# cheshmi/parsy_bench

Hardware: AMD Instinct MI355X
Metric: Cholesky factorizations/sec (+ SpTRSV solves/sec), SuiteSparse SPD set (higher is better)
Workload: dtype f64; 1 GPU; flan-class stand-in (BASELINE.json configs[2] when flan: Flan_1565): grid (116, 116, 116) 27-point stencil, geometric nested dissection; n=1560896, nnz_A_lower=21491316, nsuper=81191, nnz_L=2044454227, xsize=2421483055, etree_levels=17, launches_per_factorization=357, parallelism=1 GPU

## Files before the change

### parsy_bench_amd/csrc/capi_exec.hip

```cpp
#include <hip/hip_runtime.h>

#include <chrono>
#include <cstdio>
#include <cstring>
#include <map>
#include <algorithm>
#include <atomic>
#include <mutex>
#include <thread>
#include <string>
#include <tuple>
#include <vector>

#include "../../include/parsy_amd.h"
#include "errors.hpp"
#include "hip_check.hpp"
#include "dist.hpp"
#include "executor.hpp"
#include "inspector.hpp"
#include "refine.hpp"

using parsy::set_last_error;

namespace {

double now_s() {
    return std::chrono::duration<double>(std::chrono::steady_clock::now().time_since_epoch()).count();
}

int pick_device() {
    const char* e = std::getenv("PARSY_DEVICE");
    return e ? std::atoi(e) : 0;
}

uint64_t fnv(uint64_t h, const void* p, size_t bytes) {
    const unsigned char* c = (const unsigned char*)p;
    uint64_t lane[4] = {h, h ^ 0x9E3779B97F4A7C15ULL, h ^ 0xC2B2AE3D27D4EB4FULL, h ^ 0x165667B19E3779F9ULL};
    size_t i = 0;
    for (; i + 32 <= bytes; i += 32)
        for (int k = 0; k < 4; ++k) {
            uint64_t w;
            std::memcpy(&w, c + i + 8 * k, 8);
            lane[k] = (lane[k] ^ w) * 1099511628211ULL;
            lane[k] ^= lane[k] >> 29;
        }
    for (int k = 0; k < 4; ++k) h = (h ^ lane[k]) * 1099511628211ULL;
    for (; i < bytes; ++i) {
        h ^= c[i];
        h *= 1099511628211ULL;
    }
    return h ^ (uint64_t)bytes;
}

struct CacheKey {
    const void* a;
    const void* b;
    const void* c;
    uint64_t hash;
    int n, supNo, kind;
    bool operator<(const CacheKey& o) const {
        return std::tie(a, b, c, hash, n, supNo, kind) < std::tie(o.a, o.b, o.c, o.hash, o.n, o.supNo, o.kind);
    }
};

std::mutex g_mu;
std::map<CacheKey, parsy_plan*> g_plans;

bool validate_partition(int supNo, int nLevels, const int* levelPtr, const int* parPtr,
                        const int* partition, const char* who) {
    if (!levelPtr || !parPtr || !partition || nLevels < 1) {
        set_last_error(std::string(who) + ": null H-level schedule");
        return false;
    }
    std::vector<char> seen(supNo, 0);
    const int nparts = levelPtr[nLevels];
    int cnt = 0;
    for (int q = 0; q < nparts; ++q)
        for (int k = parPtr[q]; k < parPtr[q + 1]; ++k) {
            const int s = partition[k];
            if (s < 0 || s >= supNo || seen[s]) {
                set_last_error(std::string(who) + ": H-level partition is not a permutation of the supernodes");
                return false;
            }
            seen[s] = 1;
            ++cnt;
        }
    if (cnt != supNo) {
        set_last_error(std::string(who) + ": H-level partition does not cover every supernode");
        return false;
    }
    return true;
}

bool validate_levelset(int supNo, int nLevels, const int* levelPtr, const int* levelSet, const char* who) {
    if (!levelPtr || !levelSet || nLevels < 1 || levelPtr[nLevels] != supNo) {
        set_last_error(std::string(who) + ": level set does not cover every supernode");
        return false;
    }
    std::vector<char> seen(supNo, 0);
    for (int k = 0; k < supNo; ++k) {
        const int s = levelSet[k];
        if (s < 0 || s >= supNo || seen[s]) {
            set_last_error(std::string(who) + ": level set is not a permutation of the supernodes");
            return false;
        }
        seen[s] = 1;
    }
    return true;
}

void loud(const char* who) {
    std::fprintf(stderr, "[parsy_amd] %s failed: %s\n", who, parsy_last_error());
}

parsy_plan* cached_chol_plan(int n, int supNo, const int* blockSet, const size_t* lC,
                             const size_t* Li_ptr, const int* lR, const int* aTree,
                             const int* col2Sup, const int* cT, const int* rT, const int* c,
                             const int* r) {
    uint64_t h = 1469598103934665603ULL;
    h = fnv(h, blockSet, sizeof(int) * (supNo + 1));
    h = fnv(h, lR, sizeof(int) * Li_ptr[n]);
    h = fnv(h, c, sizeof(int) * (n + 1));
    h = fnv(h, r, sizeof(int) * c[n]);
    h = fnv(h, Li_ptr, sizeof(size_t) * (n + 1));
    h = fnv(h, lC, sizeof(size_t) * (n + 1));
    h = fnv(h, aTree, sizeof(int) * supNo);
    CacheKey key{blockSet, lR, c, h, n, supNo, 0};
    std::lock_guard<std::mutex> lk(g_mu);
    auto it = g_plans.find(key);
    if (it != g_plans.end()) return it->second;
    parsy_plan* pl = parsy_plan_create(n, supNo, blockSet, lC, Li_ptr, lR, aTree, col2Sup, cT, rT, c, r,
                                       pick_device());
    if (pl) g_plans[key] = pl;
    return pl;
}

parsy_plan* cached_chol_plan_prune(int n, int supNo, const int* blockSet, const size_t* lC, const size_t* Li_ptr,
                                   const int* lR, const int* prunePtr, const int* pruneSet, const int* c,
                                   const int* r) {
    uint64_t h = 1469598103934665603ULL;
    h = fnv(h, blockSet, sizeof(int) * (supNo + 1));
    h = fnv(h, lR, sizeof(int) * Li_ptr[n]);
    h = fnv(h, c, sizeof(int) * (n + 1));
    h = fnv(h, r, sizeof(int) * c[n]);
    h = fnv(h, Li_ptr, sizeof(size_t) * (n + 1));
    h = fnv(h, lC, sizeof(size_t) * (n + 1));
    h = fnv(h, prunePtr, sizeof(int) * (supNo + 1));
    h = fnv(h, pruneSet, sizeof(int) * prunePtr[supNo]);
    CacheKey key{blockSet, lR, c, h, n, supNo, 2};
    std::lock_guard<std::mutex> lk(g_mu);
    auto it = g_plans.find(key);
    if (it != g_plans.end()) return it->second;
    const int dev = pick_device();
    if (dev >= parsy_device_count()) {
        set_last_error("cholesky_left_par_05_prune: no usable HIP device " + std::to_string(dev) +
                       " (this library has no CPU fallback)");
        return nullptr;
    }
    std::vector<int> col2sup(n), sparent(supNo, -1);
    for (int s = 0; s < supNo; ++s)
        for (int k = blockSet[s]; k < blockSet[s + 1]; ++k) col2sup[k] = s;
    for (int s = 0; s < supNo; ++s) {
        const int w = blockSet[s + 1] - blockSet[s];
        const size_t b = Li_ptr[blockSet[s]], e = Li_ptr[blockSet[s + 1]];
        if (e - b > (size_t)w) sparent[s] = col2sup[lR[b + w]];
    }
    parsy::PatternRef P;
    P.n = n;
    P.nsuper = supNo;
    P.super = blockSet;
    P.col2sup = col2sup.data();
    P.sparent = sparent.data();
    P.i_ptr = Li_ptr;
    P.s = lR;
    P.prunePtr = prunePtr;
    P.pruneSet = pruneSet;
    parsy_plan* pl = parsy::plan_build(P, lC, c, r, dev);
    if (pl) g_plans[key] = pl;
    return pl;
}

parsy_plan* cached_solve_plan(int n, int supNo, const size_t* Lp, const int* Li, const size_t* Li_ptr,
                              const int* sup2col) {
    uint64_t h = 1469598103934665603ULL;
    h = fnv(h, sup2col, sizeof(int) * (supNo + 1));
    h = fnv(h, Li, sizeof(int) * Li_ptr[n]);
    h = fnv(h, Li_ptr, sizeof(size_t) * (n + 1));
    h = fnv(h, Lp, sizeof(size_t) * (n + 1));
    CacheKey key{sup2col, Li, Lp, h, n, supNo, 1};
    std::lock_guard<std::mutex> lk(g_mu);
    auto it = g_plans.find(key);
    if (it != g_plans.end()) return it->second;
    std::vector<int> col2sup(n), sparent(supNo, -1);
    for (int s = 0; s < supNo; ++s)
        for (int k = sup2col[s]; k < sup2col[s + 1]; ++k) col2sup[k] = s;
    for (int s = 0; s < supNo; ++s) {
        const int w = sup2col[s + 1] - sup2col[s];
        const size_t b = Li_ptr[sup2col[s]], e = Li_ptr[sup2col[s + 1]];
        if (e - b > (size_t)w) sparent[s] = col2sup[Li[b + w]];
    }
    parsy::PatternRef P;
    P.n = n;
    P.nsuper = supNo;
    P.super = sup2col;
    P.col2sup = col2sup.data();
    P.sparent = sparent.data();
    P.i_ptr = Li_ptr;
    P.s = Li;
    if (parsy_device_count() < 1) {
        set_last_error("no usable HIP device: the BCSC solve has no CPU fallback in this library");
        return nullptr;
    }
    parsy_plan* pl = parsy::plan_build(P, Lp, nullptr, nullptr, pick_device());
    if (pl) g_plans[key] = pl;
    return pl;
}

int dropin_solve(const char* who, int n, size_t* Lp, int* Li, double* Lx, size_t* Li_ptr,
                 int* sup2col, int supNo, double* x) {
    if (!Lp || !Li || !x) return 0;
    parsy_plan* pl = cached_solve_plan(n, supNo, Lp, Li, Li_ptr, sup2col);
    std::unique_lock<std::mutex> use;
    if (pl) use = std::unique_lock<std::mutex>(pl->use_mu);
    if (!pl || parsy_solve_host(pl, Lx, x, 1, n, nullptr) != 0) {
        loud(who);
        return 0;
    }
    return 1;
}

}

extern "C" {

int parsy_device_count(void) {
    int n = 0;
    if (hipGetDeviceCount(&n) != hipSuccess) return 0;
    return n;
}

parsy_plan* parsy_plan_create(int n, int supNo, const int* blockSet, const size_t* lC,
                              const size_t* Li_ptr, const int* lR, const int* aTree,
                              const int* col2Sup, const int* cT, const int* rT, const int* c,
                              const int* r, int device) {
    if (!blockSet || !lC || !Li_ptr || !lR || !aTree || !col2Sup || !cT || !rT || !c || !r || n < 0 ||
        supNo < 0) {
        set_last_error("parsy_plan_create: null or negative argument");
        return nullptr;
    }
    if (device >= 0 && device >= parsy_device_count()) {
        set_last_error("parsy_plan_create: no usable HIP device " + std::to_string(device) +
                       " (this library has no CPU fallback; pass device < 0 for a host-only schedule)");
        return nullptr;
    }
    parsy::PatternRef P;
    P.n = n;
    P.nsuper = supNo;
    P.super = blockSet;
    P.col2sup = col2Sup;
    P.sparent = aTree;
    P.i_ptr = Li_ptr;
    P.s = lR;
    P.A1p = cT;
    P.A1i = rT;
    return parsy::plan_build(P, lC, c, r, device);
}

parsy_plan* parsy_plan_from_symbolic(const parsy_symbolic* sym, int device) {
    const parsy::Symbolic* S = parsy_symbolic_cxx(sym);
    if (!S) {
        set_last_error("parsy_plan_from_symbolic: null symbolic");
        return nullptr;
    }
    return parsy_plan_create(S->n, S->nsuper, S->super.data(), S->p.data(), S->i_ptr.data(), S->s.data(),
                             S->sparent.data(), S->col2sup.data(), S->A1.p.data(), S->A1.i.data(),
                             S->A2.p.data(), S->A2.i.data(), device);
}

void parsy_plan_destroy(parsy_plan* plan) { parsy::plan_free(plan); }

int parsy_plan_get_info(const parsy_plan* pl, parsy_plan_info* o) {
    if (!pl || !o) return -1;
    const parsy::Schedule& S = pl->S;
    std::memset(o, 0, sizeof(*o));
    o->n = S.n;
    o->nsuper = S.nsuper;
    o->nlevels = S.nlevels;
    o->max_width = S.max_width;
    o->max_rows = S.max_rows;
    o->n_small = S.n_small;
    o->n_big = S.n_big;
    o->chol_launches = (int32_t)S.chol.size() + 1;
    o->solve_launches = (int32_t)S.solve.size();
    o->nnzA = S.nnzA;
    o->ssize = S.ssize;
    o->xsize = S.xsize;
    o->nnzL = S.nnzL;
    o->n_updates = (int64_t)S.upd.size();
    o->relpos_len = (int64_t)S.relpos.size();
    o->device_bytes = pl->device_bytes;
    o->flops_stored = S.flops_stored;
    o->update_flops = S.update_flops;
    o->reread_bytes = S.reread_bytes;
    o->inner_flops = S.inner_flops;
    o->tile_update_flops = S.tile_update_flops;
    o->big_flops = S.big_flops;
    o->big_entries = (int64_t)S.big_entries.size();
    o->big_tasks = (int32_t)S.big_tasks.size();
    o->n_pieces = (int32_t)S.csn.size();
    o->chol_levels = S.cnlevels;
    o->piece_width = S.piece_width;
    o->big_min_k = S.big_min_k;
    o->chol_subtrees = (int32_t)S.small_ranges.size() / 2;
    for (size_t b = 0; b + 1 < S.small_ranges.size(); b += 2) o->chol_subtree_supernodes += S.small_ranges[b + 1] - S.small_ranges[b];
    o->solve_subtrees = (int32_t)S.solve_small_ranges.size() / 2;
    for (size_t b = 0; b + 1 < S.solve_small_ranges.size(); b += 2)
        o->solve_subtree_supernodes += S.solve_small_ranges[b + 1] - S.solve_small_ranges[b];
    o->backsolve_launches = (int32_t)S.bsolve.size();
    for (const parsy::Launch& l : S.chol)
        if (l.kind == parsy::kLaunchDense) o->dense_tasks += l.count;
    o->dense_flops = S.dense_flops;
    o->dense_entries = S.n_dense_entries;
    o->solve_one = (S.solve_one ? 1 : 0) | (S.solve_one_back ? 2 : 0) | ((S.solve_one || S.solve_one_back) && S.one_subtrees ? 4 : 0);
    o->solve_one_blocks = S.solve_one ? (int32_t)S.one_f.sn.size() : S.solve_one_back ? (int32_t)S.one_back().sn.size() : 0;
    o->sub_mrhs_trees = (int32_t)S.sub_trees.size();
    o->sub_mrhs_slots = S.sub_max_slots;
    o->sub_mrhs_tiers = (int32_t)S.sub_tiers.size();
    o->sub_mrhs_cover_level = S.sub_cover_level;
    o->dense_strip_entries = S.n_strip_entries;
    return 0;
}

long long parsy_plan_chain_check(const parsy_plan* pl, int slots) {
    if (!pl || slots < 1) {
        set_last_error("parsy_plan_chain_check: null plan or slots < 1");
        return -1;
    }
    return (long long)simulate_chain(pl->S, slots);
}

long long parsy_plan_check(const parsy_plan* pl) {
    if (!pl) {
        set_last_error("parsy_plan_check: null plan");
        return -1;
    }
    std::string what;
    const long long bad = (long long)parsy::check_schedule(pl->S, what);
    if (bad) set_last_error("parsy_plan_check: " + what);
    return bad;
}

int parsy_plan_set_active(parsy_plan* pl, const uint8_t* mask) {
    if (!pl) return -1;
    std::vector<uint8_t> pieces;
    if (pl->piece_mask_set) pieces = pl->S.active_piece;
    parsy::build_launches(pl->S, mask, pl->piece_mask_set ? pieces.data() : nullptr);
    pl->sn_mask_set = mask != nullptr;
    return parsy::plan_upload_launches(pl);
}

int parsy_plan_set_active_pieces(parsy_plan* pl, const uint8_t* piece_mask) {
    if (!pl) return -1;
    std::vector<uint8_t> sn_mask;
    if (pl->sn_mask_set) sn_mask = pl->S.active;
    parsy::build_launches(pl->S, pl->sn_mask_set ? sn_mask.data() : nullptr, piece_mask);
    pl->piece_mask_set = piece_mask != nullptr;
    return parsy::plan_upload_launches(pl);
}

int parsy_plan_pieces(const parsy_plan* pl, int32_t* supernode, int32_t* level, int32_t* col0, int32_t* width,
                      int32_t* rows, int64_t* value_begin, int64_t* value_end) {
    if (!pl) return -1;
    const parsy::Schedule& S = pl->S;
    const int nc = (int)S.csn.size();
    for (int p = 0; p < nc; ++p) {
        const parsy::SnDesc& C = S.csn[(size_t)p];
        const parsy::SnDesc& R = S.sn[(size_t)S.csn_real[(size_t)p]];
        if (supernode) supernode[p] = S.csn_real[(size_t)p];
        if (level) level[p] = S.level_of.empty() ? 0 : S.level_of[(size_t)p];
        if (col0) col0[p] = C.c0;
        if (width) width[p] = C.w;
        if (rows) rows[p] = C.r;
        if (value_begin) value_begin[p] = R.px + (int64_t)C.rbias * R.r;
        if (value_end) value_end[p] = R.px + (int64_t)(C.rbias + C.w) * R.r;
    }
    return nc;
}

int parsy_plan_solve_levels(const parsy_plan* pl, int32_t* level) {
    if (!pl) return -1;
    const parsy::Schedule& S = pl->S;
    if (level)
        for (int l = 0; l < S.nlevels; ++l)
            for (int q = S.levelPtr[(size_t)l]; q < S.levelPtr[(size_t)l + 1]; ++q) level[S.levelSet[(size_t)q]] = l;
    return S.nlevels;
}

int64_t parsy_debug_big_entries(const parsy_plan* pl, int32_t* out, int64_t cap) {
    if (!pl) return -1;
    const parsy::Schedule& S = pl->S;
    int64_t n = 0, t = 0;
    for (const parsy::Schedule::BigTask& b : S.big_all) {
        for (int64_t e = b.e0; e < b.e1; ++e, ++n) {
            if (!out || n >= cap) continue;
            const parsy::WaveEntry& E = S.big_entries[(size_t)e];
            int32_t* o = out + 7 * n;
            o[0] = (int32_t)t;
            o[1] = b.src_level * 2 + (b.next ? 0 : 1);
            o[2] = E.K;
            o[3] = E.mn & 255;
            o[4] = (E.mn >> 8) & 255;
            o[5] = ((E.mn >> 16) & 1) != 0;
            o[6] = E.ia - E.ja;
        }
        ++t;
    }
    return n;
}

int64_t parsy_debug_big_windows(const parsy_plan* pl, int64_t* out, int64_t cap) {
    if (!pl) return -1;
    const parsy::Schedule& S = pl->S;
    int64_t n = 0, t = 0;
    for (const parsy::Schedule::BigTask& b : S.big_all) {
        for (int64_t e = b.e0; e < b.e1; ++e, ++n) {
            if (!out || n >= cap) continue;
            const parsy::WaveEntry& E = S.big_entries[(size_t)e];
            int64_t* o = out + 9 * n;
            o[0] = t;
            o[1] = b.src_level * 2 + (b.next ? 0 : 1);
            o[2] = E.K;
            o[3] = E.mn & 255;
            o[4] = (E.mn >> 8) & 255;
            o[5] = E.ia;
            o[6] = E.ja;
            o[7] = E.src;
            o[8] = e < b.em;
        }
        ++t;
    }
    return n;
}

int64_t parsy_debug_dense_tasks(const parsy_plan* pl, int32_t* out, int64_t cap) {
    if (!pl) return -1;
    const parsy::Schedule& S = pl->S;
    int64_t n = 0;
    int li = 0;
    for (const parsy::Launch& l : S.chol) {
        if (l.kind != parsy::kLaunchDense) continue;
        for (int q = l.first; q < l.first + l.count; ++q, ++n)
            if (out && n < cap) {
                out[2 * n] = li;
                out[2 * n + 1] = S.big_tasks[(size_t)q].part;
            }
        ++li;
    }
    return n;
}

int64_t parsy_debug_launch_times(const parsy_plan* pl, double* out, int64_t cap) {
    if (!pl) return -1;
    const int64_t n = (int64_t)std::min(pl->pev_ms.size(), pl->pev_kind.size());
    for (int64_t i = 0; out && i < n && i < cap; ++i) {
        out[4 * i] = pl->pev_kind[(size_t)i];
        out[4 * i + 1] = (size_t)i < pl->pev_level.size() ? pl->pev_level[(size_t)i] : -1;
        out[4 * i + 2] = (size_t)i < pl->pev_count.size() ? pl->pev_count[(size_t)i] : 0;
        out[4 * i + 3] = pl->pev_ms[(size_t)i];
    }
    return n;
}

int parsy_factor_begin(parsy_plan* pl, const double* d_values, double* d_lValues, void* stream, int flags) {
    if (!pl || !d_values || !d_lValues) {
        set_last_error("parsy_factor_begin: null argument");
        return -1;
    }
    return parsy::plan_factor_begin(pl, d_values, d_lValues, (hipStream_t)stream, (flags & PARSY_FACTOR_NO_INIT) == 0);
}

int parsy_factor_level(parsy_plan* pl, int level, double* d_lValues, void* stream) {
    if (!pl || !d_lValues) {
        set_last_error("parsy_factor_level: null argument");
        return -1;
    }
    return parsy::plan_factor_levels(pl, level, level + 1, d_lValues, (hipStream_t)stream);
}

int parsy_factor_end(parsy_plan* pl, void* stream) {
    if (!pl) {
        set_last_error("parsy_factor_end: null plan");
        return -1;
    }
    return parsy::plan_factor_end(pl, (hipStream_t)stream);
}

int parsy_factor_device(parsy_plan* pl, const double* d_values, double* d_lValues, void* stream) {
    if (!pl || !d_values || !d_lValues) {
        set_last_error("parsy_factor_device: null argument");
        return -1;
    }
    return parsy::plan_factor(pl, d_values, d_lValues, (hipStream_t)stream);
}

int parsy_factor_device_ex(parsy_plan* pl, const double* d_values, double* d_lValues, void* stream,
                           int flags) {
    if (!pl || !d_values || !d_lValues) {
        set_last_error("parsy_factor_device_ex: null argument");
        return -1;
    }
    return parsy::plan_factor(pl, d_values, d_lValues, (hipStream_t)stream,
                              (flags & PARSY_FACTOR_NO_INIT) == 0);
}

int parsy_factor_status(parsy_plan* pl) {
    if (!pl || pl->device < 0) return -1;
    int v = 0;
    if (hipMemcpy(&v, pl->dp.info, sizeof(int), hipMemcpyDeviceToHost) != hipSuccess) return -1;
    return v >= 0x7f7f7f7f ? 0 : v;
}

int parsy_solve_status(parsy_plan* pl) {
    if (!pl || pl->device < 0) return -1;
    int v = 0;
    const int* word = pl->solve_status_word ? pl->solve_status_word : pl->dp.sinfo;
    if (hipMemcpy(&v, word, sizeof(int), hipMemcpyDeviceToHost) != hipSuccess) return -1;
    if (v < 0) set_last_error("solve: a hand-off wait inside a chain launch timed out; x is not the solution");
    return v < 0 ? -1 : 0;
}

int parsy_solve_device(parsy_plan* pl, const double* d_lValues, double* d_x, int nrhs, int ldx,
                       void* stream) {
    if (!pl || !d_lValues || !d_x) {
        set_last_error("parsy_solve_device: null argument");
        return -1;
    }
    return parsy::plan_solve(pl, d_lValues, d_x, nrhs, ldx, (hipStream_t)stream);
}

double parsy_last_factor_ms(parsy_plan* pl) {
    float ms = -1;
    if (!pl || !pl->have_f) return -1;
    if (hipEventSynchronize(pl->ev_f1) != hipSuccess) return -1;
    if (hipEventElapsedTime(&ms, pl->ev_f0, pl->ev_f1) != hipSuccess) return -1;
    return ms;
}

double parsy_last_solve_ms(parsy_plan* pl) {
    float ms = -1;
    if (!pl || !pl->have_s) return -1;
    if (hipEventSynchronize(pl->ev_s1) != hipSuccess) return -1;
    if (hipEventElapsedTime(&ms, pl->ev_s0, pl->ev_s1) != hipSuccess) return -1;
    return ms;
}

int parsy_plan_profile(parsy_plan* pl, int enable) {
    if (!pl) return -1;
    pl->profile = enable != 0;
    if (enable == 2) {
        for (int k = 0; k < 10; ++k) pl->kind_ms[k] = 0, pl->kind_launches[k] = 0;
        pl->profiled_runs = 0;
        pl->level_ms.clear();
    }
    return 0;
}

int parsy_plan_profile_collect(parsy_plan* pl) { return pl ? parsy::plan_collect_profile(pl) : -1; }

int parsy_plan_profile_get(parsy_plan* pl, double* kind_ms, int* kind_launches, int* runs) {
    if (!pl) return -1;
    for (int k = 0; k < 10; ++k) {
        if (kind_ms) kind_ms[k] = pl->kind_ms[k];
        if (kind_launches) kind_launches[k] = pl->kind_launches[k];
    }
    if (runs) *runs = pl->profiled_runs;
    return 0;
}

int parsy_plan_profile_levels(parsy_plan* pl, double* main_ms, double* side_ms) {
    if (!pl) return -1;
    const int nl = pl->S.cnlevels;
    for (int l = 0; l < nl; ++l) {
        const size_t a = (size_t)l << 1, b = a | 1;
        if (main_ms) main_ms[l] = a < pl->level_ms.size() ? pl->level_ms[a] : 0.0;
        if (side_ms) side_ms[l] = b < pl->level_ms.size() ? pl->level_ms[b] : 0.0;
    }
    return nl;
}

static void build_download_bands(parsy_plan* pl) {
    const parsy::Schedule& S = pl->S;
    const int nl = S.cnlevels, np = (int)S.csn.size();
    {
        std::vector<double> bytes((size_t)nl, 0.0);
        for (int p = 0; p < np; ++p) bytes[(size_t)S.level_of[(size_t)p]] += 8.0 * S.csn[(size_t)p].w * S.csn[(size_t)p].ld;
        const double total = 8.0 * (double)S.xsize;
        pl->h_band_level.clear();
        double run = 0, next = total / 8;
        for (int l = 0; l < nl; ++l) {
            run += bytes[(size_t)l];
            if (l == nl - 1 || run >= next) {
                pl->h_band_level.push_back(l);
                while (next <= run) next += total / 8;
            }
        }
    }
    const size_t nb = pl->h_band_level.size();
    pl->h_band_runs.assign(nb, {});
    std::vector<int> band_of((size_t)nl, 0);
    for (size_t b = 0, l = 0; b < nb; ++b)
        for (; (int)l <= pl->h_band_level[b]; ++l) band_of[l] = (int)b;
    const int64_t gap = 131072;
    for (int p = 0; p < np; ++p) {
        const parsy::SnDesc& C = S.csn[(size_t)p];
        const parsy::SnDesc& R = S.sn[(size_t)S.csn_real[(size_t)p]];
        const int64_t a = R.px + (int64_t)C.rbias * R.r, e = R.px + (int64_t)(C.rbias + C.w) * R.r;
        auto& runs = pl->h_band_runs[(size_t)band_of[(size_t)S.level_of[(size_t)p]]];
        if (!runs.empty() && a - (runs.back().first + runs.back().second) <= gap && a >= runs.back().first)
            runs.back().second = std::max(runs.back().second, e - runs.back().first);
        else
            runs.push_back({a, e - a});
    }
}

int parsy_factor_host(parsy_plan* pl, const double* values, double* lValues, double* seconds) {
    if (!pl || !values || !lValues) {
        set_last_error("parsy_factor_host: null argument");
        return -1;
    }
    if (pl->device < 0) {
        set_last_error("parsy_factor_host: plan has no device");
        return -1;
    }
    const parsy::Schedule& S = pl->S;
    PARSY_HIP(hipSetDevice(pl->device));
    if (!pl->h_values_dev) PARSY_HIP(hipMalloc((void**)&pl->h_values_dev, std::max<int64_t>(S.nnzA, 1) * 8));
    if (!pl->h_L_dev) PARSY_HIP(hipMalloc((void**)&pl->h_L_dev, std::max<int64_t>(S.xsize, 1) * 8));
    PARSY_HIP(hipMemcpy(pl->h_values_dev, values, (size_t)S.nnzA * 8, hipMemcpyHostToDevice));
    const char* pe = std::getenv("PARSY_HOST_PIPELINE");
    const bool pipeline_on = !(pe && pe[0] == '0'), pipeline_forced = pe && pe[0] == '2';
    if (!pipeline_on || (!pipeline_forced && S.xsize * 8 < (int64_t)256 << 20) || pl->profile || S.cnlevels < 1) {
        if (parsy::plan_factor(pl, pl->h_values_dev, pl->h_L_dev, nullptr) != 0) return -1;
        PARSY_HIP(hipDeviceSynchronize());
        if (seconds) *seconds = parsy_last_factor_ms(pl) * 1e-3;
        PARSY_HIP(hipMemcpy(lValues, pl->h_L_dev, (size_t)S.xsize * 8, hipMemcpyDeviceToHost));
        return 0;
    }
    if (!pl->h_ready) {
        hipStream_t hs = nullptr, hc = nullptr;
        std::vector<hipEvent_t> evs;
        auto undo = [&] {
            for (hipEvent_t e : evs) (void)hipEventDestroy(e);
            if (hs) (void)hipStreamDestroy(hs);
            if (hc) (void)hipStreamDestroy(hc);
            pl->h_band_level.clear();
            pl->h_band_runs.clear();
            (void)hipGetLastError();
        };
        bool ok = hipStreamCreateWithFlags(&hs, hipStreamNonBlocking) == hipSuccess &&
                  hipStreamCreateWithFlags(&hc, hipStreamNonBlocking) == hipSuccess;
        if (ok) {
            build_download_bands(pl);
            evs.resize(pl->h_band_level.size(), nullptr);
            for (hipEvent_t& e : evs)
                if (ok && hipEventCreateWithFlags(&e, hipEventDisableTiming) != hipSuccess) {
                    e = nullptr;
                    ok = false;
                }
            ok = ok && !evs.empty();
        }
        if (!ok) {
            evs.erase(std::remove(evs.begin(), evs.end(), (hipEvent_t) nullptr), evs.end());
            undo();
            if (parsy::plan_factor(pl, pl->h_values_dev, pl->h_L_dev, nullptr) != 0) return -1;
            PARSY_HIP(hipDeviceSynchronize());
            if (seconds) *seconds = parsy_last_factor_ms(pl) * 1e-3;
            PARSY_HIP(hipMemcpy(lValues, pl->h_L_dev, (size_t)S.xsize * 8, hipMemcpyDeviceToHost));
            return 0;
        }
        pl->h_stream = hs;
        pl->h_copy = hc;
        pl->h_band_ev = evs;
        pl->h_ready = true;
    }
    const size_t nb = pl->h_band_level.size();
    std::atomic<int> recorded{0};
    std::atomic<int> failed{0};
    double* const dL = pl->h_L_dev;
    const int device = pl->device;
    std::thread worker([&, dL, device] {
        if (hipSetDevice(device) != hipSuccess) {
            failed = 1;
            return;
        }
        for (size_t b = 0; b < nb; ++b) {
            while (recorded.load(std::memory_order_acquire) <= (int)b && !failed.load()) std::this_thread::yield();
            if (failed.load()) return;
            if (hipEventSynchronize(pl->h_band_ev[b]) != hipSuccess) {
                failed = 1;
                return;
            }
            for (const auto& r : pl->h_band_runs[b])
                if (hipMemcpyAsync(lValues + r.first, dL + r.first, (size_t)r.second * 8, hipMemcpyDeviceToHost, pl->h_copy) !=
                    hipSuccess) {
                    failed = 1;
                    return;
                }
            if (hipStreamSynchronize(pl->h_copy) != hipSuccess) {
                failed = 1;
                return;
            }
        }
    });
    int rc = parsy::plan_factor_begin(pl, pl->h_values_dev, dL, pl->h_stream, true);
    size_t b = 0;
    for (int lev = 0; rc == 0 && lev < S.cnlevels; ++lev) {
        rc = parsy::plan_factor_levels(pl, lev, lev + 1, dL, pl->h_stream);
        if (rc == 0 && b < nb && pl->h_band_level[b] == lev) {
            if (hipEventRecord(pl->h_band_ev[b], pl->h_stream) != hipSuccess) rc = -1;
            ++b;
            recorded.store((int)b, std::memory_order_release);
        }
    }
    if (rc == 0) rc = parsy::plan_factor_end(pl, pl->h_stream);
    if (rc != 0) {
        failed = 1;
        worker.join();
        parsy::plan_factor_abort(pl, pl->h_stream);
        return -1;
    }
    const hipError_t es = hipStreamSynchronize(pl->h_stream);
    worker.join();
    if (es != hipSuccess || failed.load()) {
        set_last_error("parsy_factor_host: the pipelined download failed");
        return -1;
    }
    if (seconds) *seconds = parsy_last_factor_ms(pl) * 1e-3;
    return 0;
}

int parsy_solve_host(parsy_plan* pl, const double* lValues, double* x, int nrhs, int ldx,
                     double* seconds) {
    if (!pl || !lValues || !x) {
        set_last_error("parsy_solve_host: null argument");
        return -1;
    }
    if (pl->device < 0) {
        set_last_error("parsy_solve_host: plan has no device");
        return -1;
    }
    const parsy::Schedule& S = pl->S;
    PARSY_HIP(hipSetDevice(pl->device));
    if (!pl->h_L_dev) PARSY_HIP(hipMalloc((void**)&pl->h_L_dev, std::max<int64_t>(S.xsize, 1) * 8));
    const int64_t need = (int64_t)ldx * nrhs;
    PARSY_HIP(parsy::grow_device(pl->h_x_dev, pl->h_x_len, need));
    PARSY_HIP(hipMemcpy(pl->h_L_dev, lValues, (size_t)S.xsize * 8, hipMemcpyHostToDevice));
    PARSY_HIP(hipMemcpy(pl->h_x_dev, x, (size_t)need * 8, hipMemcpyHostToDevice));
    if (parsy::plan_solve(pl, pl->h_L_dev, pl->h_x_dev, nrhs, ldx, nullptr) != 0) return -1;
    PARSY_HIP(hipDeviceSynchronize());
    if (parsy_solve_status(pl) != 0) return -1;
    if (seconds) *seconds = parsy_last_solve_ms(pl) * 1e-3;
    PARSY_HIP(hipMemcpy(x, pl->h_x_dev, (size_t)need * 8, hipMemcpyDeviceToHost));
    return 0;
}

int parsy_backsolve_device(parsy_plan* pl, const double* d_lValues, double* d_x, int nrhs, int ldx,
                           void* stream) {
    if (!pl || !d_lValues || !d_x) {
        set_last_error("parsy_backsolve_device: null argument");
        return -1;
    }
    return parsy::plan_backsolve(pl, d_lValues, d_x, nrhs, ldx, (hipStream_t)stream);
}

int parsy_solve_levels_device(parsy_plan* pl, const double* d_lValues, double* d_x, int nrhs, int ldx, void* stream,
                              int level_begin, int level_end, int flags) {
    if (!pl || !d_lValues || !d_x) {
        set_last_error("parsy_solve_levels_device: null argument");
        return -1;
    }
    return parsy::plan_solve_levels(pl, d_lValues, d_x, nrhs, ldx, (hipStream_t)stream, level_begin, level_end, flags);
}

int parsy_copy_segments_device(double* d_dst, const double* d_src, const int64_t* d_dst_off,
                               const int64_t* d_src_off, const int32_t* d_len, int64_t nseg, void* stream) {
    if (nseg < 0 || (nseg > 0 && (!d_dst || !d_src || !d_dst_off || !d_src_off || !d_len))) {
        set_last_error("parsy_copy_segments_device: null argument");
        return -1;
    }
    parsy::launch_copy_segments(d_dst, d_src, d_dst_off, d_src_off, d_len, nseg, (hipStream_t)stream);
    PARSY_HIP(hipGetLastError());
    return 0;
}

int parsy_rhs_ones_device(parsy_plan* pl, const double* d_lValues, double* d_b, void* stream) {
    if (!pl || !d_lValues || !d_b || pl->device < 0) {
        set_last_error("parsy_rhs_ones_device: null argument or plan without a device");
        return -1;
    }
    PARSY_HIP(hipSetDevice(pl->device));
    PARSY_HIP(hipMemsetAsync(d_b, 0, (size_t)pl->S.n * sizeof(double), (hipStream_t)stream));
    parsy::launch_rhs_ones(pl->dp, pl->S.nsuper, pl->S.max_rows, d_lValues, d_b, (hipStream_t)stream);
    PARSY_HIP(hipGetLastError());
    return 0;
}

int parsy_solve2_host(parsy_plan* pl, const double* lValues, double* x, int nrhs, int ldx, int forward,
                      double* seconds) {
    if (!pl || !lValues || !x) {
        set_last_error("parsy_solve2_host: null argument");
        return -1;
    }
    if (pl->device < 0) {
        set_last_error("parsy_solve2_host: plan has no device");
        return -1;
    }
    const parsy::Schedule& S = pl->S;
    PARSY_HIP(hipSetDevice(pl->device));
    if (!pl->h_L_dev) PARSY_HIP(hipMalloc((void**)&pl->h_L_dev, std::max<int64_t>(S.xsize, 1) * 8));
    const int64_t need = (int64_t)ldx * nrhs;
    PARSY_HIP(parsy::grow_device(pl->h_x_dev, pl->h_x_len, need));
    PARSY_HIP(hipMemcpy(pl->h_L_dev, lValues, (size_t)S.xsize * 8, hipMemcpyHostToDevice));
    PARSY_HIP(hipMemcpy(pl->h_x_dev, x, (size_t)need * 8, hipMemcpyHostToDevice));
    double sec = 0;
    if (forward) {
        if (parsy::plan_solve(pl, pl->h_L_dev, pl->h_x_dev, nrhs, ldx, nullptr) != 0) return -1;
        PARSY_HIP(hipDeviceSynchronize());
        if (parsy_solve_status(pl) != 0) return -1;
        sec += parsy_last_solve_ms(pl) * 1e-3;
    }
    if (parsy::plan_backsolve(pl, pl->h_L_dev, pl->h_x_dev, nrhs, ldx, nullptr) != 0) return -1;
    PARSY_HIP(hipDeviceSynchronize());
    if (parsy_solve_status(pl) != 0) return -1;
    sec += parsy_last_solve_ms(pl) * 1e-3;
    if (seconds) *seconds = sec;
    PARSY_HIP(hipMemcpy(x, pl->h_x_dev, (size_t)need * 8, hipMemcpyDeviceToHost));
    return 0;
}

int parsy_plan_set_perm(parsy_plan* pl, const int* perm) {
    if (!pl) {
        set_last_error("parsy_plan_set_perm: null plan");
        return -1;
    }
    return parsy::plan_set_perm(pl, perm);
}

int parsy_residual_device(parsy_plan* pl, const double* d_values, const double* d_x, int ldx, const double* d_b, int ldb,
                          double* d_r, int ldr, int nrhs, double* berr, void* stream) {
    if (!pl || !d_values || !d_x || !d_b) {
        set_last_error("parsy_residual_device: null argument");
        return -1;
    }
    return parsy::plan_residual(pl, d_values, d_x, ldx, d_b, ldb, d_r, ldr, nrhs, berr, (hipStream_t)stream);
}

int parsy_solve_spd_device(parsy_plan* pl, const double* d_values, const double* d_lValues, const double* d_b, int ldb,
                           double* d_x, int ldx, int nrhs, int max_steps, int32_t* steps, double* berr, void* stream) {
    if (!pl || !d_values || !d_lValues || !d_b || !d_x) {
        set_last_error("parsy_solve_spd_device: null argument");
        return -1;
    }
    return parsy::plan_solve_refined(pl, d_values, d_lValues, d_b, ldb, d_x, ldx, nrhs, max_steps, steps, berr,
                                     (hipStream_t)stream);
}

int parsy_solve_spd_host(parsy_plan* pl, const double* values, const double* lValues, const double* b, int ldb,
                         double* x, int ldx, int nrhs, int max_steps, int32_t* steps, double* berr, double* seconds) {
    if (!pl || !values || !lValues || !b || !x) {
        set_last_error("parsy_solve_spd_host: null argument");
        return -1;
    }
    if (pl->device < 0) {
        set_last_error("parsy_solve_spd_host: plan was built without a device (device < 0)");
        return -1;
    }
    const parsy::Schedule& S = pl->S;
    if (nrhs < 1 || ldb < S.n || ldx < S.n) {
        set_last_error("parsy_solve_spd_host: need nrhs >= 1 and leading dimensions >= n");
        return -1;
    }
    PARSY_HIP(hipSetDevice(pl->device));
    if (!pl->h_values_dev) PARSY_HIP(hipMalloc((void**)&pl->h_values_dev, std::max<int64_t>(S.nnzA, 1) * 8));
    if (!pl->h_L_dev) PARSY_HIP(hipMalloc((void**)&pl->h_L_dev, std::max<int64_t>(S.xsize, 1) * 8));
    const int64_t need = std::max<int64_t>((int64_t)S.n * nrhs, 1);
    PARSY_HIP(parsy::grow_device(pl->h_x_dev, pl->h_x_len, need));
    const size_t row = (size_t)S.n * 8;
    PARSY_HIP(hipMemcpy(pl->h_values_dev, values, (size_t)S.nnzA * 8, hipMemcpyHostToDevice));
    PARSY_HIP(hipMemcpy(pl->h_L_dev, lValues, (size_t)S.xsize * 8, hipMemcpyHostToDevice));
    if (S.n > 0) PARSY_HIP(hipMemcpy2D(pl->h_x_dev, row, b, (size_t)ldb * 8, row, nrhs, hipMemcpyHostToDevice));
    hipEvent_t e0 = nullptr, e1 = nullptr;
    PARSY_HIP(hipEventCreate(&e0));
    if (hipEventCreate(&e1) != hipSuccess) {
        (void)hipEventDestroy(e0);
        set_last_error("parsy_solve_spd_host: hipEventCreate failed");
        return -1;
    }
    (void)hipEventRecord(e0, nullptr);
    int rc = parsy::plan_solve_refined(pl, pl->h_values_dev, pl->h_L_dev, pl->h_x_dev, S.n, pl->h_x_dev, S.n, nrhs,
                                       max_steps, steps, berr, nullptr);
    float ms = 0;
    if (rc == 0 && (hipEventRecord(e1, nullptr) != hipSuccess || hipEventSynchronize(e1) != hipSuccess ||
                    hipEventElapsedTime(&ms, e0, e1) != hipSuccess)) {
        set_last_error("parsy_solve_spd_host: timing the call failed");
        rc = -1;
    }
    (void)hipEventDestroy(e0);
    (void)hipEventDestroy(e1);
    if (rc != 0) return -1;
    if (parsy_solve_status(pl) != 0) return -1;
    if (seconds) *seconds = ms * 1e-3;
    if (S.n > 0) PARSY_HIP(hipMemcpy2D(x, (size_t)ldx * 8, pl->h_x_dev, row, row, nrhs, hipMemcpyDeviceToHost));
    return 0;
}

void parsy_dropin_reset(void) {
    std::lock_guard<std::mutex> lk(g_mu);
    for (auto& kv : g_plans) parsy::plan_free(kv.second);
    g_plans.clear();
}


bool cholesky_left_par_05(int n, int* c, int* r, double* values, size_t* lC, int* lR, size_t* Li_ptr,
                          double* lValues, int* blockSet, int supNo, double* timing, int* aTree,
                          int* cT, int* rT, int* col2Sup, int nLevels, int* levelPtr, int* levelSet,
                          int nPar, int* parPtr, int* partition, int chunk, int threads,
                          int super_max, int col_max, double* nodCost) {
    (void)levelSet; (void)nPar; (void)chunk; (void)threads; (void)super_max; (void)col_max; (void)nodCost;
    const char* who = "cholesky_left_par_05";
    const double t0 = now_s();
    if (!validate_partition(supNo, nLevels, levelPtr, parPtr, partition, who)) {
        loud(who);
        return false;
    }
    parsy_plan* pl = cached_chol_plan(n, supNo, blockSet, lC, Li_ptr, lR, aTree, col2Sup, cT, rT, c, r);
    double dev_s = 0;
    std::unique_lock<std::mutex> use;
    if (pl) use = std::unique_lock<std::mutex>(pl->use_mu);
    if (!pl || parsy_factor_host(pl, values, lValues, &dev_s) != 0) {
        loud(who);
        return false;
    }
    if (timing) {
        timing[0] = now_s() - t0;
        timing[1] = 0.0;
        timing[2] = dev_s;
    }
    return parsy_factor_status(pl) == 0;
}

bool cholesky_left_par_05_prune(int n, int* c, int* r, double* values, size_t* lC, int* lR, size_t* Li_ptr,
                                double* lValues, int* blockSet, int supNo, double* timing, int* prunePtr,
                                int* pruneSet, int nLevels, int* levelPtr, int* levelSet, int nPar, int* parPtr,
                                int* partition, int chunk, int threads, int super_max, int col_max,
                                double* nodCost) {
    (void)levelSet; (void)nPar; (void)chunk; (void)threads; (void)super_max; (void)col_max; (void)nodCost;
    const char* who = "cholesky_left_par_05_prune";
    const double t0 = now_s();
    if (!c || !r || !values || !lC || !lR || !Li_ptr || !lValues || !blockSet || !prunePtr || !pruneSet || n < 0 ||
        supNo < 0) {
        set_last_error(std::string(who) + ": null or negative argument");
        loud(who);
        return false;
    }
    if (!validate_partition(supNo, nLevels, levelPtr, parPtr, partition, who)) {
        loud(who);
        return false;
    }
    parsy_plan* pl = cached_chol_plan_prune(n, supNo, blockSet, lC, Li_ptr, lR, prunePtr, pruneSet, c, r);
    double dev_s = 0;
    std::unique_lock<std::mutex> use;
    if (pl) use = std::unique_lock<std::mutex>(pl->use_mu);
    if (!pl || parsy_factor_host(pl, values, lValues, &dev_s) != 0) {
        loud(who);
        return false;
    }
    if (timing) {
        timing[0] = now_s() - t0;
        timing[1] = 0.0;
        timing[2] = dev_s;
    }
    return parsy_factor_status(pl) == 0;
}

bool cholesky_left_par_waveFront(int n, int* c, int* r, double* values, size_t* lC, int* lR,
                                 size_t* Li_ptr, double* lValues, int* blockSet, int supNo,
                                 double* timing, int* aTree, int* cT, int* rT, int* col2Sup,
                                 int nLevels, int* levelPtr, int* levelSet, int chunk, int threads,
                                 int super_max, int col_max) {
    (void)chunk; (void)threads; (void)super_max; (void)col_max;
    const char* who = "cholesky_left_par_waveFront";
    const double t0 = now_s();
    if (!validate_levelset(supNo, nLevels, levelPtr, levelSet, who)) {
        loud(who);
        return false;
    }
    parsy_plan* pl = cached_chol_plan(n, supNo, blockSet, lC, Li_ptr, lR, aTree, col2Sup, cT, rT, c, r);
    double dev_s = 0;
    std::unique_lock<std::mutex> use;
    if (pl) use = std::unique_lock<std::mutex>(pl->use_mu);
    if (!pl || parsy_factor_host(pl, values, lValues, &dev_s) != 0) {
        loud(who);
        return false;
    }
    if (timing) {
        timing[0] = now_s() - t0;
        timing[1] = 0.0;
        timing[2] = dev_s;
    }
    const int st = parsy_factor_status(pl);
    if (st != 0)
        std::fprintf(stderr, "[parsy_amd] %s: non-positive pivot at column %d (the reference ignores LAPACK's info here)\n",
                     who, st);
    return true;
}

int blockedLsolve(int n, size_t* Lp, int* Li, double* Lx, int NNZ, size_t* Li_ptr, int* col2sup,
                  int* sup2col, int supNo, double* x) {
    (void)NNZ; (void)col2sup;
    return dropin_solve("blockedLsolve", n, Lp, Li, Lx, Li_ptr, sup2col, supNo, x);
}

int leveledBlockedLsolve(int n, size_t* Lp, int* Li, double* Lx, int NNZ, size_t* Li_ptr,
                         int* col2sup, int* sup2col, int supNo, double* x, int levels,
                         int* levelPtr, int* levelSet, int chunk) {
    (void)NNZ; (void)col2sup; (void)chunk;
    if (!Lp || !Li || !x) return 0;
    if (!validate_levelset(supNo, levels, levelPtr, levelSet, "leveledBlockedLsolve")) {
        loud("leveledBlockedLsolve");
        return 0;
    }
    return dropin_solve("leveledBlockedLsolve", n, Lp, Li, Lx, Li_ptr, sup2col, supNo, x);
}

int H2LeveledBlockedLsolve(int n, size_t* Lp, int* Li, double* Lx, int NNZ, size_t* Li_ptr,
                           int* col2sup, int* sup2col, int supNo, double* x, int levels,
                           int* levelPtr, int* levelSet, int parts, int* parPtr, int* partition,
                           int chunk) {
    (void)NNZ; (void)col2sup; (void)chunk; (void)levelSet; (void)parts;
    if (!Lp || !Li || !x) return 0;
    if (!validate_partition(supNo, levels, levelPtr, parPtr, partition, "H2LeveledBlockedLsolve")) {
        loud("H2LeveledBlockedLsolve");
        return 0;
    }
    return dropin_solve("H2LeveledBlockedLsolve", n, Lp, Li, Lx, Li_ptr, sup2col, supNo, x);
}

int H2LeveledBlockedLsolve_Peeled(int n, size_t* Lp, int* Li, double* Lx, int NNZ, size_t* Li_ptr,
                                  int* col2sup, int* sup2col, int supNo, double* x, int levels,
                                  int* levelPtr, int* levelSet, int parts, int* parPtr,
                                  int* partition, int chunk, int threads) {
    (void)NNZ; (void)col2sup; (void)chunk; (void)levelSet; (void)parts; (void)threads;
    if (!Lp || !Li || !x) return 0;
    if (!validate_partition(supNo, levels, levelPtr, parPtr, partition, "H2LeveledBlockedLsolve_Peeled")) {
        loud("H2LeveledBlockedLsolve_Peeled");
        return 0;
    }
    return dropin_solve("H2LeveledBlockedLsolve_Peeled", n, Lp, Li, Lx, Li_ptr, sup2col, supNo, x);
}

}
```

### parsy_bench_amd/csrc/schedule.cpp

```cpp
#include "schedule.hpp"

#include <cstdio>
#include <map>
#include <algorithm>
#include <queue>
#include <climits>
#include <cmath>
#include <cstdlib>
#include <cstdint>
#include <functional>
#include <stdexcept>
#include <string>

namespace parsy {

static inline int ceil_div(int a, int b) { return (a + b - 1) / b; }

static int env_int(const char* name, int dflt) {
    const char* v = std::getenv(name);
    if (!v || !*v) return dflt;
    return std::atoi(v);
}

static int find_subtrees(const std::vector<int>& parent, const std::vector<uint8_t>& eligible,
                         const std::vector<double>& cost, double cap, std::vector<int32_t>& subtree,
                         const std::vector<std::pair<int32_t, int32_t>>* slots = nullptr, int64_t slot_cap = 0) {
    const int ns = (int)parent.size();
    subtree.assign(ns, -1);
    std::vector<uint8_t> whole(eligible);
    std::vector<double> sub(cost);
    std::vector<int64_t> cols(slots ? ns : 0);
    for (int s = 0; s < ns && slots; ++s) cols[s] = (*slots)[s].first;
    for (int s = 0; s < ns; ++s) {
        const int p = parent[s];
        if (p < 0) continue;
        if (p <= s) return 0;
        if (!whole[s]) whole[p] = 0;
        sub[p] += sub[s];
        if (slots) cols[p] += cols[s];
    }
    int count = 0;
    for (int s = ns - 1; s >= 0; --s) {
        const int p = parent[s];
        if (p >= 0 && subtree[p] >= 0) subtree[s] = subtree[p];
        else if (whole[s] && sub[s] <= cap && (!slots || cols[s] + (*slots)[s].second <= slot_cap)) subtree[s] = count++;
    }
    return count;
}

void build_schedule(const PatternRef& P, const size_t* lC, const int* A2p, const int* A2i,
                    const uint8_t* active, Schedule& S, int compute_units) {
    S = Schedule();
    if (compute_units > 0) S.walker_batch = std::max(4, std::min(kWalkerBatch, compute_units / 2));
    const int n = P.n, ns = P.nsuper;
    S.n = n;
    S.nsuper = ns;
    S.solve_only = (A2p == nullptr);
    S.nnzA = A2p ? A2p[n] : 0;
    S.rows.assign(P.s, P.s + P.i_ptr[n]);
    S.ssize = (int64_t)P.i_ptr[n];
    S.xsize = (int64_t)lC[n];
    S.sn.resize(ns);
    for (int t = 0; t < ns; ++t) {
        SnDesc& d = S.sn[t];
        d.c0 = P.super[t];
        d.w = P.super[t + 1] - P.super[t];
        d.r = (int)(P.i_ptr[P.super[t + 1]] - P.i_ptr[P.super[t]]);
        d.ld = d.r;
        d.rbias = 0;
        d.px = (int64_t)lC[d.c0];
        d.pi = (int64_t)P.i_ptr[d.c0];
        d.a0 = A2p ? A2p[d.c0] : 0;
        d.a1 = A2p ? A2p[P.super[t + 1]] : 0;
        d.upd0 = 0;
        d.nupd = 0;
        d.dslot = -1;
        d.tflag0 = -1;
        if (d.w <= 0 || d.r < d.w) throw std::runtime_error("schedule: malformed supernode");
        if ((int64_t)d.w * d.r > 0x7fffffffLL)
            throw std::runtime_error("schedule: a single panel exceeds 2^31 entries");
        for (int col = d.c0; col < d.c0 + d.w; ++col)
            if (lC[col + 1] - lC[col] != (size_t)d.r || P.i_ptr[col] != P.i_ptr[d.c0])
                throw std::runtime_error("schedule: lC / Li_ptr are not a column-major panel layout");
        S.max_width = std::max(S.max_width, d.w);
        S.max_rows = std::max(S.max_rows, d.r);
        S.nnzL += (int64_t)d.w * d.r - (int64_t)d.w * (d.w - 1) / 2;
        for (int k = 0; k < d.w; ++k) S.flops_stored += (double)(d.r - k) * (double)(d.r - k);
        for (int k = 0; k < d.w; ++k)
            if (S.rows[d.pi + k] != d.c0 + k)
                throw std::runtime_error("schedule: supernode rows do not start with its own columns");
        if (d.w > kTile) {
            d.dslot = (int32_t)S.n_dslots;
            S.n_dslots += ceil_div(d.w, kTile);
        }
    }

    std::vector<int64_t> uptr(ns + 1, 0);
    std::vector<int> usn, ulb, uub;
    if (!S.solve_only) build_update_lists(P, uptr, usn, ulb, uub);
    std::vector<int64_t> urel(usn.size(), 0);
    S.a_dst.assign((size_t)S.nnzA, 0);
    std::vector<int> map(n, -1), stamp(n, -1);
    for (int t = 0; t < ns; ++t) {
        const SnDesc& T = S.sn[t];
        for (int k = 0; k < T.r; ++k) {
            const int row = S.rows[T.pi + k];
            map[row] = k;
            stamp[row] = t;
        }
        for (int col = T.c0; !S.solve_only && col < T.c0 + T.w; ++col)
            for (int q = A2p[col]; q < A2p[col + 1]; ++q) {
                const int row = A2i[q];
                if (stamp[row] != t) throw std::runtime_error("schedule: A entry outside the pattern of L");
                S.a_dst[q] = (int64_t)lC[col] + map[row];
            }
        for (int64_t u = uptr[t]; u < uptr[t + 1]; ++u) {
            const SnDesc& D = S.sn[usn[u]];
            urel[u] = (int64_t)S.relpos.size();
            for (int k = ulb[u]; k < D.r; ++k) {
                const int row = S.rows[D.pi + k];
                if (stamp[row] != t)
                    throw std::runtime_error("schedule: descendant row missing from the target's pattern");
                S.relpos.push_back(map[row]);
            }
            const double K = D.w, m = D.r - ulb[u], n1 = uub[u] - ulb[u] + 1;
            S.update_flops += K * n1 * (n1 + 1) + 2.0 * K * (m - n1) * n1;
            S.reread_bytes += 8.0 * K * m;
        }
    }
    if (S.relpos.size() > 0x7fffffffULL) throw std::runtime_error("schedule: relative index array exceeds int32");

    S.big_min_k = S.update_flops >= kBigAutoFlops ? kBigMinK : INT_MAX;
    S.piece_width = S.update_flops >= kPieceAutoFlops ? kPieceWidth : 0;
    if (std::getenv("PARSY_BIG_MINK")) S.big_min_k = std::max(1, env_int("PARSY_BIG_MINK", kBigMinK));
    if (std::getenv("PARSY_PIECE_WIDTH")) S.piece_width = env_int("PARSY_PIECE_WIDTH", kPieceWidth);
    if (S.piece_width > 0) S.piece_width = ceil_div(std::max(S.piece_width, kBigTile), kBigTile) * kBigTile;
    if (S.piece_width < S.big_min_k) S.piece_width = 0;
    S.push_group = std::max(1, env_int("PARSY_PUSH_GROUP", kPushGroup));
    const int split_chunks = env_int("PARSY_SPLIT_CHUNKS", kSplitChunks), split_target = std::max(1, env_int("PARSY_SPLIT_TARGET", kSplitTarget)),
              split_max = std::max(1, env_int("PARSY_SPLIT_MAX", kSplitMaxParts));
    const bool split_env = std::getenv("PARSY_SPLIT_CHUNKS") != nullptr;

    std::vector<int> tree(P.sparent, P.sparent + ns);
    S.sparent = tree;
    level_sets(tree, S.levelPtr, S.levelSet);
    S.nlevels = (int)S.levelPtr.size() - 1;

    S.piece0.assign(ns + 1, 0);
    for (int t = 0; t < ns; ++t) {
        const SnDesc& T = S.sn[t];
        S.piece0[t] = (int32_t)S.csn.size();
        int np = 1;
        const int pw = S.piece_width;
        if (!S.solve_only && pw > 0 && T.w > pw + pw / 2) {
            np = ceil_div(T.w, pw);
            if (T.w - (np - 1) * pw < pw / 2) --np;
        }
        for (int j = 0; j < np; ++j) {
            const int off = j * pw;
            SnDesc c = T;
            c.c0 = T.c0 + off;
            c.w = (j == np - 1) ? T.w - off : pw;
            c.r = T.r - off;
            c.ld = T.r;
            c.rbias = off;
            c.px = T.px + (int64_t)off * T.r + off;
            c.pi = T.pi + off;
            c.dslot = -1;
            S.csn.push_back(c);
            S.csn_real.push_back(t);
        }
    }
    const int nc = (int)S.csn.size();
    S.piece0[ns] = nc;
    {
        std::vector<int> ctree(nc, -1);
        for (int t = 0; t < ns; ++t)
            for (int p = S.piece0[t]; p < S.piece0[t + 1]; ++p)
                ctree[p] = (p + 1 < S.piece0[t + 1]) ? p + 1 : (tree[t] >= 0 ? S.piece0[tree[t]] : -1);
        level_sets(ctree, S.clevelPtr, S.clevelSet);
    }
    S.cnlevels = (int)S.clevelPtr.size() - 1;
    S.level_of.assign(nc, 0);
    for (int l = 0; l < S.cnlevels; ++l)
        for (int q = S.clevelPtr[l]; q < S.clevelPtr[l + 1]; ++q) S.level_of[S.clevelSet[q]] = l;

    for (int t = 0; t < ns && !S.solve_only; ++t) {
        const SnDesc& T = S.sn[t];
        for (int p = S.piece0[t]; p < S.piece0[t + 1]; ++p) {
            SnDesc& C = S.csn[p];
            C.upd0 = (int64_t)S.upd.size();
            const int col_lo = C.c0, col_hi = C.c0 + C.w;
            for (int64_t u = uptr[t]; u < uptr[t + 1]; ++u) {
                const SnDesc& D = S.sn[usn[u]];
                int lb = ulb[u], ub = uub[u];
                if (S.piece0[t + 1] - S.piece0[t] > 1) {
                    while (lb <= ub && S.rows[D.pi + lb] < col_lo) ++lb;
                    while (ub >= lb && S.rows[D.pi + ub] >= col_hi) --ub;
                    if (lb > ub) continue;
                }
                UpdDesc U;
                U.src = D.px + lb;
                U.ld = D.r;
                U.K = D.w;
                U.m = D.r - lb;
                U.n1 = ub - lb + 1;
                U.rel = urel[u] + (lb - ulb[u]);
                S.upd.push_back(U);
                S.upd_src.push_back(S.piece0[usn[u] + 1] - 1);
            }
            const int j = p - S.piece0[t];
            for (int g0 = 0; g0 < j; ) {
                int g1 = (g0 == j - 1) ? j : std::min(j - 1, (g0 / S.push_group + 1) * S.push_group);
                const SnDesc& Q0 = S.csn[S.piece0[t] + g0];
                int K = 0;
                for (int q = g0; q < g1; ++q) K += S.csn[S.piece0[t] + q].w;
                UpdDesc U;
                U.src = T.px + (int64_t)Q0.rbias * T.r + C.rbias;
                U.ld = T.r;
                U.K = K;
                U.m = C.r;
                U.n1 = C.w;
                U.rel = -1;
                S.upd.push_back(U);
                S.upd_src.push_back(S.piece0[t] + g1 - 1);
                g0 = g1;
            }
            C.nupd = (int)((int64_t)S.upd.size() - C.upd0);
        }
    }
    const bool forced = std::getenv("PARSY_SUBTREES") != nullptr;
    const int per_cu = env_int("PARSY_SUBTREES", kSubtreesPerCu);
    if (per_cu > 0) {
        const int cus = compute_units > 0 ? compute_units : 256;
        std::vector<uint8_t> elig(ns, 0);
        auto cut = [&](std::vector<double>& cost, double min_cost, std::vector<int32_t>& subtree,
                       const std::vector<std::pair<int32_t, int32_t>>* slots = nullptr, int64_t min_members = -1, int aim_per_cu = 0) {
            double total = 0;
            int64_t members = 0;
            {
                std::vector<int32_t> all;
                find_subtrees(tree, elig, cost, 1e300, all, slots, kSubMaxSlots);
                for (int t = 0; t < ns; ++t)
                    if (all[t] >= 0) {
                        total += cost[t];
                        ++members;
                    }
            }
            if (!forced && members < (min_members >= 0 ? min_members : (int64_t)kSubtreeMinPerSlot * per_cu * cus)) return 0;
            return find_subtrees(tree, elig, cost, std::max(min_cost, total / ((double)(aim_per_cu > 0 ? aim_per_cu : per_cu) * cus)), subtree, slots,
                                 kSubMaxSlots);
        };
        if (!S.solve_only) {
            S.chol_cost.assign(ns, 0.0);
            for (int t = 0; t < ns; ++t) {
                const SnDesc& C = S.csn[S.piece0[t]];
                elig[t] = S.piece0[t + 1] - S.piece0[t] == 1 && is_small(C);
                double c = 5e4 + (double)C.w * C.r * C.r;
                for (int64_t u = C.upd0; u < C.upd0 + C.nupd && elig[t]; ++u)
                    c += 1e4 + 2.0 * S.upd[u].K * (double)S.upd[u].m * S.upd[u].n1;
                S.chol_cost[t] = c;
            }
            S.n_chol_subtrees = cut(S.chol_cost, kSubtreeMinCost, S.chol_subtree, nullptr, -1,
                                    forced ? 0 : std::max(1, env_int("PARSY_CHOL_SUBTREES", kCholSubtreesPerCu)));
        }
        S.solve_cost.assign(ns, 0.0);
        std::vector<std::pair<int32_t, int32_t>> slots((size_t)ns);
        for (int t = 0; t < ns; ++t) {
            elig[t] = S.sn[t].w <= kTinyWidth;
            S.solve_cost[t] = 2e3 + (double)S.sn[t].w * S.sn[t].r;
            slots[(size_t)t] = {S.sn[t].w, S.sn[t].r - S.sn[t].w};
        }
        S.n_solve_subtrees = cut(S.solve_cost, kSubtreeMinCost / 16, S.solve_subtree, &slots, kSolveSubtreeMinMembers);
        S.bsolve_subtree = S.solve_subtree;
        S.n_bsolve_subtrees = S.n_solve_subtrees;
    }
    if (S.chol_subtree.empty()) S.chol_subtree.assign(ns, -1);
    if (S.solve_subtree.empty()) S.solve_subtree.assign(ns, -1);
    if (S.bsolve_subtree.empty()) S.bsolve_subtree.assign(ns, -1);

    auto is_big = [&](const UpdDesc& U, int target_piece) {
        const int real = S.csn_real[target_piece];
        return U.rel < 0 || U.K >= S.big_min_k || S.piece0[real + 1] - S.piece0[real] > 1;
    };

    S.sn_wp0.assign(nc, -1);
    S.sn_tw0.assign(nc, -1);
    struct Group { int32_t win, first, len; };
    std::vector<Group> groups, cgroups;
    std::vector<int64_t> cursor;
    struct BigKeyed { int64_t launch_tile; WaveEntry e; int16_t sr, sc; };
    std::vector<BigKeyed> bigk;
    std::vector<int64_t> big_tile0(nc + 1, 0);
    int env_sr = 0, env_sc = 0;
    if (const char* e = std::getenv("PARSY_BIG_SUPER")) {
        int a = 0, b = 0;
        const int got = std::sscanf(e, "%dx%d", &a, &b);
        if (got >= 1 && a >= 1 && a <= 64) {
            env_sr = a;
            env_sc = (got == 2 && b >= 1 && b <= 64) ? b : a;
        }
    }
    std::vector<int8_t> launch_super((size_t)2 * std::max(S.cnlevels, 1), 1);
    if (env_sr == 0 && !S.solve_only) {
        const int64_t super_min_tasks = env_int("PARSY_BIG_SUPER_MIN", kBigSuperMinTasks);
        const double super_max_fill = env_int("PARSY_BIG_SUPER_FILL", (int)(kBigSuperMaxFill * 100 + 0.5)) / 100.0;
        const int super_hi = std::max(1, std::min(8, env_int("PARSY_BIG_SUPER_HI", 2)));
        std::vector<int64_t> ltasks(launch_super.size(), 0);
        std::vector<double> lfrag(launch_super.size(), 0.0), lchunks(launch_super.size(), 0.0);
        std::vector<int64_t> keys;
        for (int t = 0; t < nc; ++t) {
            const SnDesc& T = S.csn[t];
            if (is_small(T)) continue;
            const int lev_t = S.level_of[t], nbr128 = ceil_div(T.r, kBigTile);
            keys.clear();
            for (int64_t u = T.upd0; u < T.upd0 + T.nupd; ++u) {
                const UpdDesc& U = S.upd[u];
                if (!is_big(U, t)) continue;
                const int lev_s = S.level_of[S.upd_src[u]];
                const int64_t launch = (int64_t)lev_s * 2 + (lev_s == lev_t - 1 ? 0 : 1);
                groups.clear();
                for (int k = 0; k < U.m;) {
                    const int win = (U.rel < 0 ? k : S.relpos[(size_t)U.rel + k] - T.rbias) / kBigTile;
                    int k1 = k + 1;
                    if (U.rel < 0) k1 = std::min(U.m, (win + 1) * kBigTile);
                    else while (k1 < U.m && (S.relpos[(size_t)U.rel + k1] - T.rbias) / kBigTile == win) ++k1;
                    groups.push_back(Group{win, k, k1 - k});
                    k = k1;
                }
                const double chunks = ceil_div(U.K, 16);
                for (const Group& gc : groups) {
                    if (gc.first >= U.n1) break;
                    const int nj = std::min(gc.len, U.n1 - gc.first);
                    for (const Group& gr : groups) {
                        if (gr.win < gc.win) continue;
                        keys.push_back((launch << 40) | ((int64_t)gc.win * nbr128 + gr.win));
                        lfrag[(size_t)launch] += chunks * ceil_div(gr.len, 16) * ceil_div(nj, 16);
                        lchunks[(size_t)launch] += chunks;
                    }
                }
            }
            std::sort(keys.begin(), keys.end());
            keys.erase(std::unique(keys.begin(), keys.end()), keys.end());
            for (int64_t k : keys) ltasks[(size_t)(k >> 40)]++;
        }
        for (size_t l = 0; l < launch_super.size(); ++l)
            if (ltasks[l] >= super_min_tasks && lfrag[l] < super_max_fill * 64.0 * lchunks[l]) launch_super[l] = (int8_t)super_hi;
    }
    S.big_super_r = env_sr;
    S.big_super_c = env_sc;
    std::vector<int64_t> level_tiles((size_t)std::max(S.cnlevels, 1), 0);
    if (!S.solve_only)
        for (int t = 0; t < nc; ++t)
            if (!is_small(S.csn[t])) {
                const int nbc = ceil_div(S.csn[t].w, kTile), nbr = ceil_div(S.csn[t].r, kTile);
                level_tiles[(size_t)S.level_of[t]] += (int64_t)nbc * nbr - (int64_t)nbc * (nbc - 1) / 2;
            }
    for (int t = 0; t < nc; ++t) {
        SnDesc& T = S.csn[t];
        big_tile0[t + 1] = big_tile0[t];
        if (S.solve_only) continue;
        if (is_small(T)) {
            S.n_small++;
            continue;
        }
        S.n_big++;
        const int nbc = ceil_div(T.w, kTile), nbr = ceil_div(T.r, kTile);
        if (S.n_tflags + (int64_t)nbc * nbr > 0x7fffffffLL) throw std::runtime_error("schedule: too many tiles");
        T.tflag0 = (int32_t)S.n_tflags;
        S.n_tflags += (int64_t)nbc * nbr;
        for (int jb = 1; jb < nbc; ++jb) {
            const double K = (double)jb * kTile, wb = std::min(kTile, T.w - jb * kTile);
            S.inner_flops += K * wb * (wb + 1) + 2.0 * K * (double)(T.r - jb * kTile - wb) * wb;
        }
        const int lev_t = S.level_of[t];
        auto rel_at = [&](const UpdDesc& U, int k) { return U.rel < 0 ? k : S.relpos[(size_t)U.rel + k] - T.rbias; };
        const size_t nkeys = (size_t)nbc * nbr * 8;
        auto for_each_entry = [&](auto&& fn) {
            for (int64_t u = T.upd0; u < T.upd0 + T.nupd; ++u) {
                const UpdDesc& U = S.upd[u];
                if (is_big(U, t)) continue;
                const int phase = (S.level_of[S.upd_src[u]] <= lev_t - 2) ? 0 : 1;
                groups.clear();
                for (int k = 0; k < U.m;) {
                    const int win = rel_at(U, k) / kSub;
                    int k1 = k + 1;
                    while (k1 < U.m && rel_at(U, k1) / kSub == win) ++k1;
                    groups.push_back(Group{win, k, k1 - k});
                    k = k1;
                }
                for (const Group& gc : groups) {
                    if (gc.first >= U.n1) break;
                    const int nj = std::min(gc.len, U.n1 - gc.first);
                    for (const Group& gr : groups) {
                        if (gr.win < gc.win) continue;
                        const int I = gr.win / 2, J = gc.win / 2;
                        const size_t key = (((size_t)J * nbr + I) * 2 + phase) * 4 + (gr.win & 1) * 2 + (gc.win & 1);
                        fn(key, U, gr.first, gr.len, gc.first, nj);
                    }
                }
            }
        };
        cursor.assign(nkeys + 1, 0);
        for_each_entry([&](size_t key, const UpdDesc&, int, int, int, int) { cursor[key + 1]++; });
        const int64_t base = (int64_t)S.wave_entries.size();
        for (size_t k = 0; k < nkeys; ++k) cursor[k + 1] += cursor[k];
        S.sn_wp0[t] = (int64_t)S.wave_ptr.size();
        for (size_t k = 0; k <= nkeys; ++k) S.wave_ptr.push_back(base + cursor[k]);
        S.wave_entries.resize((size_t)(base + cursor[nkeys]));
        for_each_entry([&](size_t key, const UpdDesc& U, int ia, int mi, int ja, int nj) {
            S.wave_entries[(size_t)(base + cursor[key]++)] =
                WaveEntry{U.src, (int32_t)U.rel, U.ld, U.K, ia, ja, mi | (nj << 8)};
        });
        const int nbr128 = ceil_div(T.r, kBigTile), nbc128 = ceil_div(T.w, kBigTile);
        big_tile0[t + 1] = big_tile0[t] + (int64_t)nbr128 * nbc128;
        for (int64_t u = T.upd0; u < T.upd0 + T.nupd; ++u) {
            const UpdDesc& U = S.upd[u];
            const double f = (double)U.K * U.n1 * (U.n1 + 1) + 2.0 * U.K * (double)(U.m - U.n1) * U.n1;
            if (!is_big(U, t)) {
                S.tile_update_flops += f;
                continue;
            }
            S.big_flops += f;
            const int lev_s = S.level_of[S.upd_src[u]];
            if (lev_s >= lev_t) throw std::runtime_error("schedule: an update source is not below its target");
            const int64_t launch = (int64_t)lev_s * 2 + (lev_s == lev_t - 1 ? 0 : 1);
            const int sr = env_sr ? env_sr : launch_super[(size_t)launch], sc = env_sr ? env_sc : launch_super[(size_t)launch];
            auto make_groups = [&](int win_rows, std::vector<Group>& out) {
                out.clear();
                for (int k = 0; k < U.m;) {
                    const int win = rel_at(U, k) / win_rows;
                    int k1 = k + 1;
                    if (U.rel < 0) k1 = std::min(U.m, (win + 1) * win_rows);
                    else while (k1 < U.m && rel_at(U, k1) / win_rows == win) ++k1;
                    out.push_back(Group{win, k, k1 - k});
                    k = k1;
                }
            };
            make_groups(kBigTile * sr, groups);
            if (sc == sr) cgroups = groups;
            else make_groups(kBigTile * sc, cgroups);
            for (const Group& gc : cgroups) {
                if (gc.first >= U.n1) break;
                const int njt = std::min(gc.len, U.n1 - gc.first);
                for (const Group& gr : groups) {
                    if ((int64_t)(gr.win + 1) * sr * kBigTile - 1 < (int64_t)gc.win * sc * kBigTile) continue;
                    const int64_t tile = big_tile0[t] + (int64_t)gc.win * sc * nbr128 + (int64_t)gr.win * sr;
                    for (int cb = 0; cb < njt; cb += kBigTile)
                        for (int rb = 0; rb < gr.len; rb += kBigTile) {
                            const int mi = std::min(kBigTile, gr.len - rb), nj = std::min(kBigTile, njt - cb);
                            const int ia = gr.first + rb, ja = gc.first + cb;
                            if (ia + mi - 1 < ja) continue;
                            bigk.push_back(BigKeyed{(launch << 40) | tile,
                                                    WaveEntry{U.src, (int32_t)std::max<int64_t>(U.rel, 0), U.ld, U.K, ia, ja,
                                                              mi | (nj << 8) | ((U.rel < 0) << 16)},
                                                    (int16_t)sr, (int16_t)sc});
                        }
                }
            }
        }
        S.sn_tw0[t] = (int64_t)S.tile_w.size();
        S.tile_w.resize(S.tile_w.size() + (size_t)nbc * nbr * 2, 0);
        S.tile_split.resize(S.tile_w.size() / 2, -1);
        int32_t* tw = &S.tile_w[S.sn_tw0[t]];
        int64_t* tsplit = &S.tile_split[S.sn_tw0[t] / 2];
        const int64_t* wp = &S.wave_ptr[S.sn_wp0[t]];
        for (size_t tp = 0; tp < (size_t)nbc * nbr * 2; ++tp) {
            int64_t wchunks[4];
            for (int q = 0; q < 4; ++q) {
                int64_t chunks = 0;
                for (int64_t e = wp[tp * 4 + q]; e < wp[tp * 4 + q + 1]; ++e)
                    chunks += ceil_div(S.wave_entries[(size_t)e].K, 16);
                wchunks[q] = chunks;
                tw[tp] = std::max<int32_t>(tw[tp], (int32_t)std::min<int64_t>(chunks, INT32_MAX));
            }
            const bool few = level_tiles[(size_t)lev_t] <= kSplitFewTiles && !split_env;
            if ((tp & 1) == 0 && tw[tp] > (few ? kSplitFewChunks : split_chunks)) {
                const int nparts = few ? std::min<int>(kSplitFewMaxParts, ceil_div(tw[tp], kSplitFewTarget))
                                       : std::min<int>(split_max, ceil_div(tw[tp], split_target));
                Schedule::SplitDesc sd{(int64_t)S.split_ranges.size(), S.n_split_doubles, nparts, 0};
                S.n_split_doubles += (int64_t)(nparts - 1) * kTile * kTile;
                S.split_ranges.resize(S.split_ranges.size() + (size_t)nparts * 8, 0);
                int64_t* rg = &S.split_ranges[(size_t)sd.ranges];
                for (int q = 0; q < 4; ++q) {
                    int64_t e = wp[tp * 4 + q], done = 0;
                    for (int part = 0; part < nparts; ++part) {
                        rg[part * 8 + 2 * q] = e;
                        const int64_t goal = wchunks[q] * (part + 1) / nparts;
                        while (e < wp[tp * 4 + q + 1] && (part == nparts - 1 || done < goal))
                            done += ceil_div(S.wave_entries[(size_t)e++].K, 16);
                        rg[part * 8 + 2 * q + 1] = e;
                    }
                }
                tsplit[tp / 2] = (int64_t)S.split_desc.size();
                S.split_desc.push_back(sd);
            }
        }
    }
    if (!bigk.empty()) {
        std::stable_sort(bigk.begin(), bigk.end(),
                         [](const BigKeyed& a, const BigKeyed& b) { return a.launch_tile < b.launch_tile; });
        auto is_full = [](const WaveEntry& E) {
            const int mi = E.mn & 255, nj = (E.mn >> 8) & 255;
            return mi == kBigTile && nj == kBigTile && E.K >= kDenseChunk;
        };
        const int dense_mode = env_int("PARSY_BIG_DENSE", 1);
        std::vector<double> lprod(launch_super.size(), 0.0), ldense(launch_super.size(), 0.0);
        auto products_of = [](const WaveEntry& E) {
            const int mi = E.mn & 255, nj = (E.mn >> 8) & 255;
            return (double)ceil_div(E.K, 4) * ceil_div(mi, 16) * ceil_div(nj, 16);
        };
        for (const BigKeyed& b : bigk) {
            const size_t l = (size_t)(b.launch_tile >> 40);
            lprod[l] += products_of(b.e);
            if (is_full(b.e)) ldense[l] += products_of(b.e);
        }
        std::vector<uint8_t> launch_dense(launch_super.size(), 0);
        for (size_t l = 0; l < launch_dense.size(); ++l) {
            if (dense_mode == 4) {
                launch_dense[l] = lprod[l] > 0 ? 2 : 0;
                continue;
            }
            if (dense_mode == 0 || ldense[l] <= 0) continue;
            if (dense_mode >= 2 || ldense[l] >= kDenseMinShare * lprod[l]) launch_dense[l] = 1;
            if (launch_dense[l] && lprod[l] - ldense[l] <= kDenseAllShare * lprod[l] && dense_mode != 3) launch_dense[l] = 2;
        }
        const double min_share = env_int("PARSY_DENSE_MIN_SHARE", (int)(kDenseMinShare * 100 + 0.5)) / 100.0;
        const double all_share = env_int("PARSY_DENSE_ALL_SHARE", (int)(kDenseAllShare * 100 + 0.5)) / 100.0;
        const int fill_min = env_int("PARSY_DENSE_FILL", (int)(kDenseMinFill * 100 + 0.5)) * kBigTile * kBigTile / 100;
        for (size_t l = 0; l < launch_dense.size(); ++l) {
            if (dense_mode == 4 || dense_mode == 0 || ldense[l] <= 0) continue;
            launch_dense[l] = (dense_mode >= 2 || ldense[l] >= min_share * lprod[l]) ? 1 : 0;
            if (launch_dense[l] && lprod[l] - ldense[l] <= all_share * lprod[l] && dense_mode != 3) launch_dense[l] = 2;
        }
        auto is_dense = [&](const WaveEntry& E, int mode) {
            if (mode == 2) return E.K >= kDenseChunk;
            const int mi = E.mn & 255, nj = (E.mn >> 8) & 255;
            return mode == 1 && E.K >= kDenseChunk && mi * nj >= fill_min;
        };
        S.big_entries.resize(bigk.size());
        const bool dense_strips = env_int("PARSY_DENSE_STRIPS", 1) != 0;
        std::map<std::pair<int64_t, int64_t>, size_t> strip_of;
        std::vector<uint8_t> absorbed;
        int t = 0;
        for (size_t i = 0; i < bigk.size();) {
            size_t j = i;
            while (j < bigk.size() && bigk[j].launch_tile == bigk[i].launch_tile) ++j;
            const int64_t launch = bigk[i].launch_tile >> 40, tile = bigk[i].launch_tile & ((1LL << 40) - 1);
            size_t at = i;
            int64_t weight = 0, dweight = 0, dchunks = 0;
            const int lmode = launch_dense[(size_t)launch];
            if (lmode)
                for (size_t q = i; q < j; ++q)
                    if (is_dense(bigk[q].e, lmode)) {
                        S.big_entries[at++] = bigk[q].e;
                        dchunks += ceil_div(bigk[q].e.K, kDenseChunk);
                        dweight += ceil_div(bigk[q].e.K, 16) + 2;
                        {
                            const WaveEntry& E = bigk[q].e;
                            const int mi = E.mn & 255, nj = (E.mn >> 8) & 255;
                            double pairs = 0;
                            for (int jj = E.ja; jj < E.ja + nj; ++jj) pairs += std::max(0, E.ia + mi - std::max(E.ia, jj));
                            S.dense_flops += 2.0 * E.K * pairs;
                        }
                    }
            const size_t mid = at;
            int32_t nstrips = 0;
            absorbed.assign(j - i, 0);
            if (lmode && dense_strips && mid > i) {
                strip_of.clear();
                for (size_t d = i; d < mid; ++d) {
                    const WaveEntry& E = S.big_entries[d];
                    if ((E.mn & 0xffff) == (kBigTile | (kBigTile << 8))) strip_of[{E.src, ((int64_t)E.ia << 32) | (uint32_t)E.ja}] = d;
                }
                for (size_t q = i; q < j && !strip_of.empty(); ++q) {
                    const WaveEntry& R = bigk[q].e;
                    if (is_dense(R, lmode)) continue;
                    const int mi = R.mn & 255, nj = (R.mn >> 8) & 255;
                    const bool row_strip = mi <= kStripMax && nj == kBigTile, col_strip = nj <= kStripMax && mi == kBigTile;
                    if (!row_strip && !col_strip) continue;
                    const auto it = strip_of.find({R.src, ((int64_t)(R.ia - (row_strip ? kBigTile : 0)) << 32) |
                                                          (uint32_t)(R.ja - (col_strip ? kBigTile : 0))});
                    if (it == strip_of.end()) continue;
                    WaveEntry& E = S.big_entries[it->second];
                    if (E.K != R.K || ((E.mn >> 16) & 1) != ((R.mn >> 16) & 1) || E.rel != R.rel || E.ld != R.ld) continue;
                    if ((row_strip ? big_strip_rows(E) : big_strip_cols(E)) != 0) continue;
                    if (big_strip_rows(E) == 0 && big_strip_cols(E) == 0) ++nstrips;
                    E.mn |= row_strip ? mi << 17 : nj << 22;
                    absorbed[q - i] = 1;
                    {
                        double pairs = 0;
                        for (int jj = R.ja; jj < R.ja + nj; ++jj) pairs += std::max(0, R.ia + mi - std::max(R.ia, jj));
                        S.dense_flops += 2.0 * R.K * pairs;
                    }
                    dweight += ceil_div(R.K, 64);
                }
            }
            for (size_t q = i; q < j; ++q)
                if (!is_dense(bigk[q].e, lmode) && !absorbed[q - i]) {
                    S.big_entries[at++] = bigk[q].e;
                    weight += ceil_div(bigk[q].e.K, 16) + 4;
                }
            const size_t jend = at;
            S.n_dense_entries += (int64_t)(mid - i);
            S.n_strip_entries += nstrips;
            while (t + 1 < nc && big_tile0[t + 1] <= tile) ++t;
            if (tile < big_tile0[t]) {
                t = 0;
                while (big_tile0[t + 1] <= tile) ++t;
            }
            const int nbr128 = ceil_div(S.csn[t].r, kBigTile);
            const int64_t local = tile - big_tile0[t];
            S.big_all.push_back(Schedule::BigTask{t, (int32_t)(local % nbr128) * kBigTile,
                                                  (int32_t)(local / nbr128) * kBigTile,
                                                  (int32_t)std::min<int64_t>(weight, INT32_MAX), (int64_t)i, (int64_t)jend,
                                                  (int32_t)(launch >> 1), (int32_t)((launch & 1) == 0), bigk[i].sr, bigk[i].sc,
                                                  (int64_t)mid, (int32_t)std::min<int64_t>(dweight, INT32_MAX),
                                                  (int32_t)std::min<int64_t>(dchunks, INT32_MAX), nstrips});
            i = j;
        }
    }

    build_launches(S, active);
}

static void build_solve_one(Schedule& S, bool sharded);

static bool append_sub_tier(Schedule& S, const std::vector<std::vector<int32_t>>& trees, int top_level, int max_slots) {
    const size_t members0 = S.sub_members.size(), trees0 = S.sub_trees.size(), slots0 = S.sub_slots.size(),
                 outs0 = S.sub_out_rows.size();
    auto drop = [&] {
        S.sub_members.resize(members0);
        S.sub_trees.resize(trees0);
        S.sub_slots.resize(slots0);
        S.sub_out_rows.resize(outs0);
        return false;
    };
    if (trees.empty()) return false;
    std::vector<int32_t> col_slot((size_t)S.n, -1);
    std::vector<int32_t> out_slot((size_t)S.n, -1);
    std::vector<int32_t> root_slot((size_t)S.nsuper, -1);
    std::vector<int32_t> owner;
    SubTier tier{(int32_t)trees0, 0, 0, top_level};
    for (const std::vector<int32_t>& tree : trees) {
        SubTree T{};
        T.m0 = (int32_t)S.sub_members.size();
        T.out0 = (int32_t)S.sub_out_rows.size();
        for (size_t q = tree.size(); q-- > 0;) {
            const int32_t t = tree[q];
            const SnDesc& D = S.sn[t];
            const int p = S.sparent[(size_t)t];
            const int32_t off = (p >= 0 && root_slot[(size_t)p] >= 0) ? root_slot[(size_t)p] + S.sn[p].w : 0;
            root_slot[(size_t)t] = off;
            for (int c = 0; c < D.w; ++c) col_slot[(size_t)D.c0 + c] = off + c;
            T.ncols = std::max(T.ncols, off + D.w);
        }
        std::vector<int32_t> outs;
        for (int32_t t : tree) {
            const SnDesc& D = S.sn[t];
            for (int k = D.w; k < D.r; ++k) {
                const int32_t row = S.rows[(size_t)D.pi + k];
                if (col_slot[(size_t)row] < 0 && out_slot[(size_t)row] < 0) {
                    out_slot[(size_t)row] = 0;
                    outs.push_back(row);
                }
            }
        }
        std::sort(outs.begin(), outs.end());
        T.nout = (int32_t)outs.size();
        for (int32_t j = 0; j < T.nout; ++j) out_slot[(size_t)outs[(size_t)j]] = T.ncols + j;
        S.sub_out_rows.insert(S.sub_out_rows.end(), outs.begin(), outs.end());
        const int32_t trash = T.ncols + T.nout;
        bool ok = trash + 1 <= max_slots && trash + 1 <= 65535;
        auto row_id = [&](const SnDesc& D, int k) { return k < D.w ? D.c0 + k : S.rows[(size_t)D.pi + k]; };
        auto slot_of = [&](int32_t row) { return col_slot[(size_t)row] >= 0 ? col_slot[(size_t)row] : out_slot[(size_t)row]; };
        for (size_t q = 0; q < tree.size() && ok; ++q) {
            const SnDesc& D = S.sn[tree[q]];
            for (int j0 = 0; j0 < D.w; j0 += kTinyWidth) {
                const int wb = std::min(kTinyWidth, D.w - j0);
                SubMember M{D.px + (int64_t)j0 * D.r + j0, D.c0 + j0, wb, D.r - j0, root_slot[(size_t)tree[q]] + j0,
                            (int32_t)(S.sub_slots.size() / 16), D.r};
                for (int k0 = wb; k0 < M.r; k0 += 16)
                    for (int kq = 0; kq < 4; ++kq)
                        for (int v = 0; v < 4; ++v) {
                            const int k = k0 + 4 * v + kq;
                            S.sub_slots.push_back((uint16_t)(k < M.r ? slot_of(row_id(D, j0 + k)) : trash));
                        }
                S.sub_members.push_back(M);
            }
        }
        T.m1 = (int32_t)S.sub_members.size();
        owner.assign((size_t)T.ncols, -1);
        for (size_t q = 0; q < tree.size() && ok; ++q) {
            const SnDesc& D = S.sn[tree[q]];
            for (int c = 0; c < D.w && ok; ++c) {
                int32_t& o = owner[(size_t)col_slot[(size_t)D.c0 + c]];
                ok = o < 0 || o == D.c0 + c;
                o = -1;
            }
            for (int k = D.w; k < D.r && ok; ++k) {
                const int32_t row = S.rows[(size_t)D.pi + k];
                if (col_slot[(size_t)row] < 0) continue;
                int32_t& o = owner[(size_t)col_slot[(size_t)row]];
                ok = o < 0 || o == row;
                o = row;
            }
        }
        for (int32_t o : owner) ok = ok && o < 0;
        owner.assign((size_t)T.ncols, -1);
        for (size_t q = tree.size(); q-- > 0 && ok;) {
            const SnDesc& D = S.sn[tree[q]];
            for (int k = D.w; k < D.r && ok; ++k) {
                const int32_t row = S.rows[(size_t)D.pi + k];
                if (col_slot[(size_t)row] >= 0) ok = owner[(size_t)col_slot[(size_t)row]] == row;
            }
            for (int c = 0; c < D.w; ++c) owner[(size_t)col_slot[(size_t)D.c0 + c]] = D.c0 + c;
        }
        for (int32_t t : tree) {
            const SnDesc& D = S.sn[t];
            for (int c = 0; c < D.w; ++c) col_slot[(size_t)D.c0 + c] = -1;
            root_slot[(size_t)t] = -1;
        }
        for (int32_t row : outs) out_slot[(size_t)row] = -1;
        if (!ok) return drop();
        tier.max_slots = std::max(tier.max_slots, trash + 1);
        S.sub_trees.push_back(T);
    }
    tier.ntrees = (int32_t)(S.sub_trees.size() - trees0);
    S.sub_tiers.push_back(tier);
    S.sub_max_slots = std::max(S.sub_max_slots, tier.max_slots);
    return true;
}

static void build_sub_tiers(Schedule& S) {
    S.sub_members.clear();
    S.sub_trees.clear();
    S.sub_slots.clear();
    S.sub_out_rows.clear();
    S.sub_tiers.clear();
    S.sub_max_slots = 0;
    S.sub_cover_level = -1;
    const int ns = S.nsuper;
    std::vector<uint8_t> covered((size_t)ns, 0);
    {
        std::vector<std::vector<int32_t>> trees(S.solve_small_ranges.size() / 2);
        for (size_t b = 0; b < trees.size(); ++b)
            trees[b].assign(S.solve_small_list.begin() + S.solve_small_ranges[2 * b],
                            S.solve_small_list.begin() + S.solve_small_ranges[2 * b + 1]);
        if (trees.empty() || !append_sub_tier(S, trees, -1, kSubMaxSlots + 1)) return;
        for (const auto& tr : trees)
            for (int32_t t : tr) covered[(size_t)t] = 1;
    }
    const int min_trees = env_int("PARSY_SUB_TIER_MIN_TREES", kSubTierMinTrees);
    if (min_trees <= 0) return;
    if (std::getenv("PARSY_SUB_TIER_MIN_TREES") == nullptr && S.xsize >= (int64_t)kSubTierMaxDensity * S.n) return;
    std::vector<int> level((size_t)ns, 0);
    for (int l = 0; l < S.nlevels; ++l)
        for (int q = S.levelPtr[l]; q < S.levelPtr[l + 1]; ++q) level[(size_t)S.levelSet[q]] = l;
    int lmax = S.nlevels - 1;
    for (int t = 0; t < ns; ++t)
        if (!covered[(size_t)t] && (S.sn[t].w > kSubTierMaxWidth || !S.active[t])) lmax = std::min(lmax, level[(size_t)t] - 1);
    auto trees_of_band = [&](int top, std::vector<std::vector<int32_t>>& trees) {
        std::vector<int32_t> root_of((size_t)ns, -1), tree_of((size_t)ns, -1);
        trees.clear();
        for (int t = ns - 1; t >= 0; --t) {
            if (covered[(size_t)t] || level[(size_t)t] > top) continue;
            const int p = S.sparent[(size_t)t];
            if (p >= 0 && tree_of[(size_t)p] >= 0) tree_of[(size_t)t] = tree_of[(size_t)p];
            else {
                tree_of[(size_t)t] = (int32_t)trees.size();
                trees.emplace_back();
            }
        }
        for (int t = 0; t < ns; ++t)
            if (tree_of[(size_t)t] >= 0) trees[(size_t)tree_of[(size_t)t]].push_back(t);
    };
    int next = 0;
    while (true) {
        next = S.nlevels;
        for (int t = 0; t < ns; ++t)
            if (!covered[(size_t)t]) next = std::min(next, level[(size_t)t]);
        if (next > lmax) break;
        std::vector<std::vector<int32_t>> trees, best;
        int best_top = -1;
        for (int need : {min_trees, std::max(min_trees / 4, 1)}) {
            for (int top = next; top <= lmax; ++top) {
                trees_of_band(top, trees);
                if ((int)trees.size() < need) continue;
                best.swap(trees);
                best_top = top;
            }
            if (best_top >= 0) break;
        }
        if (best_top < 0) break;
        std::vector<double> cost(best.size(), 0.0);
        for (size_t b = 0; b < best.size(); ++b)
            for (int32_t t : best[b]) cost[b] += 2e3 + (double)S.sn[t].w * S.sn[t].r;
        std::vector<size_t> order(best.size());
        for (size_t b = 0; b < order.size(); ++b) order[b] = b;
        std::stable_sort(order.begin(), order.end(), [&](size_t a, size_t b) { return cost[a] > cost[b]; });
        std::vector<std::vector<int32_t>> sorted(best.size());
        for (size_t b = 0; b < order.size(); ++b) sorted[b].swap(best[order[b]]);
        bool ok = append_sub_tier(S, sorted, best_top, kSubTierMaxSlots + 1);
        while (!ok && best_top > next) {
            --best_top;
            trees_of_band(best_top, sorted);
            ok = append_sub_tier(S, sorted, best_top, kSubTierMaxSlots + 1);
        }
        if (!ok) break;
        for (const auto& tr : sorted)
            for (int32_t t : tr) covered[(size_t)t] = 1;
        S.sub_cover_level = best_top;
    }
}

void build_launches(Schedule& S, const uint8_t* active, const uint8_t* active_pieces) {
    const int ns = S.nsuper;
    const char* fu = std::getenv("PARSY_FORCE_UNFUSED");
    const bool force_unfused = fu && fu[0] == '1';
    const int max_chain = force_unfused ? -1 : INT_MAX;
    S.n_solve_chain_launches = 0;
    S.active.assign(ns, 1);
    if (active) S.active.assign(active, active + ns);
    const int npieces = (int)S.csn.size();
    S.active_piece.assign((size_t)npieces, 1);
    for (int t = 0; t < npieces; ++t)
        S.active_piece[t] = active_pieces ? (active_pieces[t] != 0) : S.active[S.csn_real[t]];
    if (S.solve_subtree_all.empty()) {
        S.solve_subtree_all = S.solve_subtree;
        S.bsolve_subtree_all = S.bsolve_subtree;
    }
    S.solve_subtree = S.solve_subtree_all;
    S.bsolve_subtree = S.bsolve_subtree_all;
    if (active)
        for (auto* sub : {&S.solve_subtree, &S.bsolve_subtree}) {
            const int count = sub == &S.solve_subtree ? S.n_solve_subtrees : S.n_bsolve_subtrees;
            std::vector<uint8_t> whole((size_t)std::max(count, 0), 1);
            for (int t = 0; t < ns; ++t)
                if ((*sub)[t] >= 0 && !S.active[t]) whole[(size_t)(*sub)[t]] = 0;
            for (int t = 0; t < ns; ++t)
                if ((*sub)[t] >= 0 && !whole[(size_t)(*sub)[t]]) (*sub)[t] = -1;
        }
    S.small_list.clear();
    S.tiles.clear();
    S.n_chain_launches = 0;
    S.chol.clear();
    S.solve_small_list.clear();
    S.solve_panels.clear();
    S.solve_mtasks.clear();
    S.solve_fix_list.clear();
    S.solve_wide_list.clear();
    S.solve.clear();
    S.n_solve_wide = 0;

    S.big_tasks.clear();
    std::vector<Launch> early_launches;
    std::vector<size_t> level_begin;
    std::vector<int> bigs, sbigs;
    std::vector<std::vector<const Schedule::BigTask*>> big_next(S.cnlevels), big_push(S.cnlevels);
    for (const Schedule::BigTask& b : S.big_all)
        if (S.active_piece[b.sn]) (b.next ? big_next : big_push)[b.src_level].push_back(&b);
    const int big_group = env_int("PARSY_BIG_GROUP", kBigGroup);
    auto emit_big = [&](const std::vector<const Schedule::BigTask*>& all, Launch L, bool dense) {
        std::vector<const Schedule::BigTask*> v;
        for (const Schedule::BigTask* b : all)
            if (dense ? b->em > b->e0 : b->e1 > b->em) v.push_back(b);
        if (v.empty()) return L;
        L.first = (int32_t)S.big_tasks.size();
        auto wt = [dense](const Schedule::BigTask* b) { return dense ? b->dweight : b->weight; };
        auto desc = [dense](const Schedule::BigTask* b) {
            return dense ? TileDesc{b->sn, b->row0, b->col0, b->dchunks | (b->strips > 0 ? kDenseStripTask : 0), b->e0, b->em}
                         : TileDesc{b->sn, b->row0, b->col0, 0, b->em, b->e1};
        };
        auto by_weight = [&](const Schedule::BigTask* a, const Schedule::BigTask* b) { return wt(a) > wt(b); };
        int g = big_group;
        const int per_task = v[0]->sr * v[0]->sc;
        while (g > 1 && (int64_t)v.size() * per_task < (int64_t)8 * kBigGroupsPerXcd * g * g) g /= 2;
        if (g < std::max(v[0]->sr, v[0]->sc)) g = 1;
        if (g <= 1) {
            std::stable_sort(v.begin(), v.end(), by_weight);
            for (const Schedule::BigTask* b : v) S.big_tasks.push_back(desc(b));
            L.count = (int32_t)v.size();
            return L;
        }
        struct Group { int64_t key, weight; int32_t maxw; std::vector<const Schedule::BigTask*> tasks; };
        std::vector<const Schedule::BigTask*> seq[8];
        int64_t load[8] = {0, 0, 0, 0, 0, 0, 0, 0};
        auto least = [&] {
            int x = 0;
            for (int q = 1; q < 8; ++q)
                if (load[q] < load[x]) x = q;
            return x;
        };
        std::vector<const Schedule::BigTask*> rest(v);
        for (; !rest.empty(); g /= 2) {
            if (g <= 1) {
                std::stable_sort(rest.begin(), rest.end(), by_weight);
                for (const Schedule::BigTask* b : rest) {
                    const int x = least();
                    seq[x].push_back(b);
                    load[x] += wt(b);
                }
                break;
            }
            std::vector<std::pair<int64_t, const Schedule::BigTask*>> keyed;
            keyed.reserve(rest.size());
            for (const Schedule::BigTask* b : rest) {
                const int64_t gi = b->row0 / (kBigTile * g), gj = b->col0 / (kBigTile * g);
                keyed.push_back({((int64_t)b->sn << 32) | (gj << 16) | gi, b});
            }
            std::stable_sort(keyed.begin(), keyed.end(), [](const auto& a, const auto& b) { return a.first < b.first; });
            std::vector<Group> groups;
            for (const auto& kb : keyed) {
                if (groups.empty() || groups.back().key != kb.first) groups.push_back(Group{kb.first, 0, 0, {}});
                Group& G = groups.back();
                G.tasks.push_back(kb.second);
                G.weight += wt(kb.second);
                G.maxw = std::max(G.maxw, wt(kb.second));
            }
            std::stable_sort(groups.begin(), groups.end(), [](const Group& a, const Group& b) {
                return a.maxw != b.maxw ? a.maxw > b.maxw : a.weight > b.weight;
            });
            const size_t bulk = groups.size() > (size_t)kBigTailGroups ? groups.size() - kBigTailGroups : 0;
            rest.clear();
            for (size_t q = 0; q < groups.size(); ++q) {
                Group& G = groups[q];
                if (q >= bulk) {
                    rest.insert(rest.end(), G.tasks.begin(), G.tasks.end());
                    continue;
                }
                const int x = least();
                std::stable_sort(G.tasks.begin(), G.tasks.end(), by_weight);
                seq[x].insert(seq[x].end(), G.tasks.begin(), G.tasks.end());
                load[x] += G.weight;
            }
        }
        size_t len = 0;
        for (int x = 0; x < 8; ++x) len = std::max(len, seq[x].size());
        for (size_t s = 0; s < len; ++s)
            for (int x = 0; x < 8; ++x) {
                if (s < seq[x].size()) {
                    S.big_tasks.push_back(desc(seq[x][s]));
                } else {
                    S.big_tasks.push_back(TileDesc{0, 0, 0, 0, 0, 0});
                }
            }
        L.count = (int32_t)(8 * len);
        return L;
    };
    auto subtree_ranges = [&](const std::vector<int32_t>& subtree, int count, const std::vector<double>& cost,
                              auto&& position, auto&& append, std::vector<int32_t>& ranges, bool chol = false) {
        std::vector<std::vector<int32_t>> members((size_t)count);
        std::vector<double> total((size_t)count, 0.0);
        for (int t = 0; t < ns; ++t)
            if (subtree[t] >= 0 && (chol ? S.active_piece[S.piece0[t]] : S.active[t])) {
                members[(size_t)subtree[t]].push_back(t);
                total[(size_t)subtree[t]] += cost[t];
            }
        std::vector<int32_t> order;
        for (int k = 0; k < count; ++k)
            if (!members[(size_t)k].empty()) order.push_back(k);
        std::stable_sort(order.begin(), order.end(), [&](int a, int b) { return total[(size_t)a] > total[(size_t)b]; });
        for (int k : order) {
            ranges.push_back(position());
            for (int32_t t : members[(size_t)k]) append(t);
            ranges.push_back(position());
        }
        return (int32_t)order.size();
    };
    S.small_ranges.clear();
    S.solve_small_ranges.clear();
    S.bsolve_ranges.clear();
    S.sub_members.clear();
    S.sub_trees.clear();
    S.sub_slots.clear();
    S.sub_out_rows.clear();
    S.sub_max_slots = 0;
    S.bsolve_blocks.clear();
    S.bsolve_pairs.clear();
    for (int lev = 0; lev < S.cnlevels && !S.solve_only; ++lev) {
        level_begin.push_back(S.chol.size());
        bigs.clear();
        if (lev == 0 && S.n_chol_subtrees > 0) {
            Launch L{kLaunchSmall, 0, 0, 0, 0, 0, 2, 0, -1, 0};
            L.count = subtree_ranges(
                S.chol_subtree, S.n_chol_subtrees, S.chol_cost, [&] { return (int32_t)S.small_list.size(); },
                [&](int32_t t) {
                    const SnDesc& T = S.csn[S.piece0[t]];
                    S.small_list.push_back(S.piece0[t]);
                    L.lds_bytes = std::max<int32_t>(L.lds_bytes, T.w * T.r * (int)sizeof(double));
                    for (int64_t u = T.upd0; u < T.upd0 + T.nupd; ++u)
                        L.jb = std::max<int32_t>(L.jb, std::min<int64_t>((int64_t)S.upd[u].m * S.upd[u].K, 2048));
                },
                S.small_ranges, true);
            if (L.count > 0) S.chol.push_back(L);
        }
        {
            Launch L{kLaunchSmall, (int32_t)S.small_list.size(), 0, lev, 0, 0, 0, 0, -1, 0};
            for (int q = S.clevelPtr[lev]; q < S.clevelPtr[lev + 1]; ++q) {
                const int t = S.clevelSet[q];
                if (!S.active_piece[t] || S.chol_subtree[S.csn_real[t]] >= 0) continue;
                const SnDesc& T = S.csn[t];
                if (is_small(T)) {
                    S.small_list.push_back(t);
                    L.lds_bytes = std::max<int32_t>(L.lds_bytes, T.w * T.r * (int)sizeof(double));
                    for (int64_t u = T.upd0; u < T.upd0 + T.nupd; ++u)
                        L.jb = std::max<int32_t>(L.jb, std::min<int64_t>((int64_t)S.upd[u].m * S.upd[u].K, 2048));
                } else {
                    bigs.push_back(t);
                }
            }
            L.count = (int32_t)S.small_list.size() - L.first;
            if (L.count > 0) S.chol.push_back(L);
        }
        if (lev + 2 < S.cnlevels) {
            Launch Ld = emit_big(big_push[lev], Launch{kLaunchDense, 0, 0, lev + 2, 0, 0, 0, 1, lev, 1}, true);
            if (Ld.count > 0) early_launches.push_back(Ld);
            Launch Lp = emit_big(big_push[lev], Launch{kLaunchBig, 0, 0, lev + 2, 0, 0, 0, 1, lev, 1}, false);
            if (Lp.count > 0) early_launches.push_back(Lp);
        }
        if (lev > 0) {
            Launch Ld = emit_big(big_next[lev - 1], Launch{kLaunchDense, 0, 0, lev, 0, 0, 0, 0, -1, 0}, true);
            if (Ld.count > 0) S.chol.push_back(Ld);
            Launch Ln = emit_big(big_next[lev - 1], Launch{kLaunchBig, 0, 0, lev, 0, 0, 0, 0, -1, 0}, false);
            if (Ln.count > 0) S.chol.push_back(Ln);
        }
        if (!bigs.empty()) {
            {
                Launch Lt{kLaunchTiles, (int32_t)S.tiles.size(), 0, lev, 0, 0, 0, 1, lev - 2, 1};
                std::vector<std::pair<int32_t, TileDesc>> wt;
                for (int t : bigs) {
                    const SnDesc& T = S.csn[t];
                    const int nbc = ceil_div(T.w, kTile), nbr = ceil_div(T.r, kTile);
                    const int32_t* tw = &S.tile_w[S.sn_tw0[t]];
                    for (int J = 0; J < nbc; ++J)
                        for (int I = J; I < nbr; ++I) {
                            const int32_t wgt = tw[((size_t)J * nbr + I) * 2];
                            if (wgt <= 0) continue;
                            const int64_t si = S.tile_split[S.sn_tw0[t] / 2 + (size_t)J * nbr + I];
                            if (si < 0) {
                                wt.push_back({wgt, TileDesc{t, I * kTile, J * kTile, 0,
                                                            S.sn_wp0[t] + (((int64_t)J * nbr + I) * 2) * 4, -1}});
                            } else {
                                const Schedule::SplitDesc& sd = S.split_desc[(size_t)si];
                                for (int part = 0; part < sd.nparts; ++part)
                                    wt.push_back({ceil_div(wgt, sd.nparts),
                                                  TileDesc{t, I * kTile, J * kTile, part | (sd.nparts << 8),
                                                           sd.ranges + part * 8, sd.sp}});
                            }
                        }
                }
                std::stable_sort(wt.begin(), wt.end(),
                                 [](const auto& a, const auto& b) { return a.first > b.first; });
                for (auto& x : wt) S.tiles.push_back(x.second);
                Lt.count = (int32_t)S.tiles.size() - Lt.first;
                if (Lt.count > 0) early_launches.push_back(Lt);
            }
            const int chain_split_mode = env_int("PARSY_CHAIN_SPLIT", S.update_flops >= kChainSplitAutoFlops ? 2 : 0);
            auto splits = [&](int t) {
                const int real = S.csn_real[t];
                return chain_split_mode == 2 || (chain_split_mode == 1 && S.piece0[real + 1] - S.piece0[real] > 1);
            };
            bool chain_split = false;
            for (int t : bigs) chain_split = chain_split || splits(t);
            for (int part = 0; part < (chain_split ? 2 : 1); ++part) {
            Launch Lc{kLaunchChain, (int32_t)S.tiles.size(), 0, lev, S.n_chain_launches++, 0, 0, 0, -1, 0};
            Lc.fused = part;
            for (size_t b0 = 0; b0 < bigs.size(); b0 += (size_t)S.walker_batch) {
              const size_t b1 = std::min(bigs.size(), b0 + (size_t)S.walker_batch);
              int maxnb = 0;
              for (size_t q = b0; q < b1; ++q) maxnb = std::max(maxnb, ceil_div(S.csn[bigs[q]].w, kTile));
              for (int J = 0; J < maxnb; ++J)
                for (size_t q = b0; q < b1; ++q) {
                    const int t = bigs[q];
                    const SnDesc& T = S.csn[t];
                    const int nbc = ceil_div(T.w, kTile), nbr = ceil_div(T.r, kTile);
                    if (J >= nbc) continue;
                    auto push = [&](int I, int Jc) {
                        if (chain_split && ((I < nbc || !splits(t)) != (part == 0))) return;
                        const int64_t si = S.tile_split[S.sn_tw0[t] / 2 + (size_t)Jc * nbr + I];
                        S.tiles.push_back(TileDesc{t, I * kTile, Jc * kTile,
                                                   si < 0 ? 0 : S.split_desc[(size_t)si].nparts,
                                                   S.sn_wp0[t] + (((int64_t)Jc * nbr + I) * 2 + 1) * 4,
                                                   si < 0 ? -1 : S.split_desc[(size_t)si].sp});
                    };
                    if (J == 0) push(0, 0);
                    const bool next_diag = J + 1 < nbc;
                    if (next_diag) {
                        push(J + 1, J);
                        push(J + 1, J + 1);
                    }
                    for (int I = next_diag ? J + 2 : J + 1; I < nbr; ++I) push(I, J);
                }
            }
            Lc.count = (int32_t)S.tiles.size() - Lc.first;
            if (Lc.count > 0) S.chol.push_back(Lc);
            else --S.n_chain_launches;
            }
        }
    }
    S.chol_level_begin.assign(level_begin.begin(), level_begin.end());
    if (!early_launches.empty()) {
        std::vector<Launch> merged;
        size_t e = 0;
        std::stable_sort(early_launches.begin(), early_launches.end(),
                         [](const Launch& a, const Launch& b) { return a.level < b.level; });
        for (int lev = 0; lev < S.cnlevels; ++lev) {
            S.chol_level_begin[(size_t)lev] = merged.size();
            while (e < early_launches.size() && early_launches[e].level - 1 <= lev) merged.push_back(early_launches[e++]);
            const size_t b0 = level_begin[lev], b1 = lev + 1 < S.cnlevels ? level_begin[lev + 1] : S.chol.size();
            merged.insert(merged.end(), S.chol.begin() + b0, S.chol.begin() + b1);
        }
        S.chol.swap(merged);
    }
    S.chol_level_begin.push_back(S.chol.size());
    for (int lev = 0; lev < S.nlevels; ++lev) {
        sbigs.clear();
        if (lev == 0 && S.n_solve_subtrees > 0) {
            Launch L{kLaunchSolveSmall, 0, 0, 0, 0, 0, 2, 0, -1, 0};
            L.count = subtree_ranges(
                S.solve_subtree, S.n_solve_subtrees, S.solve_cost, [&] { return (int32_t)S.solve_small_list.size(); },
                [&](int32_t t) {
                    S.solve_small_list.push_back(t);
                    L.jb = std::max<int32_t>(L.jb, S.sn[t].w);
                },
                S.solve_small_ranges);
            if (L.count > 0) S.solve.push_back(L);
        }
        {
            std::vector<int32_t> tiny, narrow;
            for (int q = S.levelPtr[lev]; q < S.levelPtr[lev + 1]; ++q) {
                const int t = S.levelSet[q];
                if (!S.active[t] || S.solve_subtree[t] >= 0) continue;
                if (S.sn[t].w <= kTinyWidth) tiny.push_back(t);
                else if (S.sn[t].w <= kTile) narrow.push_back(t);
                else sbigs.push_back(t);
            }
            if (!narrow.empty() && tiny.size() < 64) {
                narrow.insert(narrow.end(), tiny.begin(), tiny.end());
                tiny.clear();
            }
            for (const std::vector<int32_t>* group : {&tiny, &narrow}) {
                if (group->empty()) continue;
                Launch L{kLaunchSolveSmall, (int32_t)S.solve_small_list.size(), (int32_t)group->size(), lev, 0, 0, 0, 0, -1, 0};
                for (int32_t t : *group) {
                    S.solve_small_list.push_back(t);
                    L.jb = std::max<int32_t>(L.jb, S.sn[t].w);
                }
                S.solve.push_back(L);
            }
        }
        if (!sbigs.empty()) {
            S.n_solve_wide += (int)sbigs.size();
            int chain_wgs = 0;
            for (int t : sbigs) chain_wgs += ceil_div(S.sn[t].r, kSolveRows);
            if (chain_wgs <= max_chain) {
                Launch Lc{kLaunchSolvePanel, (int32_t)S.solve_panels.size(), 0, lev, S.n_solve_chain_launches++, 0, 1, 0, -1, 0};
                for (int t : sbigs)
                    for (int c = 0; c * kSolveRows < S.sn[t].r; ++c)
                        S.solve_panels.push_back(PanelDesc{t, c, c * kSolveRows, 0});
                Lc.count = (int32_t)S.solve_panels.size() - Lc.first;
                Lc.lds_bytes = (int32_t)S.solve_mtasks.size();
                for (int t : sbigs)
                    for (int jb = 0; jb * kTile < S.sn[t].w; ++jb) S.solve_mtasks.push_back(PanelDesc{t, jb, -1, 0});
                for (int t : sbigs)
                    for (int c = 0, row0 = S.sn[t].w; row0 < S.sn[t].r; ++c, row0 += kSolveRowsMrhs)
                        S.solve_mtasks.push_back(PanelDesc{t, c, row0, 0});
                Lc.wait_level = (int32_t)S.solve_mtasks.size() - Lc.lds_bytes;
                S.solve.push_back(Lc);
                for (int t : sbigs) {
                    for (int jb = 0; jb * kTile < S.sn[t].w; ++jb) {
                        S.solve_wide_list.push_back(t);
                        S.solve_wide_list.push_back(jb);
                    }
                }
            } else {
                int maxnb = 0;
                for (int t : sbigs) maxnb = std::max(maxnb, ceil_div(S.sn[t].w, kTile));
                for (int jb = 0; jb < maxnb; ++jb) {
                    Launch Lp{kLaunchSolvePanel, (int32_t)S.solve_panels.size(), 0, lev, jb, 0, 0, 0, -1, 0};
                    for (int t : sbigs) {
                        const SnDesc& T = S.sn[t];
                        if (ceil_div(T.w, kTile) <= jb) continue;
                        const int wb = std::min(kTile, T.w - jb * kTile);
                        S.solve_panels.push_back(PanelDesc{t, jb, -1, 0});
                        for (int row0 = jb * kTile + wb; row0 < T.r; row0 += kSolveRows)
                            S.solve_panels.push_back(PanelDesc{t, jb, row0, 0});
                    }
                    Lp.count = (int32_t)S.solve_panels.size() - Lp.first;
                    S.solve.push_back(Lp);
                }
                S.solve_fix_list.insert(S.solve_fix_list.end(), sbigs.begin(), sbigs.end());
            }
        }
    }
    build_sub_tiers(S);
    S.bsolve.clear();
    S.bsolve_below.clear();
    S.n_bpart_slots = 0;
    const int below_mode = env_int("PARSY_BSOLVE_BELOW", 1);
    auto in_level_launches = [&](int t) { return S.active[t] && S.bsolve_subtree[t] < 0; };
    auto narrow_launches = [&](int lev) {
        std::vector<int32_t> tiny, tiny2, narrow;
        for (int q = S.levelPtr[lev]; q < S.levelPtr[lev + 1]; ++q) {
            const int t = S.levelSet[q];
            if (!in_level_launches(t) || S.sn[t].w > kTile) continue;
            (S.sn[t].w <= kTinyWidth ? tiny : S.sn[t].w <= kTinyWidth2 ? tiny2 : narrow).push_back(t);
        }
        if (tiny2.size() < 512 && !narrow.empty()) {
            narrow.insert(narrow.end(), tiny2.begin(), tiny2.end());
            tiny2.clear();
        }
        if (tiny.size() < 64 && !(tiny2.empty() && narrow.empty())) {
            (tiny2.empty() ? narrow : tiny2).insert((tiny2.empty() ? narrow : tiny2).end(), tiny.begin(), tiny.end());
            tiny.clear();
        }
        for (const std::vector<int32_t>* group : {&tiny, &tiny2, &narrow}) {
            if (group->empty()) continue;
            Launch Ln{kLaunchBackBlock, (int32_t)S.bsolve_blocks.size(), (int32_t)group->size(), lev, 0, 0, 0, 0, -1,
                      group == &tiny ? 1 : group == &tiny2 ? 2 : 0};
            for (int32_t t : *group) S.bsolve_blocks.push_back(PanelDesc{t, 0, 0, 0});
            S.bsolve.push_back(Ln);
        }
    };
    for (int lev = S.nlevels - 1; lev >= 0; --lev) {
        int maxnb = 0, wide_blocks = 0;
        for (int q = S.levelPtr[lev]; q < S.levelPtr[lev + 1]; ++q) {
            const int t = S.levelSet[q];
            if (!in_level_launches(t)) continue;
            const int nbc = ceil_div(S.sn[t].w, kTile);
            maxnb = std::max(maxnb, nbc);
            if (nbc > 1) wide_blocks += nbc;
        }
        if (wide_blocks > 0 && wide_blocks <= max_chain) {
            Launch Lc{kLaunchBackBlock, (int32_t)S.bsolve_blocks.size(), 0, lev, S.n_solve_chain_launches++,
                      (int32_t)S.bsolve_pairs.size(), 1, 0, -1, 0};
            int64_t groups_here = 0;
            for (int q = S.levelPtr[lev]; q < S.levelPtr[lev + 1]; ++q) {
                const int t = S.levelSet[q];
                if (S.active[t] && S.sn[t].w > kTile) groups_here += ceil_div(ceil_div(S.sn[t].w, kTile), kBackGroup);
            }
            const bool below_level = below_mode >= 2 || (below_mode == 1 && groups_here <= kBelowMaxGroups);
            Launch Lw{kLaunchBackBelow, (int32_t)S.bsolve_below.size(), 0, lev, 0, 0, 0, 0, -1, 0};
            for (int q = S.levelPtr[lev]; q < S.levelPtr[lev + 1]; ++q) {
                const int t = S.levelSet[q];
                const int nbc = ceil_div(S.sn[t].w, kTile);
                if (!S.active[t] || nbc < 2) continue;
                const int below = S.sn[t].r - S.sn[t].w;
                int32_t slot1 = 0;
                if (below_level && below >= (below_mode >= 2 ? 1 : kBelowRows) &&
                    S.n_bpart_slots + (int64_t)nbc * ceil_div(below, kBelowRows) < 0x7fffffffLL) {
                    const int nch = ceil_div(below, kBelowRows);
                    slot1 = (int32_t)S.n_bpart_slots + 1;
                    for (int jb = 0; jb < nbc; ++jb)
                        for (int c = 0; c < nch; ++c)
                            S.bsolve_below.push_back(PanelDesc{t, jb, S.sn[t].w + c * kBelowRows, (int32_t)(S.n_bpart_slots + (int64_t)jb * nch + c)});
                    S.n_bpart_slots += (int64_t)nbc * nch;
                }
                for (int jb = nbc - 1; jb >= 0; --jb) S.bsolve_blocks.push_back(PanelDesc{t, jb, 0, 0});
                for (int jb = nbc - 1; jb >= 0; jb -= kBackGroup)
                    S.bsolve_pairs.push_back(PanelDesc{t, jb, std::min(kBackGroup, jb + 1), slot1});
            }
            Lw.count = (int32_t)S.bsolve_below.size() - Lw.first;
            if (Lw.count > 0) S.bsolve.push_back(Lw);
            Lc.count = (int32_t)S.bsolve_blocks.size() - Lc.first;
            Lc.wait_level = (int32_t)S.bsolve_pairs.size() - Lc.lds_bytes;
            S.bsolve.push_back(Lc);
            narrow_launches(lev);
            continue;
        }
        for (int jb = maxnb - 1; jb >= 1; --jb) {
            Launch Lb{kLaunchBackBlock, (int32_t)S.bsolve_blocks.size(), 0, lev, jb, 0, 0, 0, -1, 0};
            for (int q = S.levelPtr[lev]; q < S.levelPtr[lev + 1]; ++q) {
                const int t = S.levelSet[q];
                if (in_level_launches(t) && ceil_div(S.sn[t].w, kTile) > jb) S.bsolve_blocks.push_back(PanelDesc{t, jb, 0, 0});
            }
            Lb.count = (int32_t)S.bsolve_blocks.size() - Lb.first;
            if (Lb.count > 0) S.bsolve.push_back(Lb);
        }
        if (maxnb > 1) {
            Launch Lb{kLaunchBackBlock, (int32_t)S.bsolve_blocks.size(), 0, lev, 0, 0, 0, 0, -1, 0};
            for (int q = S.levelPtr[lev]; q < S.levelPtr[lev + 1]; ++q) {
                const int t = S.levelSet[q];
                if (in_level_launches(t) && ceil_div(S.sn[t].w, kTile) > 1) S.bsolve_blocks.push_back(PanelDesc{t, 0, 0, 0});
            }
            Lb.count = (int32_t)S.bsolve_blocks.size() - Lb.first;
            if (Lb.count > 0) S.bsolve.push_back(Lb);
        }
        narrow_launches(lev);
    }
    if (S.n_bsolve_subtrees > 0) {
        Launch L{kLaunchBackBlock, 0, 0, 0, 0, 0, 2, 0, -1, 1};
        std::vector<int32_t> members;
        L.count = subtree_ranges(
            S.bsolve_subtree, S.n_bsolve_subtrees, S.solve_cost,
            [&] {
                for (size_t q = members.size(); q-- > 0;) S.bsolve_blocks.push_back(PanelDesc{members[q], 0, 0, 0});
                members.clear();
                return (int32_t)S.bsolve_blocks.size();
            },
            [&](int32_t t) { members.push_back(t); }, S.bsolve_ranges);
        if (L.count > 0) S.bsolve.push_back(L);
    }
    if (!S.solve_fix_list.empty())
        S.solve.push_back(Launch{kLaunchSolveFixup, 0, (int32_t)S.solve_fix_list.size(), S.nlevels, 0, 0, 0, 0, -1, 0});
    build_solve_one(S, active != nullptr || active_pieces != nullptr);
}

static void build_one_lists(const Schedule& S, const std::vector<uint8_t>& member, Schedule::OneLists& O) {
    const int ns = S.nsuper;
    O.clear();
    O.member = member;
    std::vector<int32_t> blk_of_col((size_t)S.n, -1), blk_sn;
    for (int q = 0; q < ns; ++q) {
        const int t = S.levelSet[(size_t)q];
        if (!member[(size_t)t]) continue;
        const SnDesc& T = S.sn[t];
        for (int cb = 0; cb < T.w; cb += kTile) {
            SnDesc B = T;
            B.c0 = T.c0 + cb;
            B.w = std::min(kTile, T.w - cb);
            B.r = T.r - cb;
            B.px = T.px + (int64_t)cb * T.r + cb;
            B.pi = T.pi + cb;
            B.ld = T.r;
            for (int c = B.c0; c < B.c0 + B.w; ++c) blk_of_col[(size_t)c] = (int32_t)O.sn.size();
            O.slot0.push_back(O.nslots);
            O.wleft.push_back(T.w - cb);
            O.nslots += B.r - B.w;
            O.sn.push_back(B);
            blk_sn.push_back(t);
        }
    }
    const int nb = (int)O.sn.size();
    if (O.nslots > INT32_MAX / 2) throw std::runtime_error("schedule: too many hand-off slots for a ONE-launch solve");
    auto col_of = [&](int p, int k) {
        const SnDesc& T = S.sn[blk_sn[(size_t)p]];
        const int kk = (O.sn[(size_t)p].c0 - T.c0) + k;
        return kk < T.w ? T.c0 + kk : S.rows[(size_t)T.pi + kk];
    };
    O.pull_ptr.assign((size_t)nb + 1, 0);
    for (int p = 0; p < nb; ++p)
        for (int k = O.sn[(size_t)p].w; k < O.sn[(size_t)p].r; ++k) {
            const int owner = blk_of_col[(size_t)col_of(p, k)];
            if (owner <= p) throw std::runtime_error("schedule: a row below a block's columns is not owned by a later block of the launch");
            O.pull_ptr[(size_t)owner + 1]++;
        }
    for (int p = 0; p < nb; ++p) O.pull_ptr[(size_t)p + 1] += O.pull_ptr[(size_t)p];
    O.pull_slot.resize((size_t)O.pull_ptr[(size_t)nb]);
    O.pull_pos.resize(O.pull_slot.size());
    std::vector<int32_t> at(O.pull_ptr.begin(), O.pull_ptr.end() - 1);
    for (int p = 0; p < nb; ++p)
        for (int k = O.sn[(size_t)p].w; k < O.sn[(size_t)p].r; ++k) {
            const int col = col_of(p, k), owner = blk_of_col[(size_t)col];
            const int32_t e = at[(size_t)owner]++;
            O.pull_slot[(size_t)e] = (int32_t)(O.slot0[(size_t)p] + (k - O.sn[(size_t)p].w));
            O.pull_pos[(size_t)e] = col - O.sn[(size_t)owner].c0;
        }
}

static void build_solve_one(Schedule& S, bool sharded) {
    const int ns = S.nsuper;
    S.solve_one = S.solve_one_back = S.one_subtrees = S.one_forced = S.one_big = false;
    S.one_f.clear();
    S.one_b.clear();
    const int mode = env_int("PARSY_SOLVE_ONE", 1);
    if (mode == 0 || sharded || ns == 0 || (int)S.levelSet.size() != ns) return;
    const bool sub = S.n_solve_subtrees > 0 || S.n_bsolve_subtrees > 0;
    std::vector<uint8_t> mf((size_t)ns, 1), mb((size_t)ns, 1);
    int64_t nf = ns, nbk = ns;
    if (sub) {
        nf = nbk = 0;
        for (int t = 0; t < ns; ++t) {
            mf[(size_t)t] = S.solve_subtree[t] < 0;
            mb[(size_t)t] = S.bsolve_subtree[t] < 0;
            nf += mf[(size_t)t];
            nbk += mb[(size_t)t];
        }
        int nfused_f = 0, nfused_b = 0;
        for (const Launch& l : S.solve) nfused_f += l.fused == 2 && l.kind == kLaunchSolveSmall;
        for (const Launch& l : S.bsolve) nfused_b += l.fused == 2 && l.kind == kLaunchBackBlock;
        const bool first_ok = nfused_f == (S.n_solve_subtrees > 0) && (nfused_f == 0 || S.solve.front().fused == 2);
        const bool last_ok = nfused_b == (S.n_bsolve_subtrees > 0) && (nfused_b == 0 || S.bsolve.back().fused == 2);
        if (!first_ok || !last_ok || nf == 0 || nbk == 0) return;
    }
    auto fits = [&](int64_t members) {
        return S.xsize <= kOneMaxEntries && members <= 2 * kOneMaxSupernodes &&
               (members <= kOneMaxSupernodes || S.xsize >= kOneLargeEntries * (int64_t)ns);
    };
    const bool ok_f = mode == 2 || fits(nf);
    const bool ok_b = mode == 2 || fits(nbk) || (sub && nbk <= kOneMaxSupernodesBig);
    S.one_big = mode != 2 && !fits(nbk);
    if (!ok_f && !ok_b) return;
    try {
        if (ok_f) build_one_lists(S, mf, S.one_f);
        if (ok_b && (!ok_f || mb != mf)) build_one_lists(S, mb, S.one_b);
    } catch (const std::runtime_error&) {
        S.one_f.clear();
        S.one_b.clear();
        S.one_big = false;
        return;
    }
    S.one_subtrees = sub;
    S.one_forced = mode == 2;
    S.solve_one = ok_f;
    S.solve_one_back = ok_b;
}

int64_t simulate_chain(const Schedule& S, int slots) {
    if (slots < 1) slots = 1;
    std::vector<uint8_t> fin((size_t)std::max<int64_t>(S.n_tflags, 1), 0), prep(fin.size(), 0);
    struct Task {
        int32_t sn, I, J, role;
        int32_t k;
    };
    int64_t stuck = 0;
    for (const Launch& L : S.chol) {
        if (L.kind != kLaunchChain) continue;
        std::vector<Task> resident;
        int64_t next = 0;
        const int64_t count = L.count;
        bool progress = true;
        while (progress && (next < count || !resident.empty())) {
            progress = false;
            while ((int)resident.size() < slots && next < count) {
                const TileDesc& td = S.tiles[(size_t)L.first + (size_t)next++];
                const SnDesc& D = S.csn[td.sn];
                const int nbc = ceil_div(D.w, kTile);
                Task t{td.sn, td.row0 / kTile, td.col0 / kTile, 3, 0};
                if (t.I == 0 && t.J == 0) t.role = 0;
                else if (t.I == t.J) t.role = 2;
                else if (t.I == t.J + 1 && t.I < nbc) t.role = 1;
                if (L.fused != 0 && t.I < nbc) ++stuck;
                resident.push_back(t);
                progress = true;
            }
            for (size_t q = 0; q < resident.size();) {
                Task& t = resident[q];
                const SnDesc& D = S.csn[t.sn];
                const int nbc = ceil_div(D.w, kTile);
                auto flag = [&](int I, int J) { return (size_t)D.tflag0 + (size_t)I * nbc + J; };
                bool done = false;
                if (t.role == 0) {
                    for (;;) {
                        fin[flag(t.k, t.k)] = 1;
                        if (t.k + 1 >= nbc) {
                            done = true;
                            break;
                        }
                        if (!prep[flag(t.k + 1, t.k)] || !prep[flag(t.k + 1, t.k + 1)]) break;
                        fin[flag(t.k + 1, t.k)] = 1;
                        ++t.k;
                        progress = true;
                    }
                } else {
                    const int need = t.role == 2 ? t.J - 1 : t.J;
                    while (t.k < need && fin[flag(t.I, t.k)] && fin[flag(t.J, t.k)]) ++t.k;
                    if (t.k >= need) {
                        if (t.role == 3) {
                            if (fin[flag(t.J, t.J)]) {
                                fin[flag(t.I, t.J)] = 1;
                                done = true;
                            }
                        } else {
                            prep[flag(t.I, t.J)] = 1;
                            done = true;
                        }
                    }
                }
                if (done) {
                    resident[q] = resident.back();
                    resident.pop_back();
                    progress = true;
                } else {
                    ++q;
                }
            }
        }
        stuck += (count - next) + (int64_t)resident.size();
    }
    return stuck;
}

static void check_solve_launches(const Schedule& S, const std::function<void(const std::string&)>& fail) {
    const int ns = S.nsuper;
    std::vector<int> level_of(ns, 0);
    for (int l = 0; l < S.nlevels; ++l)
        for (int q = S.levelPtr[l]; q < S.levelPtr[l + 1]; ++q) level_of[S.levelSet[q]] = l;
    {
        std::vector<int> seen(ns, 0);
        std::vector<int64_t> chunks(ns, 0);
        int last_level = -1;
        for (const Launch& l : S.solve) {
            if (l.kind == kLaunchSolveSmall) {
                if (l.fused == 2) {
                    for (int b = l.first; b < l.first + l.count; ++b) {
                        const int32_t q0 = S.solve_small_ranges[2 * (size_t)b], q1 = S.solve_small_ranges[2 * (size_t)b + 1];
                        if (q0 < 0 || q1 <= q0 || q1 > (int32_t)S.solve_small_list.size()) {
                            fail("forward subtree launch: bad range " + std::to_string(b));
                            continue;
                        }
                        for (int32_t q = q0; q < q1; ++q) {
                            const int t = S.solve_small_list[q];
                            seen[t]++;
                            if (q > q0 && t <= S.solve_small_list[q - 1]) fail("forward subtree run is not in index order");
                            if (S.sn[t].w > l.jb) fail("forward subtree launch: supernode wider than the launch's width class");
                        }
                    }
                } else {
                    if (l.level < last_level) fail("forward solve launches go down a level");
                    last_level = l.level;
                    for (int q = l.first; q < l.first + l.count; ++q) {
                        const int t = S.solve_small_list[q];
                        seen[t]++;
                        if (level_of[t] != l.level) fail("forward launch holds a supernode of another level");
                        if (S.sn[t].w > l.jb || S.sn[t].w > kTile) fail("forward launch: supernode wider than its width class");
                    }
                }
            } else if (l.kind == kLaunchSolvePanel) {
                if (l.level < last_level) fail("forward solve launches go down a level");
                last_level = l.level;
                for (int q = l.first; q < l.first + l.count; ++q) {
                    const PanelDesc& pd = S.solve_panels[q];
                    if (pd.sn < 0 || pd.sn >= ns || S.sn[pd.sn].w <= kTile || level_of[pd.sn] != l.level)
                        fail("forward chain launch: bad chunk descriptor " + std::to_string(q));
                    else if (l.fused) {
                        if (pd.row0 != pd.jb * kSolveRows || pd.row0 >= S.sn[pd.sn].r) fail("forward chain launch: bad chunk rows");
                        chunks[pd.sn]++;
                    }
                }
                if (l.fused) {
                    if (l.lds_bytes < 0 || l.wait_level < 0 || (size_t)l.lds_bytes + (size_t)l.wait_level > S.solve_mtasks.size())
                        fail("forward chain launch: bad task range (many right-hand sides)");
                    else {
                        std::vector<int> next_block(ns, 0);
                        std::vector<int64_t> next_row(ns, -1);
                        for (int q = l.lds_bytes; q < l.lds_bytes + l.wait_level; ++q) {
                            const PanelDesc& pd = S.solve_mtasks[(size_t)q];
                            if (pd.sn < 0 || pd.sn >= ns || S.sn[pd.sn].w <= kTile || level_of[pd.sn] != l.level) {
                                fail("forward chain launch: bad task " + std::to_string(q));
                                continue;
                            }
                            const SnDesc& T = S.sn[pd.sn];
                            if (pd.row0 < 0) {
                                if (pd.jb != next_block[pd.sn]++ || pd.jb * kTile >= T.w) fail("forward chain launch: block columns out of order");
                                if (next_row[pd.sn] >= 0) fail("forward chain launch: a block column after the row chunks that wait for it");
                            } else {
                                if (next_block[pd.sn] != ceil_div(T.w, kTile)) fail("forward chain launch: row chunk before the supernode's block columns");
                                if (next_row[pd.sn] < 0) next_row[pd.sn] = T.w;
                                if (pd.row0 != next_row[pd.sn] || pd.row0 >= T.r) fail("forward chain launch: row chunks do not tile the rows below");
                                next_row[pd.sn] = pd.row0 + kSolveRowsMrhs;
                            }
                        }
                        for (int q = l.first; q < l.first + l.count; ++q) {
                            const int t = S.solve_panels[q].sn;
                            if (t < 0 || t >= ns) continue;
                            const SnDesc& T = S.sn[t];
                            if (next_block[t] != ceil_div(T.w, kTile) || (T.r > T.w && next_row[t] < T.r) || (T.r == T.w && next_row[t] >= 0))
                                fail("forward chain launch: supernode " + std::to_string(t) + " is not covered by the many-right-hand-side tasks");
                        }
                    }
                }
            }
        }
        for (int t = 0; t < ns; ++t) {
            const bool narrow = S.sn[t].w <= kTile;
            if (narrow && seen[t] != (S.active[t] ? 1 : 0))
                fail("supernode " + std::to_string(t) + " is in " + std::to_string(seen[t]) + " forward launches");
            if (!narrow && S.solve_fix_list.empty() && chunks[t] != (S.active[t] ? ceil_div(S.sn[t].r, kSolveRows) : 0))
                fail("wide supernode " + std::to_string(t) + ": " + std::to_string(chunks[t]) + " forward chunks");
        }
    }
    {
        std::vector<int> seen(ns, 0);
        std::vector<int64_t> blocks(ns, 0), grouped(ns, 0);
        {
            std::vector<uint8_t> slot_seen((size_t)S.n_bpart_slots, 0);
            for (const PanelDesc& pd : S.bsolve_below) {
                const SnDesc& T = S.sn[(size_t)pd.sn];
                if (pd.pad < 0 || pd.pad >= S.n_bpart_slots || slot_seen[(size_t)pd.pad]++) fail("backward solve: a partial-sum slot is written twice or out of range");
                if (pd.row0 < T.w || pd.row0 >= T.r || (pd.row0 - T.w) % kBelowRows || pd.jb < 0 || pd.jb * kTile >= T.w)
                    fail("backward solve: a k_bsolve_below task has a bad chunk");
            }
            for (uint8_t v : slot_seen)
                if (v != 1) fail("backward solve: a partial-sum slot is never written");
            int64_t below_done = 0;
            for (const Launch& l : S.bsolve) {
                if (l.kind == kLaunchBackBelow) below_done += l.count;
                if (l.kind != kLaunchBackBlock || l.fused != 1) continue;
                for (int g = l.lds_bytes; g < l.lds_bytes + l.wait_level; ++g) {
                    const PanelDesc& pd = S.bsolve_pairs[(size_t)g];
                    if (pd.pad <= 0) continue;
                    const SnDesc& T = S.sn[(size_t)pd.sn];
                    const int nch = ceil_div(T.r - T.w, kBelowRows), nbc = ceil_div(T.w, kTile);
                    const int64_t last = (int64_t)(pd.pad - 1) + (int64_t)nbc * nch;
                    if (T.r <= T.w || last > S.n_bpart_slots) fail("backward solve: a chain group names partial sums that do not exist");
                    if (last > 0 && below_done < (int64_t)S.bsolve_below.size()) {
                        bool found = false;
                        for (int64_t q = 0; q < below_done && !found; ++q) found = S.bsolve_below[(size_t)q].pad == last - 1;
                        if (!found) fail("backward solve: a chain launch runs before the launch that forms its partial sums");
                    }
                }
            }
        }
        for (const Launch& l : S.bsolve) {
            if (l.kind != kLaunchBackBlock) continue;
            if (l.fused == 2) {
                for (int b = l.first; b < l.first + l.count; ++b) {
                    const int32_t q0 = S.bsolve_ranges[2 * (size_t)b], q1 = S.bsolve_ranges[2 * (size_t)b + 1];
                    if (q0 < 0 || q1 <= q0 || q1 > (int32_t)S.bsolve_blocks.size()) {
                        fail("backward subtree launch: bad range " + std::to_string(b));
                        continue;
                    }
                    for (int32_t q = q0; q < q1; ++q) {
                        const int t = S.bsolve_blocks[q].sn;
                        seen[t]++;
                        if (q > q0 && t >= S.bsolve_blocks[q - 1].sn) fail("backward subtree run is not in reverse index order");
                        if (S.sn[t].w > kTinyWidth) fail("backward subtree launch: supernode wider than the one-wave kernel");
                    }
                }
                continue;
            }
            for (int q = l.first; q < l.first + l.count; ++q) {
                const PanelDesc& pd = S.bsolve_blocks[q];
                if (pd.sn < 0 || pd.sn >= ns || pd.jb < 0 || pd.jb * kTile >= S.sn[pd.sn].w || level_of[pd.sn] != l.level) {
                    fail("backward launch: bad block descriptor " + std::to_string(q));
                    continue;
                }
                if (S.sn[pd.sn].w <= kTile) {
                    seen[pd.sn]++;
                    if (l.early == 1 && S.sn[pd.sn].w > kTinyWidth) fail("backward launch: supernode wider than its width class");
                    if (l.early == 2 && S.sn[pd.sn].w > kTinyWidth2) fail("backward launch: supernode wider than its width class");
                } else {
                    blocks[pd.sn]++;
                }
            }
            if (l.fused == 1) {
                int prev_sn = -1, next_jb = -1;
                for (int g = l.lds_bytes; g < l.lds_bytes + l.wait_level; ++g) {
                    const PanelDesc& pd = S.bsolve_pairs[(size_t)g];
                    if (pd.sn != prev_sn) {
                        if (prev_sn >= 0 && next_jb != -1) fail("backward groups of supernode " + std::to_string(prev_sn) + " stop early");
                        prev_sn = pd.sn;
                        next_jb = ceil_div(S.sn[pd.sn].w, kTile) - 1;
                    }
                    if (pd.jb != next_jb || pd.row0 < 1 || pd.row0 > kBackGroup || pd.row0 > pd.jb + 1)
                        fail("backward group " + std::to_string(g) + " does not continue its supernode's block columns");
                    grouped[pd.sn] += pd.row0;
                    next_jb = pd.jb - pd.row0;
                }
                if (prev_sn >= 0 && next_jb != -1) fail("backward groups of supernode " + std::to_string(prev_sn) + " stop early");
            }
        }
        for (int t = 0; t < ns; ++t) {
            const int nbc = ceil_div(S.sn[t].w, kTile);
            if (nbc == 1 && seen[t] != (S.active[t] ? 1 : 0))
                fail("supernode " + std::to_string(t) + " is in " + std::to_string(seen[t]) + " backward launches");
            if (nbc > 1 && blocks[t] != (S.active[t] ? nbc : 0))
                fail("wide supernode " + std::to_string(t) + ": " + std::to_string(blocks[t]) + " backward blocks");
            if (nbc > 1 && S.active[t] && !S.bsolve_pairs.empty() && grouped[t] != nbc)
                fail("wide supernode " + std::to_string(t) + ": groups cover " + std::to_string(grouped[t]) + " block columns");
        }
    }
}

template <class Fail>
static void check_one_lists(const Schedule& S, const Schedule::OneLists& O, const std::vector<int32_t>* subtree, const char* dir,
                            Fail&& fail) {
    const int ns = S.nsuper, nb = (int)O.sn.size();
    const std::string who = std::string("one-launch ") + dir + " solve: ";
    if ((int)O.member.size() != ns || (int)O.pull_ptr.size() != nb + 1 || (int)O.slot0.size() != nb || (int)O.wleft.size() != nb ||
        O.pull_slot.size() != O.pull_pos.size() || (int64_t)O.pull_slot.size() != O.nslots ||
        O.pull_ptr[(size_t)nb] != (int32_t)O.pull_slot.size()) {
        fail(who + "lists of the wrong length");
        return;
    }
    for (int t = 0; t < ns; ++t)
        if ((O.member[(size_t)t] != 0) != (subtree ? (*subtree)[(size_t)t] < 0 : true))
            fail(who + "supernode " + std::to_string(t) + " is on the wrong side of the subtree launch");
    std::vector<int32_t> blk_of_col((size_t)S.n, -1), slot_blk((size_t)O.nslots, -1), slot_col((size_t)O.nslots, -1);
    {
        int p = 0;
        int64_t slots = 0;
        for (int q = 0; q < ns; ++q) {
            const int t = S.levelSet[(size_t)q];
            if (!O.member[(size_t)t]) continue;
            const SnDesc& T = S.sn[t];
            for (int cb = 0; cb < T.w && p < nb; cb += kTile, ++p) {
                const SnDesc& B = O.sn[(size_t)p];
                const int wbk = std::min(kTile, T.w - cb);
                if (B.c0 != T.c0 + cb || B.w != wbk || B.r != T.r - cb || B.ld != T.r || B.px != T.px + (int64_t)cb * T.r + cb ||
                    B.pi != T.pi + cb || O.slot0[(size_t)p] != slots || O.wleft[(size_t)p] != T.w - cb)
                    fail(who + "block " + std::to_string(p) + " is not a block column of its supernode");
                for (int kk = cb + wbk; kk < T.r; ++kk) {
                    slot_blk[(size_t)(slots + (kk - cb - wbk))] = p;
                    slot_col[(size_t)(slots + (kk - cb - wbk))] = kk < T.w ? T.c0 + kk : S.rows[(size_t)T.pi + kk];
                }
                slots += B.r - B.w;
                for (int c = B.c0; c < B.c0 + B.w; ++c) blk_of_col[(size_t)c] = p;
            }
        }
        if (p != nb || slots != O.nslots) {
            fail(who + "the blocks do not tile the supernodes");
            return;
        }
    }
    std::vector<uint8_t> seen((size_t)O.nslots, 0);
    for (int p = 0; p < nb; ++p)
        for (int32_t e = O.pull_ptr[(size_t)p]; e < O.pull_ptr[(size_t)p + 1]; ++e) {
            const int32_t slot = O.pull_slot[(size_t)e], pos = O.pull_pos[(size_t)e];
            const bool in = slot >= 0 && slot < O.nslots;
            if (!in || seen[(size_t)slot] || pos < 0 || pos >= O.sn[(size_t)p].w || slot_col[(size_t)slot] != O.sn[(size_t)p].c0 + pos ||
                slot_blk[(size_t)slot] >= p) {
                fail(who + "bad entry " + std::to_string(e) + " in the gather list of block " + std::to_string(p));
                continue;
            }
            seen[(size_t)slot] = 1;
        }
    for (int64_t sl = 0; sl < O.nslots; ++sl)
        if (!seen[(size_t)sl]) fail(who + "slot " + std::to_string(sl) + " is never gathered");
}

template <class Fail>
static void check_solve_one(const Schedule& S, Fail&& fail) {
    if (!S.solve_one && !S.solve_one_back) return;
    if ((int)S.levelSet.size() != S.nsuper) {
        fail("one-launch solve: no level sets");
        return;
    }
    if (S.solve_one) check_one_lists(S, S.one_f, S.one_subtrees ? &S.solve_subtree : nullptr, "forward", fail);
    if (!S.solve_one_back) return;
    if (!S.one_b.sn.empty()) check_one_lists(S, S.one_b, S.one_subtrees ? &S.bsolve_subtree : nullptr, "backward", fail);
    else if (!S.solve_one) fail("one-launch backward solve: no lists");
    else if (S.one_subtrees)
        for (int t = 0; t < S.nsuper; ++t)
            if ((S.solve_subtree[t] < 0) != (S.bsolve_subtree[t] < 0)) {
                fail("one-launch backward solve: shares the forward lists although the subtree launches differ");
                break;
            }
    if (S.one_subtrees) {
        if (S.n_solve_subtrees > 0 && (S.solve.empty() || S.solve.front().fused != 2))
            fail("one-launch forward solve: the subtree launch is not the first launch");
        if (S.n_bsolve_subtrees > 0 && (S.bsolve.empty() || S.bsolve.back().fused != 2))
            fail("one-launch backward solve: the subtree launch is not the last launch");
    }
}

template <class Fail>
static void check_sub_tiers(const Schedule& S, Fail&& fail) {
    if (S.sub_tiers.empty()) return;
    const int ns = S.nsuper;
    std::vector<int32_t> sn_of_col((size_t)S.n, -1);
    for (int t = 0; t < ns; ++t)
        for (int c = 0; c < S.sn[t].w; ++c) sn_of_col[(size_t)S.sn[t].c0 + c] = t;
    std::vector<int> level((size_t)ns, 0);
    for (int l = 0; l < S.nlevels; ++l)
        for (int q = S.levelPtr[l]; q < S.levelPtr[l + 1]; ++q) level[(size_t)S.levelSet[q]] = l;
    std::vector<int32_t> tree_of((size_t)ns, -1);
    int32_t next_tree = 0;
    for (size_t k = 0; k < S.sub_tiers.size(); ++k) {
        const SubTier& R = S.sub_tiers[k];
        if (R.tree0 != next_tree || R.ntrees <= 0 || (size_t)(R.tree0 + R.ntrees) > S.sub_trees.size())
            return fail("sub tiers: tiers do not tile the trees");
        next_tree = R.tree0 + R.ntrees;
        if (k == 0 && (size_t)R.ntrees != S.solve_small_ranges.size() / 2) return fail("sub tiers: tier 0 is not the subtree launch");
        for (int32_t b = R.tree0; b < R.tree0 + R.ntrees; ++b) {
            const SubTree& T = S.sub_trees[(size_t)b];
            if (T.m0 >= T.m1 || (size_t)T.m1 > S.sub_members.size() || T.ncols + T.nout + 1 > R.max_slots ||
                (size_t)(T.out0 + T.nout) > S.sub_out_rows.size())
                return fail("sub tiers: a tree's ranges");
            int32_t prev_sn = -1, expect_c = -1;
            for (int32_t q = T.m0; q < T.m1; ++q) {
                const SubMember& M = S.sub_members[(size_t)q];
                if (M.c0 < 0 || M.c0 >= S.n || M.w < 1 || M.w > kTinyWidth) return fail("sub tiers: a member's columns");
                const int t = sn_of_col[(size_t)M.c0];
                const SnDesc& D = S.sn[t];
                const int j0 = M.c0 - D.c0;
                if (!S.active[t] || j0 % kTinyWidth != 0 || M.w != std::min(kTinyWidth, D.w - j0) || M.r != D.r - j0 || M.ld != D.r ||
                    M.px != D.px + (int64_t)j0 * D.r + j0)
                    return fail("sub tiers: a member is not a 16-column block of an active supernode");
                if (j0 == 0) {
                    if (tree_of[(size_t)t] >= 0) return fail("sub tiers: a supernode in two trees");
                    if (t <= prev_sn) return fail("sub tiers: members out of index order");
                    if (k == 0 ? S.solve_subtree[t] < 0 : (level[(size_t)t] > R.top_level || S.sn[t].w > kSubTierMaxWidth))
                        return fail("sub tiers: a supernode that does not belong to its tier");
                    tree_of[(size_t)t] = b;
                    prev_sn = t;
                } else if (t != prev_sn || M.c0 != expect_c) {
                    return fail("sub tiers: the blocks of a supernode are not in a row");
                }
                expect_c = M.c0 + M.w;
                if (M.slot0 < 0 || M.slot0 + M.w > T.ncols) return fail("sub tiers: a member's column slots");
                const int nch = (M.r - M.w + 15) / 16;
                if ((size_t)(M.so + nch) * 16 > S.sub_slots.size()) return fail("sub tiers: a member's slot words");
                for (int ch = 0; ch < nch; ++ch)
                    for (int e = 0; e < 16; ++e) {
                        const int k2 = M.w + 16 * ch + 4 * (e & 3) + (e >> 2), slot = S.sub_slots[(size_t)(M.so + ch) * 16 + e];
                        if (k2 >= M.r) {
                            if (slot != T.ncols + T.nout) return fail("sub tiers: a padding row not in the padding slot");
                            continue;
                        }
                        const int32_t row = j0 + k2 < D.w ? D.c0 + j0 + k2 : S.rows[(size_t)D.pi + j0 + k2];
                        if (slot < T.ncols) {
                            const int tt = sn_of_col[(size_t)row];
                            bool found = false;
                            for (int32_t q2 = q + 1; q2 < T.m1 && !found; ++q2) {
                                const SubMember& M2 = S.sub_members[(size_t)q2];
                                found = row >= M2.c0 && row < M2.c0 + M2.w && slot == M2.slot0 + row - M2.c0;
                            }
                            if (!found || tt < 0) return fail("sub tiers: a row's column slot does not belong to a later member");
                        } else if (slot >= T.ncols + T.nout || S.sub_out_rows[(size_t)T.out0 + slot - T.ncols] != row) {
                            return fail("sub tiers: a row's outside slot");
                        }
                    }
            }
            for (int32_t j = 0; j < T.nout; ++j) {
                const int32_t row = S.sub_out_rows[(size_t)T.out0 + j];
                if (j > 0 && row <= S.sub_out_rows[(size_t)T.out0 + j - 1]) return fail("sub tiers: outside rows not sorted");
                if (tree_of[(size_t)sn_of_col[(size_t)row]] == b) return fail("sub tiers: an outside row is a column of the tree");
            }
        }
    }
    for (int t = 0; t < ns; ++t) {
        if (S.solve_subtree[t] >= 0 && S.active[t] && tree_of[(size_t)t] < 0) return fail("sub tiers: a supernode of the subtree launch is missing");
        if (S.active[t] && level[(size_t)t] <= S.sub_cover_level && tree_of[(size_t)t] < 0) return fail("sub tiers: a covered level has a supernode outside the tiers");
    }
}

int64_t check_schedule(const Schedule& S, std::string& what) {
    int64_t bad = 0;
    auto fail = [&](const std::string& msg) {
        if (bad++ == 0) what = msg;
    };
    check_solve_launches(S, fail);
    check_solve_one(S, fail);
    check_sub_tiers(S, fail);
    if (S.solve_only) return bad;
    const int nc = (int)S.csn.size();
    for (int t = 0; t < S.nsuper; ++t) {
        int cols = 0;
        for (int p = S.piece0[t]; p < S.piece0[t + 1]; ++p) {
            const SnDesc& C = S.csn[p];
            if (C.c0 != S.sn[t].c0 + cols || C.rbias != cols || C.r != S.sn[t].r - cols || C.ld != S.sn[t].r)
                fail("piece " + std::to_string(p) + " is not a window of its supernode's panel");
            if (p > S.piece0[t] && S.level_of[p] != S.level_of[p - 1] + 1) fail("pieces of a supernode are not on consecutive levels");
            cols += C.w;
        }
        if (cols != S.sn[t].w) fail("pieces of supernode " + std::to_string(t) + " do not add up to its width");
    }
    std::vector<double> covered(S.upd.size(), 0.0);
    auto entry_flops = [](const WaveEntry& E, bool same_window) {
        const double K = E.K, mi = E.mn & 255, nj = (E.mn >> 8) & 255;
        return same_window ? K * nj * (nj + 1) + 2.0 * K * (mi - nj) * nj : 2.0 * K * mi * nj;
    };
    auto block_flops = [](const WaveEntry& E) {
        const int mi = E.mn & 255, nj = (E.mn >> 8) & 255;
        auto pairs_of = [](int ia, int m, int ja, int n) {
            double pairs = 0;
            for (int j = ja; j < ja + n; ++j) pairs += std::max(0, ia + m - std::max(ia, j));
            return pairs;
        };
        return 2.0 * E.K * (pairs_of(E.ia, mi, E.ja, nj) + pairs_of(E.ia + mi, big_strip_rows(E), E.ja, nj) +
                            pairs_of(E.ia, mi, E.ja + nj, big_strip_cols(E)));
    };
    for (int t = 0; t < nc; ++t) {
        const SnDesc& T = S.csn[t];
        for (int64_t u = T.upd0; u < T.upd0 + T.nupd; ++u)
            if (S.level_of[S.upd_src[u]] >= S.level_of[t]) fail("update " + std::to_string(u) + " comes from a level that is not below its target");
        if (is_small(T) || T.nupd == 0) continue;
        auto find_upd = [&](const WaveEntry& E) -> int64_t {
            for (int64_t u = T.upd0; u < T.upd0 + T.nupd; ++u)
                if (S.upd[u].src == E.src && S.upd[u].K == E.K) return u;
            return -1;
        };
        if (S.sn_wp0[t] >= 0) {
            const int nbc = ceil_div(T.w, kTile), nbr = ceil_div(T.r, kTile);
            const int64_t* wp = &S.wave_ptr[S.sn_wp0[t]];
            for (size_t key = 0; key < (size_t)nbc * nbr * 8; ++key)
                for (int64_t e = wp[key]; e < wp[key + 1]; ++e) {
                    const WaveEntry& E = S.wave_entries[(size_t)e];
                    const int64_t u = find_upd(E);
                    const int mi = E.mn & 255, nj = (E.mn >> 8) & 255;
                    if (u < 0 || mi < 1 || mi > kSub || nj < 1 || nj > kSub || E.ia + mi > S.upd[u].m || E.ja + nj > S.upd[u].n1) {
                        fail("wave entry " + std::to_string(e) + " of piece " + std::to_string(t) + " has a bad window");
                        continue;
                    }
                    covered[(size_t)u] += entry_flops(E, E.ia == E.ja);
                }
        }
    }
    for (const Schedule::BigTask& b : S.big_all) {
        const SnDesc& T = S.csn[b.sn];
        if (b.src_level >= S.level_of[b.sn] || (b.next != 0) != (b.src_level == S.level_of[b.sn] - 1))
            fail("BIG task of piece " + std::to_string(b.sn) + " is filed under the wrong source level");
        const int win_r = kBigTile * b.sr, win_c = kBigTile * b.sc;
        if (b.sr < 1 || b.sc < 1 || b.row0 % win_r || b.col0 % win_c || b.row0 + win_r <= b.col0 || b.row0 >= T.r || b.col0 >= T.w)
            fail("BIG task of piece " + std::to_string(b.sn) + " has a bad tile origin");
        for (int64_t e = b.e0; e < b.e1; ++e) {
            const WaveEntry& E = S.big_entries[(size_t)e];
            int64_t u = -1;
            for (int64_t q = T.upd0; q < T.upd0 + T.nupd; ++q)
                if (S.upd[q].src == E.src && S.upd[q].K == E.K) u = q;
            const int mi = E.mn & 255, nj = (E.mn >> 8) & 255;
            const bool ident = big_ident(E);
            const int ms = big_strip_rows(E), ns = big_strip_cols(E);
            if ((ms || ns) && (e >= b.em || mi != kBigTile || nj != kBigTile || ms > kStripMax || ns > kStripMax))
                fail("BIG entry " + std::to_string(e) + " carries a strip but is not a full dense block");
            if (u < 0 || mi < 1 || mi > kBigTile || nj < 1 || nj > kBigTile || E.ia + mi + ms > S.upd[u].m || E.ja + nj + ns > S.upd[u].n1 ||
                ident != (S.upd[u].rel < 0) || S.level_of[S.upd_src[u]] != b.src_level) {
                fail("BIG entry " + std::to_string(e) + " of piece " + std::to_string(b.sn) + " has a bad window or source");
                continue;
            }
            auto rel_at = [&](int k) { return ident ? k : S.relpos[(size_t)S.upd[u].rel + k] - T.rbias; };
            if (rel_at(E.ia) / win_r != b.row0 / win_r || rel_at(E.ia + mi + ms - 1) / win_r != b.row0 / win_r ||
                rel_at(E.ja) / win_c != b.col0 / win_c || rel_at(E.ja + nj + ns - 1) / win_c != b.col0 / win_c)
                fail("BIG entry " + std::to_string(e) + " names rows outside its task's tile");
            covered[(size_t)u] += block_flops(E);
        }
    }
    {
        std::vector<int64_t> starts;
        std::vector<int64_t> dense_pos(S.big_all.size(), -1), ragged_pos(S.big_all.size(), -1);
        int64_t li = 0;
        for (const Launch& l : S.chol) {
            ++li;
            if (l.kind != kLaunchBig && l.kind != kLaunchDense) continue;
            const bool dense = l.kind == kLaunchDense;
            const bool side = l.side != 0;
            auto find_task = [&](int64_t e) -> const Schedule::BigTask* {
                auto it = std::upper_bound(S.big_all.begin(), S.big_all.end(), e,
                                           [](int64_t v, const Schedule::BigTask& b) { return v < b.e0; });
                if (it == S.big_all.begin()) return nullptr;
                --it;
                return e < it->e1 ? &*it : nullptr;
            };
            auto right_launch = [&](const Schedule::BigTask& b) {
                return side != (b.next != 0) && (side ? l.wait_level : l.level - 1) == b.src_level;
            };
            for (int q = l.first; q < l.first + l.count; ++q) {
                const TileDesc& td = S.big_tasks[(size_t)q];
                if (td.wp >= td.sp) {
                    if (td.wp != td.sp) fail("BIG launch task " + std::to_string(q) + " has a negative entry range");
                    continue;
                }
                const Schedule::BigTask* it = find_task(td.wp);
                const bool ok = it && (dense ? (it->e0 == td.wp && it->em == td.sp && (td.part & ~kDenseStripTask) == it->dchunks &&
                                                ((td.part & kDenseStripTask) != 0) == (it->strips > 0))
                                             : (it->em == td.wp && it->e1 == td.sp));
                if (!ok || it->sn != td.sn || it->row0 != td.row0 || it->col0 != td.col0) {
                    fail("BIG launch task " + std::to_string(q) + " is not a task of the plan");
                    continue;
                }
                if (!right_launch(*it)) fail("BIG launch task " + std::to_string(q) + " runs in the launch of another source level");
                (dense ? dense_pos : ragged_pos)[(size_t)(it - S.big_all.data())] = li;
                starts.push_back(td.wp);
            }
        }
        std::sort(starts.begin(), starts.end());
        if (std::adjacent_find(starts.begin(), starts.end()) != starts.end()) fail("a BIG task is launched twice");
        int64_t want = 0;
        for (size_t k = 0; k < S.big_all.size(); ++k) {
            const Schedule::BigTask& b = S.big_all[k];
            if (b.em < b.e0 || b.em > b.e1) fail("BIG task " + std::to_string(k) + " has a bad dense / ragged split");
            int64_t dch = 0;
            int32_t nst = 0;
            for (int64_t e = b.e0; e < b.em; ++e) {
                const WaveEntry& E = S.big_entries[(size_t)e];
                nst += big_strip_rows(E) || big_strip_cols(E);
                if (E.K < kDenseChunk) fail("BIG entry " + std::to_string(e) + " is filed as dense but is narrower than a chunk");
                dch += ceil_div(E.K, kDenseChunk);
            }
            if (dch != b.dchunks) fail("BIG task " + std::to_string(k) + " has a wrong dense chunk count");
            if (nst != b.strips) fail("BIG task " + std::to_string(k) + " has a wrong count of entries with strips");
            if (!S.active_piece[b.sn]) continue;
            want += (b.em > b.e0) + (b.e1 > b.em);
            if (b.em > b.e0 && b.e1 > b.em && !(dense_pos[k] > 0 && ragged_pos[k] > dense_pos[k]))
                fail("BIG task " + std::to_string(k) + ": the ragged part is not launched after the dense part");
        }
        if ((int64_t)starts.size() != want)
            fail("BIG launches hold " + std::to_string(starts.size()) + " task parts, the active targets have " + std::to_string(want));
    }
    for (int t = 0; t < nc; ++t) {
        const SnDesc& T = S.csn[t];
        if (is_small(T)) continue;
        for (int64_t u = T.upd0; u < T.upd0 + T.nupd; ++u) {
            const UpdDesc& U = S.upd[u];
            const double want = (double)U.K * U.n1 * (U.n1 + 1) + 2.0 * U.K * (double)(U.m - U.n1) * U.n1;
            if (std::abs(covered[(size_t)u] - want) > 1e-9 * want + 0.5)
                fail("update " + std::to_string(u) + " of piece " + std::to_string(t) + " is not covered exactly once by its entries");
        }
    }
    for (int t = 0; t < nc; ++t) {
        const int real = S.csn_real[t], st = S.chol_subtree[real];
        if (st < 0) continue;
        if (!is_small(S.csn[t])) fail("supernode " + std::to_string(real) + " of a subtree is not a SMALL one");
        for (int64_t u = S.csn[t].upd0; u < S.csn[t].upd0 + S.csn[t].nupd; ++u)
            if (S.chol_subtree[S.csn_real[S.upd_src[u]]] != st)
                fail("supernode " + std::to_string(real) + " of a subtree is updated from outside the subtree");
    }
    {
        std::vector<int> seen(nc, 0);
        for (const Launch& l : S.chol) {
            if (l.kind != kLaunchSmall) continue;
            if (l.fused == 2) {
                for (int b = l.first; b < l.first + l.count; ++b) {
                    const int32_t q0 = S.small_ranges[2 * (size_t)b], q1 = S.small_ranges[2 * (size_t)b + 1];
                    if (q0 < 0 || q1 <= q0 || q1 > (int32_t)S.small_list.size()) {
                        fail("subtree launch: bad range " + std::to_string(b));
                        continue;
                    }
                    for (int32_t q = q0; q < q1; ++q) {
                        seen[S.small_list[q]]++;
                        if (q > q0 && S.small_list[q] <= S.small_list[q - 1]) fail("subtree launch: a run is not in index order");
                        if (S.chol_subtree[S.csn_real[S.small_list[q]]] != S.chol_subtree[S.csn_real[S.small_list[q0]]])
                            fail("subtree launch: a run mixes subtrees");
                    }
                }
            } else {
                for (int q = l.first; q < l.first + l.count; ++q) seen[S.small_list[q]]++;
            }
        }
        for (int t = 0; t < nc; ++t)
            if (seen[t] != ((is_small(S.csn[t]) && S.active_piece[t]) ? 1 : 0))
                fail("SMALL supernode " + std::to_string(t) + " is in " + std::to_string(seen[t]) + " launches");
    }
    int main_level = -1;
    for (size_t i = 0; i < S.chol.size(); ++i) {
        const Launch& l = S.chol[i];
        if (l.side) {
            if (l.wait_level >= 0 && main_level > l.wait_level + 0 && main_level >= l.level)
                fail("side launch " + std::to_string(i) + " is enqueued after the level that waits for it");
            for (size_t j = i + 1; j < S.chol.size(); ++j)
                if (!S.chol[j].side && S.chol[j].level <= l.wait_level)
                    fail("side launch " + std::to_string(i) + " precedes a main-stream launch of a level it waits for");
        } else {
            if (l.level < main_level) fail("main-stream launches go down a level");
            main_level = l.level;
        }
    }
    return bad;
}

}
```

### parsy_bench_amd/csrc/schedule.hpp

```cpp
#pragma once
#include <cstddef>
#include <cstdint>
#include <string>
#include <vector>

#include "inspector.hpp"

namespace parsy {

constexpr int kTile = 64;
constexpr int kSub = 32;
constexpr int kSmallMaxEntries = 6144;
constexpr int kSmallMaxWidth = 64;
constexpr int kBelowRows = 512;
constexpr int kBelowMaxGroups = 512;
constexpr int kBackGroup = 2;
constexpr int kTinyWidth = 16;
constexpr int kTinyWidth2 = 32;
constexpr int kPanelRows = 128;
constexpr int kSolveRows = 256;
constexpr int kSolveRowsMrhs = 128;

struct SnDesc {
    int64_t px;
    int64_t pi;
    int64_t upd0;
    int32_t c0, w, r;
    int32_t nupd;
    int32_t a0, a1;
    int32_t dslot;
    int32_t tflag0;
    int32_t ld;
    int32_t rbias;
};

struct UpdDesc {
    int64_t src;
    int64_t rel;
    int32_t ld;
    int32_t K;
    int32_t m;
    int32_t n1;
};

struct WaveEntry {
    int64_t src;
    int32_t rel;
    int32_t ld, K;
    int32_t ia, ja;
    int32_t mn;
};
constexpr int kStripMax = 16;
inline bool big_ident(const WaveEntry& E) { return (E.mn >> 16) & 1; }
inline int big_strip_rows(const WaveEntry& E) { return (E.mn >> 17) & 31; }
inline int big_strip_cols(const WaveEntry& E) { return (E.mn >> 22) & 31; }
constexpr int kDenseStripTask = 1 << 30;

struct TileDesc {
    int32_t sn;
    int32_t row0, col0;
    int32_t part;
    int64_t wp;
    int64_t sp;
};

struct PanelDesc {
    int32_t sn;
    int32_t jb;
    int32_t row0;
    int32_t pad;
};

struct SubMember {
    int64_t px;
    int32_t c0, w, r;
    int32_t slot0;
    int32_t so;
    int32_t ld;
};
struct SubTree {
    int32_t m0, m1;
    int32_t ncols;
    int32_t nout;
    int32_t out0;
    int32_t pad[3];
};
struct SubTier {
    int32_t tree0, ntrees;
    int32_t max_slots;
    int32_t top_level;
};
constexpr int kSubMaxSlots = 320;
constexpr int kSubTierMaxWidth = 64;
constexpr int kSubTierMinTrees = 512;
constexpr int kSubTierMaxSlots = 448;
constexpr int kSubTierMaxDensity = 700;

enum LaunchKind : int32_t {
    kLaunchSmall = 0, kLaunchTiles = 1, kLaunchChain = 2, kLaunchBig = 3,
    kLaunchBackBelow = 4,
    kLaunchSolveSmall = 5, kLaunchSolvePanel = 6, kLaunchSolveFixup = 7, kLaunchBackBlock = 8,
    kLaunchDense = 9,
};
inline bool is_chol_launch(int kind) { return (kind >= 0 && kind <= kLaunchBig) || kind == kLaunchDense; }

struct Launch {
    int32_t kind;
    int32_t first, count;
    int32_t level;
    int32_t jb;
    int32_t lds_bytes;
    int32_t fused;
    int32_t side;
    int32_t wait_level;
    int32_t early;
};

constexpr int kSplitChunks = 192;
constexpr int kSplitTarget = 128;
constexpr int kSplitMaxParts = 4;
constexpr int kSplitFewTiles = 128;
constexpr int kSplitFewChunks = 32;
constexpr int kSplitFewTarget = 24;
constexpr int kSplitFewMaxParts = 8;
constexpr int kWalkerBatch = 64;
constexpr int kBigTile = 128;
constexpr int kBigMinK = 128;
constexpr int kPieceWidth = 512;
constexpr double kBigAutoFlops = 1e11;
constexpr double kPieceAutoFlops = 2e12;
constexpr double kChainSplitAutoFlops = 1e11;
constexpr int kBigSuperMinTasks = 12288;
constexpr double kBigSuperMaxFill = 0.85;
constexpr int kBigGroup = 8;
constexpr int kBigGroupsPerXcd = 2;
constexpr int kBigTailGroups = 16;
constexpr int kDenseChunk = 8;
constexpr double kDenseMinShare = 0.25;
constexpr double kDenseMinFill = 0.70;
constexpr double kDenseAllShare = 0.06;
constexpr int kPushGroup = 1;
constexpr int kOneMaxSupernodes = 8192;
constexpr int64_t kOneLargeEntries = 4096;
constexpr int64_t kOneMaxEntries = 1 << 28;
constexpr int kOneMaxSupernodesBig = 32768;
constexpr int kOneSmallBlocks = 1024;
constexpr int kOneMidBlocks = 4096;
constexpr int kOneRhs8Density = 300;
constexpr int kOneMaxRhs = 8;
constexpr int kCholSubtreesPerCu = 64;
constexpr int kSubtreesPerCu = 16;
constexpr double kSubtreeMinCost = 2e5;
constexpr int kSubtreeMinPerSlot = 2;
constexpr int kSolveSubtreeMinMembers = 2048;

struct Schedule {
    int n = 0, nsuper = 0, nlevels = 0;
    bool solve_only = false;
    int64_t nnzA = 0, ssize = 0, xsize = 0, nnzL = 0;
    int max_width = 0, max_rows = 0, n_small = 0, n_big = 0;
    int n_solve_wide = 0;
    int64_t n_dslots = 0;
    int64_t n_tflags = 0;
    int n_chain_launches = 0;
    int n_solve_chain_launches = 0;
    int walker_batch = kWalkerBatch;
    double flops_stored = 0, update_flops = 0, reread_bytes = 0;
    double tile_update_flops = 0;
    double inner_flops = 0;

    std::vector<SnDesc> sn;
    std::vector<int> sparent;
    std::vector<SnDesc> csn;
    std::vector<int32_t> piece0;
    std::vector<int32_t> csn_real;
    std::vector<int> clevelPtr, clevelSet;
    int cnlevels = 0;
    int big_min_k = kBigMinK, piece_width = kPieceWidth, push_group = kPushGroup;
    int big_super_r = 0, big_super_c = 0;
    std::vector<UpdDesc> upd;
    std::vector<int32_t> upd_src;
    std::vector<int32_t> relpos;
    std::vector<int64_t> a_dst;
    std::vector<int32_t> rows;
    std::vector<WaveEntry> wave_entries;
    std::vector<int64_t> wave_ptr;

    std::vector<int32_t> chol_subtree, solve_subtree, bsolve_subtree;
    std::vector<int32_t> solve_subtree_all, bsolve_subtree_all;
    std::vector<double> chol_cost, solve_cost;
    int n_chol_subtrees = 0, n_solve_subtrees = 0, n_bsolve_subtrees = 0;
    std::vector<int32_t> small_ranges, solve_small_ranges, bsolve_ranges;
    std::vector<SubMember> sub_members;
    std::vector<SubTree> sub_trees;
    std::vector<uint16_t> sub_slots;
    std::vector<int32_t> sub_out_rows;
    std::vector<SubTier> sub_tiers;
    int sub_cover_level = -1;
    int sub_max_slots = 0;

    std::vector<int32_t> small_list;
    std::vector<TileDesc> tiles;
    std::vector<WaveEntry> big_entries;
    struct BigTask { int32_t sn, row0, col0, weight; int64_t e0, e1; int32_t src_level, next;
                     int32_t sr, sc;
                     int64_t em; int32_t dweight, dchunks;
                     int32_t strips; };
    std::vector<BigTask> big_all;
    std::vector<TileDesc> big_tasks;
    double big_flops = 0;
    double dense_flops = 0;
    int64_t n_dense_entries = 0;
    int64_t n_strip_entries = 0;
    std::vector<Launch> chol;

    std::vector<int32_t> solve_small_list;
    std::vector<PanelDesc> solve_panels;
    std::vector<PanelDesc> solve_mtasks;
    std::vector<int32_t> solve_fix_list;
    std::vector<int32_t> solve_wide_list;
    std::vector<Launch> solve;

    std::vector<PanelDesc> bsolve_pairs;
    std::vector<PanelDesc> bsolve_blocks;
    std::vector<PanelDesc> bsolve_below;
    int64_t n_bpart_slots = 0;
    std::vector<Launch> bsolve;

    struct OneLists {
        std::vector<SnDesc> sn;
        std::vector<int64_t> slot0;
        std::vector<int32_t> wleft;
        int64_t nslots = 0;
        std::vector<int32_t> pull_ptr, pull_slot, pull_pos;
        std::vector<uint8_t> member;
        void clear() { *this = OneLists(); }
    };
    bool solve_one = false, solve_one_back = false;
    bool one_subtrees = false;
    bool one_big = false;
    bool one_forced = false;
    OneLists one_f, one_b;
    const OneLists& one_back() const { return one_b.sn.empty() ? one_f : one_b; }

    std::vector<uint8_t> active;
    std::vector<uint8_t> active_piece;
    std::vector<size_t> chol_level_begin;
    std::vector<int> levelPtr, levelSet;
    std::vector<int64_t> split_ranges;
    std::vector<int64_t> tile_split;
    struct SplitDesc { int64_t ranges; int64_t sp; int32_t nparts; int32_t pad; };
    std::vector<SplitDesc> split_desc;
    int64_t n_split_doubles = 0;
    std::vector<int64_t> sn_wp0;
    std::vector<int64_t> sn_tw0;
    std::vector<int32_t> tile_w;
    std::vector<int32_t> level_of;
};

void build_schedule(const PatternRef& P, const size_t* lC, const int* A2p, const int* A2i,
                    const uint8_t* active, Schedule& out, int compute_units = 0);
void build_launches(Schedule& S, const uint8_t* active, const uint8_t* active_pieces = nullptr);
int64_t simulate_chain(const Schedule& S, int slots);
int64_t check_schedule(const Schedule& S, std::string& what);
constexpr int kSmallMaxUpdates = 8;
inline bool is_small(const SnDesc& d) {
    return d.w <= kSmallMaxWidth && (int64_t)d.w * d.r <= kSmallMaxEntries && d.nupd <= kSmallMaxUpdates;
}

}
```

Baseline: 2.982 factorizations/s.

## Regroup ragged BIG update blocks into larger per-launch regions chosen by makespan

Splits the ragged (non-dense) remainder of BIG Schedule tasks into separate RaggedTask groups whose tile region size (br x bc) per launch is picked from candidate shapes by a greedy makespan estimate over a fixed slot count. Ragged blocks in regions that already hold dense work stay tied to that dense task, while the other blocks are re-cut into coarser regions. The aim is fewer, better-balanced ragged tasks per launch and more reuse of target tiles. It adds schedule-build cost and new checker logic, and depends on the executor consuming the new ragged task lists.

```diff
diff --git a/parsy_bench_amd/csrc/capi_exec.hip b/parsy_bench_amd/csrc/capi_exec.hip
--- a/parsy_bench_amd/csrc/capi_exec.hip
+++ b/parsy_bench_amd/csrc/capi_exec.hip
@@ -3,6 +3,7 @@
 #include <chrono>
 #include <cstdio>
 #include <cstring>
+#include <functional>
 #include <map>
 #include <algorithm>
 #include <atomic>
@@ -305,7 +306,7 @@
     o->inner_flops = S.inner_flops;
     o->tile_update_flops = S.tile_update_flops;
     o->big_flops = S.big_flops;
-    o->big_entries = (int64_t)S.big_entries.size();
+    o->big_entries = S.n_big_entries;
     o->big_tasks = (int32_t)S.big_tasks.size();
     o->n_pieces = (int32_t)S.csn.size();
     o->chol_levels = S.cnlevels;
@@ -396,48 +397,77 @@
     return S.nlevels;
 }
 
+static void for_each_big_entry(const parsy::Schedule& S,
+                               const std::function<void(int64_t, int, const parsy::WaveEntry&, bool)>& fn) {
+    std::vector<int64_t> rest(S.big_all.size(), -1);
+    for (size_t r = 0; r < S.big_ragged.size(); ++r)
+        if (S.big_ragged[r].dense_task >= 0) rest[(size_t)S.big_ragged[r].dense_task] = (int64_t)r;
+    for (size_t t = 0; t < S.big_all.size(); ++t) {
+        const parsy::Schedule::BigTask& b = S.big_all[t];
+        const int launch = b.src_level * 2 + (b.next ? 0 : 1);
+        for (int64_t e = b.e0; e < b.em; ++e) fn((int64_t)t, launch, S.big_entries[(size_t)e], true);
+        if (rest[t] >= 0)
+            for (int64_t e = b.em; e < b.e1; ++e) fn((int64_t)t, launch, S.big_entries[(size_t)e], false);
+    }
+    for (size_t r = 0; r < S.big_ragged.size(); ++r) {
+        const parsy::Schedule::RaggedTask& g = S.big_ragged[r];
+        if (g.dense_task >= 0) continue;
+        for (int64_t e = g.e0; e < g.e1; ++e)
+            fn((int64_t)(S.big_all.size() + r), g.src_level * 2 + (g.next ? 0 : 1), S.big_entries[(size_t)e], false);
+    }
+}
+
 int64_t parsy_debug_big_entries(const parsy_plan* pl, int32_t* out, int64_t cap) {
     if (!pl) return -1;
-    const parsy::Schedule& S = pl->S;
-    int64_t n = 0, t = 0;
-    for (const parsy::Schedule::BigTask& b : S.big_all) {
-        for (int64_t e = b.e0; e < b.e1; ++e, ++n) {
-            if (!out || n >= cap) continue;
-            const parsy::WaveEntry& E = S.big_entries[(size_t)e];
+    int64_t n = 0;
+    for_each_big_entry(pl->S, [&](int64_t t, int launch, const parsy::WaveEntry& E, bool) {
+        if (out && n < cap) {
             int32_t* o = out + 7 * n;
             o[0] = (int32_t)t;
-            o[1] = b.src_level * 2 + (b.next ? 0 : 1);
+            o[1] = launch;
             o[2] = E.K;
             o[3] = E.mn & 255;
             o[4] = (E.mn >> 8) & 255;
             o[5] = ((E.mn >> 16) & 1) != 0;
             o[6] = E.ia - E.ja;
         }
-        ++t;
-    }
+        ++n;
+    });
     return n;
 }
 
 int64_t parsy_debug_big_windows(const parsy_plan* pl, int64_t* out, int64_t cap) {
     if (!pl) return -1;
-    const parsy::Schedule& S = pl->S;
-    int64_t n = 0, t = 0;
-    for (const parsy::Schedule::BigTask& b : S.big_all) {
-        for (int64_t e = b.e0; e < b.e1; ++e, ++n) {
-            if (!out || n >= cap) continue;
-            const parsy::WaveEntry& E = S.big_entries[(size_t)e];
+    int64_t n = 0;
+    for_each_big_entry(pl->S, [&](int64_t t, int launch, const parsy::WaveEntry& E, bool dense) {
+        if (out && n < cap) {
             int64_t* o = out + 9 * n;
             o[0] = t;
-            o[1] = b.src_level * 2 + (b.next ? 0 : 1);
+            o[1] = launch;
             o[2] = E.K;
             o[3] = E.mn & 255;
             o[4] = (E.mn >> 8) & 255;
             o[5] = E.ia;
             o[6] = E.ja;
             o[7] = E.src;
-            o[8] = e < b.em;
-        }
-        ++t;
+            o[8] = dense;
+        }
+        ++n;
+    });
+    return n;
+}
+
+int64_t parsy_debug_ragged_launches(const parsy_plan* pl, int64_t* out, int64_t cap) {
+    if (!pl) return -1;
+    const parsy::Schedule& S = pl->S;
+    int64_t n = 0;
+    for (const parsy::Schedule::RaggedLaunch& R : S.ragged_launches) {
+        if (out && n < cap) {
+            int64_t* o = out + 13 * n;
+            o[0] = R.launch, o[1] = R.sr, o[2] = R.sc, o[3] = R.br, o[4] = R.bc;
+            for (int w = 0; w < 2; ++w) o[5 + 4 * w] = R.tasks[w], o[6 + 4 * w] = R.chunks[w], o[7 + 4 * w] = R.bytes[w], o[8 + 4 * w] = R.span[w];
+        }
+        ++n;
     }
     return n;
 }
diff --git a/parsy_bench_amd/csrc/schedule.cpp b/parsy_bench_amd/csrc/schedule.cpp
--- a/parsy_bench_amd/csrc/schedule.cpp
+++ b/parsy_bench_amd/csrc/schedule.cpp
@@ -289,7 +289,7 @@
     struct Group { int32_t win, first, len; };
     std::vector<Group> groups, cgroups;
     std::vector<int64_t> cursor;
-    struct BigKeyed { int64_t launch_tile; WaveEntry e; int16_t sr, sc; };
+    struct BigKeyed { int64_t launch_tile; WaveEntry e; int16_t sr, sc; int64_t u; };
     std::vector<BigKeyed> bigk;
     std::vector<int64_t> big_tile0(nc + 1, 0);
     int env_sr = 0, env_sc = 0;
@@ -356,6 +356,26 @@
                 const int nbc = ceil_div(S.csn[t].w, kTile), nbr = ceil_div(S.csn[t].r, kTile);
                 level_tiles[(size_t)S.level_of[t]] += (int64_t)nbc * nbr - (int64_t)nbc * (nbc - 1) / 2;
             }
+    auto rows_by_window = [&](const SnDesc& T, const UpdDesc& U, int win_rows, std::vector<Group>& out) {
+        out.clear();
+        for (int k = 0; k < U.m;) {
+            const int win = (U.rel < 0 ? k : S.relpos[(size_t)U.rel + k] - T.rbias) / win_rows;
+            int k1 = k + 1;
+            if (U.rel < 0) k1 = std::min(U.m, (win + 1) * win_rows);
+            else while (k1 < U.m && (S.relpos[(size_t)U.rel + k1] - T.rbias) / win_rows == win) ++k1;
+            out.push_back(Group{win, k, k1 - k});
+            k = k1;
+        }
+    };
+    auto blocks_of = [&](const UpdDesc& U, const Group& gr, const Group& gc, int njt, auto&& fn) {
+        for (int cb = 0; cb < njt; cb += kBigTile)
+            for (int rb = 0; rb < gr.len; rb += kBigTile) {
+                const int mi = std::min(kBigTile, gr.len - rb), nj = std::min(kBigTile, njt - cb);
+                const int ia = gr.first + rb, ja = gc.first + cb;
+                if (ia + mi - 1 < ja) continue;
+                fn(WaveEntry{U.src, (int32_t)std::max<int64_t>(U.rel, 0), U.ld, U.K, ia, ja, mi | (nj << 8) | ((U.rel < 0) << 16)});
+            }
+    };
     for (int t = 0; t < nc; ++t) {
         SnDesc& T = S.csn[t];
         big_tile0[t + 1] = big_tile0[t];
@@ -426,36 +446,18 @@
             if (lev_s >= lev_t) throw std::runtime_error("schedule: an update source is not below its target");
             const int64_t launch = (int64_t)lev_s * 2 + (lev_s == lev_t - 1 ? 0 : 1);
             const int sr = env_sr ? env_sr : launch_super[(size_t)launch], sc = env_sr ? env_sc : launch_super[(size_t)launch];
-            auto make_groups = [&](int win_rows, std::vector<Group>& out) {
-                out.clear();
-                for (int k = 0; k < U.m;) {
-                    const int win = rel_at(U, k) / win_rows;
-                    int k1 = k + 1;
-                    if (U.rel < 0) k1 = std::min(U.m, (win + 1) * win_rows);
-                    else while (k1 < U.m && rel_at(U, k1) / win_rows == win) ++k1;
-                    out.push_back(Group{win, k, k1 - k});
-                    k = k1;
-                }
-            };
-            make_groups(kBigTile * sr, groups);
+            rows_by_window(T, U, kBigTile * sr, groups);
             if (sc == sr) cgroups = groups;
-            else make_groups(kBigTile * sc, cgroups);
+            else rows_by_window(T, U, kBigTile * sc, cgroups);
             for (const Group& gc : cgroups) {
                 if (gc.first >= U.n1) break;
                 const int njt = std::min(gc.len, U.n1 - gc.first);
                 for (const Group& gr : groups) {
                     if ((int64_t)(gr.win + 1) * sr * kBigTile - 1 < (int64_t)gc.win * sc * kBigTile) continue;
                     const int64_t tile = big_tile0[t] + (int64_t)gc.win * sc * nbr128 + (int64_t)gr.win * sr;
-                    for (int cb = 0; cb < njt; cb += kBigTile)
-                        for (int rb = 0; rb < gr.len; rb += kBigTile) {
-                            const int mi = std::min(kBigTile, gr.len - rb), nj = std::min(kBigTile, njt - cb);
-                            const int ia = gr.first + rb, ja = gc.first + cb;
-                            if (ia + mi - 1 < ja) continue;
-                            bigk.push_back(BigKeyed{(launch << 40) | tile,
-                                                    WaveEntry{U.src, (int32_t)std::max<int64_t>(U.rel, 0), U.ld, U.K, ia, ja,
-                                                              mi | (nj << 8) | ((U.rel < 0) << 16)},
-                                                    (int16_t)sr, (int16_t)sc});
-                        }
+                    blocks_of(U, gr, gc, njt, [&](const WaveEntry& E) {
+                        bigk.push_back(BigKeyed{(launch << 40) | tile, E, (int16_t)sr, (int16_t)sc, u});
+                    });
                 }
             }
         }
@@ -542,6 +544,7 @@
         const bool dense_strips = env_int("PARSY_DENSE_STRIPS", 1) != 0;
         std::map<std::pair<int64_t, int64_t>, size_t> strip_of;
         std::vector<uint8_t> absorbed;
+        std::vector<uint8_t> ragged_k(bigk.size(), 0);
         int t = 0;
         for (size_t i = 0; i < bigk.size();) {
             size_t j = i;
@@ -600,6 +603,7 @@
                 if (!is_dense(bigk[q].e, lmode) && !absorbed[q - i]) {
                     S.big_entries[at++] = bigk[q].e;
                     weight += ceil_div(bigk[q].e.K, 16) + 4;
+                    ragged_k[q] = 1;
                 }
             const size_t jend = at;
             S.n_dense_entries += (int64_t)(mid - i);
@@ -618,6 +622,211 @@
                                                   (int64_t)mid, (int32_t)std::min<int64_t>(dweight, INT32_MAX),
                                                   (int32_t)std::min<int64_t>(dchunks, INT32_MAX), nstrips});
             i = j;
+        }
+        {
+            const size_t nl = launch_super.size();
+            const int64_t tile_mask = (1LL << 40) - 1;
+            int force_r = env_sr ? 0 : -1, force_c = force_r;
+            if (const char* e = std::getenv("PARSY_BIG_RAGGED_REGION")) {
+                int a = 0, b = 0;
+                const int got = std::sscanf(e, "%dx%d", &a, &b);
+                if (got >= 1 && a == 0) force_r = force_c = 0;
+                else if (got == 2 && a >= 1 && a <= 64 && b >= 1 && b <= 64) force_r = a, force_c = b;
+            }
+            auto launch_of = [](const Schedule::BigTask& b) { return (size_t)b.src_level * 2 + (b.next ? 0 : 1); };
+            std::vector<int16_t> lsr(nl, 0), lsc(nl, 0);
+            for (const Schedule::BigTask& b : S.big_all)
+                if (b.e1 > b.em) lsr[launch_of(b)] = (int16_t)b.sr, lsc[launch_of(b)] = (int16_t)b.sc;
+            std::vector<int64_t> u_first(S.upd.size() + 1, 0), by_u(bigk.size());
+            for (const BigKeyed& b : bigk) u_first[(size_t)b.u + 1]++;
+            for (size_t u = 0; u < S.upd.size(); ++u) u_first[u + 1] += u_first[u];
+            {
+                std::vector<int64_t> at(u_first.begin(), u_first.end() - 1);
+                for (size_t q = 0; q < bigk.size(); ++q) by_u[(size_t)at[(size_t)bigk[q].u]++] = (int64_t)q;
+            }
+            std::vector<int64_t> dkeys;
+            auto cut = [&](const std::vector<int16_t>& gbr, const std::vector<int16_t>& gbc, auto&& fn) {
+                for (int t = 0; t < nc; ++t) {
+                    const SnDesc& T = S.csn[t];
+                    if (is_small(T)) continue;
+                    const int lev_t = S.level_of[t], nbr128 = ceil_div(T.r, kBigTile);
+                    for (int64_t u = T.upd0; u < T.upd0 + T.nupd; ++u) {
+                        const UpdDesc& U = S.upd[u];
+                        if (!is_big(U, t)) continue;
+                        const int lev_s = S.level_of[S.upd_src[u]];
+                        const int64_t launch = (int64_t)lev_s * 2 + (lev_s == lev_t - 1 ? 0 : 1);
+                        const int br = gbr[(size_t)launch], bc = gbc[(size_t)launch];
+                        if (br == 0) continue;
+                        dkeys.clear();
+                        bool any = false;
+                        auto region_of = [&](const BigKeyed& B, int& rt, int& ct) {
+                            const int64_t local = (B.launch_tile & tile_mask) - big_tile0[t];
+                            rt = (int)(local % nbr128) / br;
+                            ct = (int)(local / nbr128) / bc;
+                        };
+                        for (int64_t p = u_first[(size_t)u]; p < u_first[(size_t)u + 1]; ++p) {
+                            const size_t q = (size_t)by_u[(size_t)p];
+                            int rt, ct;
+                            region_of(bigk[q], rt, ct);
+                            if (ragged_k[q]) any = true;
+                            else dkeys.push_back(((int64_t)rt << 24) | ct);
+                        }
+                        if (!any) continue;
+                        std::sort(dkeys.begin(), dkeys.end());
+                        dkeys.erase(std::unique(dkeys.begin(), dkeys.end()), dkeys.end());
+                        if (!dkeys.empty())
+                            for (int64_t p = u_first[(size_t)u]; p < u_first[(size_t)u + 1]; ++p) {
+                                const size_t q = (size_t)by_u[(size_t)p];
+                                if (!ragged_k[q]) continue;
+                                int rt, ct;
+                                region_of(bigk[q], rt, ct);
+                                if (std::binary_search(dkeys.begin(), dkeys.end(), ((int64_t)rt << 24) | ct))
+                                    fn(launch, big_tile0[t] + (int64_t)ct * bc * nbr128 + (int64_t)rt * br, bigk[q].e);
+                            }
+                        rows_by_window(T, U, kBigTile * br, groups);
+                        if (bc == br) cgroups = groups;
+                        else rows_by_window(T, U, kBigTile * bc, cgroups);
+                        for (const Group& gc : cgroups) {
+                            if (gc.first >= U.n1) break;
+                            const int njt = std::min(gc.len, U.n1 - gc.first);
+                            for (const Group& gr : groups) {
+                                if ((int64_t)(gr.win + 1) * br * kBigTile - 1 < (int64_t)gc.win * bc * kBigTile) continue;
+                                if (std::binary_search(dkeys.begin(), dkeys.end(), ((int64_t)gr.win << 24) | gc.win)) continue;
+                                const int64_t tile = big_tile0[t] + (int64_t)gc.win * bc * nbr128 + (int64_t)gr.win * br;
+                                blocks_of(U, gr, gc, njt, [&](const WaveEntry& E) { fn(launch, tile, E); });
+                            }
+                        }
+                    }
+                }
+            };
+            auto makespan = [](std::vector<int64_t>& w) {
+                std::sort(w.begin(), w.end(), std::greater<int64_t>());
+                std::priority_queue<int64_t, std::vector<int64_t>, std::greater<int64_t>> slots;
+                int64_t span = 0;
+                for (int64_t x : w) {
+                    int64_t load = x;
+                    if ((int)slots.size() >= kRaggedSlots) {
+                        load += slots.top();
+                        slots.pop();
+                    }
+                    slots.push(load);
+                    span = std::max(span, load);
+                }
+                return span;
+            };
+            std::vector<std::vector<int64_t>> lw(nl);
+            for (const Schedule::BigTask& b : S.big_all)
+                if (b.e1 > b.em) lw[launch_of(b)].push_back(b.weight);
+            std::vector<int64_t> span0(nl, 0), best(nl, 0);
+            for (size_t l = 0; l < nl; ++l) best[l] = span0[l] = makespan(lw[l]);
+            std::vector<int16_t> cbr(nl, 0), cbc(nl, 0), gbr(nl, 0), gbc(nl, 0);
+            if (force_r > 0) {
+                for (size_t l = 0; l < nl; ++l)
+                    if (lsr[l]) {
+                        cbr[l] = (int16_t)std::min(64, ceil_div(force_r, lsr[l]) * lsr[l]);
+                        cbc[l] = (int16_t)std::min(64, ceil_div(force_c, lsc[l]) * lsc[l]);
+                        if (cbr[l] % lsr[l] || cbc[l] % lsc[l] || (cbr[l] == lsr[l] && cbc[l] == lsc[l])) cbr[l] = cbc[l] = 0;
+                    }
+            } else if (force_r < 0) {
+                static const int cand[6][2] = {{2, 2}, {4, 2}, {2, 4}, {4, 4}, {8, 2}, {8, 4}};
+                std::vector<std::pair<int64_t, int64_t>> kw;
+                for (const auto& c : cand) {
+                    bool some = false;
+                    for (size_t l = 0; l < nl; ++l) {
+                        const bool ok = lsr[l] && c[0] >= lsr[l] && c[1] >= lsc[l] && c[0] % lsr[l] == 0 && c[1] % lsc[l] == 0 &&
+                                        !(c[0] == lsr[l] && c[1] == lsc[l]);
+                        gbr[l] = ok ? (int16_t)c[0] : 0;
+                        gbc[l] = ok ? (int16_t)c[1] : 0;
+                        some |= ok;
+                    }
+                    if (!some) continue;
+                    kw.clear();
+                    cut(gbr, gbc, [&](int64_t launch, int64_t tile, const WaveEntry& E) {
+                        kw.push_back({(launch << 40) | tile, (int64_t)ceil_div(E.K, 16) + 4});
+                    });
+                    std::sort(kw.begin(), kw.end());
+                    for (size_t l = 0; l < nl; ++l) lw[l].clear();
+                    for (size_t i = 0; i < kw.size();) {
+                        size_t j = i;
+                        int64_t w = 0;
+                        for (; j < kw.size() && kw[j].first == kw[i].first; ++j) w += kw[j].second;
+                        lw[(size_t)(kw[i].first >> 40)].push_back(std::min<int64_t>(w, INT32_MAX));
+                        i = j;
+                    }
+                    for (size_t l = 0; l < nl; ++l) {
+                        if (!gbr[l]) continue;
+                        const int64_t span = makespan(lw[l]);
+                        if (span < best[l]) best[l] = span, cbr[l] = gbr[l], cbc[l] = gbc[l];
+                    }
+                }
+            }
+            struct RKeyed { int64_t key; WaveEntry e; };
+            std::vector<RKeyed> rk;
+            cut(cbr, cbc, [&](int64_t launch, int64_t tile, const WaveEntry& E) { rk.push_back(RKeyed{(launch << 40) | tile, E}); });
+            std::stable_sort(rk.begin(), rk.end(), [](const RKeyed& a, const RKeyed& b) { return a.key < b.key; });
+            std::vector<std::pair<int64_t, Schedule::RaggedTask>> tasks;
+            for (size_t k = 0; k < S.big_all.size(); ++k) {
+                const Schedule::BigTask& b = S.big_all[k];
+                if (b.e1 > b.em && cbr[launch_of(b)] == 0)
+                    tasks.push_back({(int64_t)k, Schedule::RaggedTask{b.sn, b.row0, b.col0, b.weight, b.em, b.e1, b.src_level, b.next,
+                                                                       b.sr, b.sc, (int64_t)k}});
+            }
+            std::vector<int64_t> all_keys(S.big_all.size());
+            for (size_t k = 0; k < S.big_all.size(); ++k) all_keys[k] = bigk[(size_t)S.big_all[k].e0].launch_tile;
+            const int64_t base = (int64_t)S.big_entries.size();
+            S.big_entries.resize((size_t)base + rk.size());
+            for (size_t i = 0; i < rk.size();) {
+                size_t j = i;
+                int64_t weight = 0;
+                for (; j < rk.size() && rk[j].key == rk[i].key; ++j) {
+                    S.big_entries[(size_t)base + j] = rk[j].e;
+                    weight += ceil_div(rk[j].e.K, 16) + 4;
+                }
+                const int64_t launch = rk[i].key >> 40, tile = rk[i].key & tile_mask;
+                const int tt = (int)(std::upper_bound(big_tile0.begin(), big_tile0.end(), tile) - big_tile0.begin()) - 1;
+                const int nbr128 = ceil_div(S.csn[tt].r, kBigTile);
+                const int64_t local = tile - big_tile0[tt];
+                const int64_t pos = std::lower_bound(all_keys.begin(), all_keys.end(), rk[i].key) - all_keys.begin();
+                tasks.push_back({pos, Schedule::RaggedTask{tt, (int32_t)(local % nbr128) * kBigTile, (int32_t)(local / nbr128) * kBigTile,
+                                                           (int32_t)std::min<int64_t>(weight, INT32_MAX), base + (int64_t)i, base + (int64_t)j,
+                                                           (int32_t)(launch >> 1), (int32_t)((launch & 1) == 0), cbr[(size_t)launch],
+                                                           cbc[(size_t)launch], -1}});
+                i = j;
+            }
+            std::stable_sort(tasks.begin(), tasks.end(), [](const auto& a, const auto& b) { return a.first < b.first; });
+            S.big_ragged.reserve(tasks.size());
+            for (const auto& kt : tasks) S.big_ragged.push_back(kt.second);
+            S.n_big_entries = 0;
+            for (size_t k = 0; k < S.big_all.size(); ++k) {
+                const int64_t end = k + 1 < S.big_all.size() ? S.big_all[k + 1].e0 : (int64_t)bigk.size();
+                for (int64_t q = S.big_all[k].e0; q < end; ++q) S.n_big_entries += !ragged_k[(size_t)q];
+            }
+            std::vector<Schedule::RaggedLaunch> stats(nl);
+            for (size_t l = 0; l < nl; ++l)
+                stats[l] = Schedule::RaggedLaunch{(int32_t)l, lsr[l], lsc[l], cbr[l] ? cbr[l] : lsr[l], cbr[l] ? cbc[l] : lsc[l],
+                                                  {0, 0}, {0, 0}, {0, 0}, {span0[l], 0}};
+            auto count = [&](Schedule::RaggedLaunch& R, int which, int64_t e0, int64_t e1) {
+                R.tasks[which]++;
+                for (int64_t e = e0; e < e1; ++e) {
+                    const WaveEntry& E = S.big_entries[(size_t)e];
+                    R.chunks[which] += ceil_div(E.K, 16);
+                    R.bytes[which] += 8LL * E.K * ((E.mn & 255) + ((E.mn >> 8) & 255));
+                }
+            };
+            for (const Schedule::BigTask& b : S.big_all)
+                if (b.e1 > b.em) count(stats[launch_of(b)], 0, b.em, b.e1);
+            for (size_t l = 0; l < nl; ++l) lw[l].clear();
+            for (const Schedule::RaggedTask& r : S.big_ragged) {
+                const size_t l = (size_t)r.src_level * 2 + (r.next ? 0 : 1);
+                count(stats[l], 1, r.e0, r.e1);
+                lw[l].push_back(r.weight);
+                S.n_big_entries += r.e1 - r.e0;
+            }
+            for (size_t l = 0; l < nl; ++l)
+                if (lsr[l]) {
+                    stats[l].span[1] = makespan(lw[l]);
+                    S.ragged_launches.push_back(stats[l]);
+                }
         }
     }
 
@@ -857,34 +1066,36 @@
     std::vector<Launch> early_launches;
     std::vector<size_t> level_begin;
     std::vector<int> bigs, sbigs;
-    std::vector<std::vector<const Schedule::BigTask*>> big_next(S.cnlevels), big_push(S.cnlevels);
+    struct BigItem { int32_t sn, row0, col0, weight, gr, gc, part; int64_t wp, sp; };
+    std::vector<std::vector<BigItem>> big_next(S.cnlevels), big_push(S.cnlevels), rag_next(S.cnlevels), rag_push(S.cnlevels);
     for (const Schedule::BigTask& b : S.big_all)
-        if (S.active_piece[b.sn]) (b.next ? big_next : big_push)[b.src_level].push_back(&b);
+        if (S.active_piece[b.sn] && b.em > b.e0)
+            (b.next ? big_next : big_push)[b.src_level].push_back(
+                BigItem{b.sn, b.row0, b.col0, b.dweight, b.sr, b.sc, b.dchunks | (b.strips > 0 ? kDenseStripTask : 0), b.e0, b.em});
+    for (const Schedule::RaggedTask& r : S.big_ragged)
+        if (S.active_piece[r.sn] && r.e1 > r.e0)
+            (r.next ? rag_next : rag_push)[r.src_level].push_back(BigItem{r.sn, r.row0, r.col0, r.weight, r.br, r.bc, 0, r.e0, r.e1});
     const int big_group = env_int("PARSY_BIG_GROUP", kBigGroup);
-    auto emit_big = [&](const std::vector<const Schedule::BigTask*>& all, Launch L, bool dense) {
-        std::vector<const Schedule::BigTask*> v;
-        for (const Schedule::BigTask* b : all)
-            if (dense ? b->em > b->e0 : b->e1 > b->em) v.push_back(b);
+    auto emit_big = [&](const std::vector<BigItem>& all, Launch L) {
+        std::vector<const BigItem*> v;
+        for (const BigItem& b : all) v.push_back(&b);
         if (v.empty()) return L;
         L.first = (int32_t)S.big_tasks.size();
-        auto wt = [dense](const Schedule::BigTask* b) { return dense ? b->dweight : b->weight; };
-        auto desc = [dense](const Schedule::BigTask* b) {
-            return dense ? TileDesc{b->sn, b->row0, b->col0, b->dchunks | (b->strips > 0 ? kDenseStripTask : 0), b->e0, b->em}
-                         : TileDesc{b->sn, b->row0, b->col0, 0, b->em, b->e1};
-        };
-        auto by_weight = [&](const Schedule::BigTask* a, const Schedule::BigTask* b) { return wt(a) > wt(b); };
+        auto wt = [](const BigItem* b) { return b->weight; };
+        auto desc = [](const BigItem* b) { return TileDesc{b->sn, b->row0, b->col0, b->part, b->wp, b->sp}; };
+        auto by_weight = [&](const BigItem* a, const BigItem* b) { return wt(a) > wt(b); };
         int g = big_group;
-        const int per_task = v[0]->sr * v[0]->sc;
+        const int per_task = v[0]->gr * v[0]->gc;
         while (g > 1 && (int64_t)v.size() * per_task < (int64_t)8 * kBigGroupsPerXcd * g * g) g /= 2;
-        if (g < std::max(v[0]->sr, v[0]->sc)) g = 1;
+        if (g < std::max(v[0]->gr, v[0]->gc)) g = 1;
         if (g <= 1) {
             std::stable_sort(v.begin(), v.end(), by_weight);
-            for (const Schedule::BigTask* b : v) S.big_tasks.push_back(desc(b));
+            for (const BigItem* b : v) S.big_tasks.push_back(desc(b));
             L.count = (int32_t)v.size();
             return L;
         }
-        struct Group { int64_t key, weight; int32_t maxw; std::vector<const Schedule::BigTask*> tasks; };
-        std::vector<const Schedule::BigTask*> seq[8];
+        struct Group { int64_t key, weight; int32_t maxw; std::vector<const BigItem*> tasks; };
+        std::vector<const BigItem*> seq[8];
         int64_t load[8] = {0, 0, 0, 0, 0, 0, 0, 0};
         auto least = [&] {
             int x = 0;
@@ -892,20 +1103,20 @@
                 if (load[q] < load[x]) x = q;
             return x;
         };
-        std::vector<const Schedule::BigTask*> rest(v);
+        std::vector<const BigItem*> rest(v);
         for (; !rest.empty(); g /= 2) {
             if (g <= 1) {
                 std::stable_sort(rest.begin(), rest.end(), by_weight);
-                for (const Schedule::BigTask* b : rest) {
+                for (const BigItem* b : rest) {
                     const int x = least();
                     seq[x].push_back(b);
                     load[x] += wt(b);
                 }
                 break;
             }
-            std::vector<std::pair<int64_t, const Schedule::BigTask*>> keyed;
+            std::vector<std::pair<int64_t, const BigItem*>> keyed;
             keyed.reserve(rest.size());
-            for (const Schedule::BigTask* b : rest) {
+            for (const BigItem* b : rest) {
                 const int64_t gi = b->row0 / (kBigTile * g), gj = b->col0 / (kBigTile * g);
                 keyed.push_back({((int64_t)b->sn << 32) | (gj << 16) | gi, b});
             }
@@ -1014,15 +1225,15 @@
             if (L.count > 0) S.chol.push_back(L);
         }
         if (lev + 2 < S.cnlevels) {
-            Launch Ld = emit_big(big_push[lev], Launch{kLaunchDense, 0, 0, lev + 2, 0, 0, 0, 1, lev, 1}, true);
+            Launch Ld = emit_big(big_push[lev], Launch{kLaunchDense, 0, 0, lev + 2, 0, 0, 0, 1, lev, 1});
             if (Ld.count > 0) early_launches.push_back(Ld);
-            Launch Lp = emit_big(big_push[lev], Launch{kLaunchBig, 0, 0, lev + 2, 0, 0, 0, 1, lev, 1}, false);
+            Launch Lp = emit_big(rag_push[lev], Launch{kLaunchBig, 0, 0, lev + 2, 0, 0, 0, 1, lev, 1});
             if (Lp.count > 0) early_launches.push_back(Lp);
         }
         if (lev > 0) {
-            Launch Ld = emit_big(big_next[lev - 1], Launch{kLaunchDense, 0, 0, lev, 0, 0, 0, 0, -1, 0}, true);
+            Launch Ld = emit_big(big_next[lev - 1], Launch{kLaunchDense, 0, 0, lev, 0, 0, 0, 0, -1, 0});
             if (Ld.count > 0) S.chol.push_back(Ld);
-            Launch Ln = emit_big(big_next[lev - 1], Launch{kLaunchBig, 0, 0, lev, 0, 0, 0, 0, -1, 0}, false);
+            Launch Ln = emit_big(rag_next[lev - 1], Launch{kLaunchBig, 0, 0, lev, 0, 0, 0, 0, -1, 0});
             if (Ln.count > 0) S.chol.push_back(Ln);
         }
         if (!bigs.empty()) {
@@ -1889,14 +2100,16 @@
                 }
         }
     }
-    for (const Schedule::BigTask& b : S.big_all) {
-        const SnDesc& T = S.csn[b.sn];
-        if (b.src_level >= S.level_of[b.sn] || (b.next != 0) != (b.src_level == S.level_of[b.sn] - 1))
-            fail("BIG task of piece " + std::to_string(b.sn) + " is filed under the wrong source level");
-        const int win_r = kBigTile * b.sr, win_c = kBigTile * b.sc;
-        if (b.sr < 1 || b.sc < 1 || b.row0 % win_r || b.col0 % win_c || b.row0 + win_r <= b.col0 || b.row0 >= T.r || b.col0 >= T.w)
-            fail("BIG task of piece " + std::to_string(b.sn) + " has a bad tile origin");
-        for (int64_t e = b.e0; e < b.e1; ++e) {
+    struct Rect { int64_t u; int32_t ia, mi, ja, nj; };
+    std::vector<Rect> rects;
+    auto check_task = [&](int32_t sn, int32_t src_level, int32_t next, int win_r, int win_c, int32_t row0, int32_t col0, int64_t e0,
+                          int64_t e1, bool dense) {
+        const SnDesc& T = S.csn[sn];
+        if (src_level >= S.level_of[sn] || (next != 0) != (src_level == S.level_of[sn] - 1))
+            fail("BIG task of piece " + std::to_string(sn) + " is filed under the wrong source level");
+        if (win_r < kBigTile || win_c < kBigTile || row0 % win_r || col0 % win_c || row0 + win_r <= col0 || row0 >= T.r || col0 >= T.w)
+            fail("BIG task of piece " + std::to_string(sn) + " has a bad tile origin");
+        for (int64_t e = e0; e < e1; ++e) {
             const WaveEntry& E = S.big_entries[(size_t)e];
             int64_t u = -1;
             for (int64_t q = T.upd0; q < T.upd0 + T.nupd; ++q)
@@ -1904,23 +2117,76 @@
             const int mi = E.mn & 255, nj = (E.mn >> 8) & 255;
             const bool ident = big_ident(E);
             const int ms = big_strip_rows(E), ns = big_strip_cols(E);
-            if ((ms || ns) && (e >= b.em || mi != kBigTile || nj != kBigTile || ms > kStripMax || ns > kStripMax))
+            if ((ms || ns) && (!dense || mi != kBigTile || nj != kBigTile || ms > kStripMax || ns > kStripMax))
                 fail("BIG entry " + std::to_string(e) + " carries a strip but is not a full dense block");
             if (u < 0 || mi < 1 || mi > kBigTile || nj < 1 || nj > kBigTile || E.ia + mi + ms > S.upd[u].m || E.ja + nj + ns > S.upd[u].n1 ||
-                ident != (S.upd[u].rel < 0) || S.level_of[S.upd_src[u]] != b.src_level) {
-                fail("BIG entry " + std::to_string(e) + " of piece " + std::to_string(b.sn) + " has a bad window or source");
+                ident != (S.upd[u].rel < 0) || S.level_of[S.upd_src[u]] != src_level) {
+                fail("BIG entry " + std::to_string(e) + " of piece " + std::to_string(sn) + " has a bad window or source");
                 continue;
             }
             auto rel_at = [&](int k) { return ident ? k : S.relpos[(size_t)S.upd[u].rel + k] - T.rbias; };
-            if (rel_at(E.ia) / win_r != b.row0 / win_r || rel_at(E.ia + mi + ms - 1) / win_r != b.row0 / win_r ||
-                rel_at(E.ja) / win_c != b.col0 / win_c || rel_at(E.ja + nj + ns - 1) / win_c != b.col0 / win_c)
+            if (rel_at(E.ia) / win_r != row0 / win_r || rel_at(E.ia + mi + ms - 1) / win_r != row0 / win_r ||
+                rel_at(E.ja) / win_c != col0 / win_c || rel_at(E.ja + nj + ns - 1) / win_c != col0 / win_c)
                 fail("BIG entry " + std::to_string(e) + " names rows outside its task's tile");
             covered[(size_t)u] += block_flops(E);
+            rects.push_back(Rect{u, E.ia, mi, E.ja, nj});
+            if (ms) rects.push_back(Rect{u, E.ia + mi, ms, E.ja, nj});
+            if (ns) rects.push_back(Rect{u, E.ia, mi, E.ja + nj, ns});
+        }
+    };
+    for (const Schedule::BigTask& b : S.big_all) {
+        if (b.sr < 1 || b.sc < 1) fail("BIG task of piece " + std::to_string(b.sn) + " has a bad tile origin");
+        check_task(b.sn, b.src_level, b.next, kBigTile * b.sr, kBigTile * b.sc, b.row0, b.col0, b.e0, b.em, true);
+    }
+    for (const Schedule::RaggedTask& r : S.big_ragged) {
+        if (r.br < 1 || r.bc < 1) fail("ragged BIG task of piece " + std::to_string(r.sn) + " has a bad region");
+        check_task(r.sn, r.src_level, r.next, kBigTile * r.br, kBigTile * r.bc, r.row0, r.col0, r.e0, r.e1, false);
+        if (r.dense_task >= 0) {
+            const bool ok = r.dense_task < (int64_t)S.big_all.size();
+            const Schedule::BigTask* b = ok ? &S.big_all[(size_t)r.dense_task] : nullptr;
+            if (!ok || b->sn != r.sn || b->row0 != r.row0 || b->col0 != r.col0 || b->sr != r.br || b->sc != r.bc || b->em != r.e0 ||
+                b->e1 != r.e1 || b->src_level != r.src_level || b->next != r.next)
+                fail("ragged BIG task of piece " + std::to_string(r.sn) + " is not the ragged rest of the task it names");
+        }
+    }
+    std::sort(rects.begin(), rects.end(), [](const Rect& a, const Rect& b) {
+        return a.u != b.u ? a.u < b.u : a.ia != b.ia ? a.ia < b.ia : a.ja < b.ja;
+    });
+    for (size_t i = 0; i < rects.size(); ++i)
+        for (size_t j = i + 1; j < rects.size() && rects[j].u == rects[i].u && rects[j].ia < rects[i].ia + rects[i].mi; ++j)
+            if (rects[j].ja < rects[i].ja + rects[i].nj && rects[i].ja < rects[j].ja + rects[j].nj) {
+                fail("update " + std::to_string(rects[i].u) + ": two BIG blocks overlap");
+                break;
+            }
+    {
+        std::vector<size_t> order(S.big_ragged.size());
+        for (size_t k = 0; k < order.size(); ++k) order[k] = k;
+        auto key = [&](size_t k) {
+            const Schedule::RaggedTask& r = S.big_ragged[k];
+            return ((int64_t)(r.src_level * 2 + (r.next ? 0 : 1)) << 32) | (uint32_t)r.sn;
+        };
+        std::sort(order.begin(), order.end(), [&](size_t a, size_t b) {
+            return key(a) != key(b) ? key(a) < key(b) : S.big_ragged[a].row0 < S.big_ragged[b].row0;
+        });
+        for (size_t i = 0; i < order.size(); ++i) {
+            const Schedule::RaggedTask& a = S.big_ragged[order[i]];
+            for (size_t j = i + 1; j < order.size() && key(order[j]) == key(order[i]); ++j) {
+                const Schedule::RaggedTask& b = S.big_ragged[order[j]];
+                if (b.row0 >= a.row0 + kBigTile * a.br) break;
+                if (b.col0 < a.col0 + kBigTile * a.bc && a.col0 < b.col0 + kBigTile * b.bc) {
+                    fail("two ragged BIG tasks of piece " + std::to_string(a.sn) + " share tiles in one launch");
+                    break;
+                }
+            }
         }
     }
     {
         std::vector<int64_t> starts;
-        std::vector<int64_t> dense_pos(S.big_all.size(), -1), ragged_pos(S.big_all.size(), -1);
+        std::vector<std::pair<int64_t, size_t>> ragged_at(S.big_ragged.size());
+        for (size_t k = 0; k < S.big_ragged.size(); ++k) ragged_at[k] = {S.big_ragged[k].e0, k};
+        std::sort(ragged_at.begin(), ragged_at.end());
+        const size_t nlaunch = (size_t)2 * std::max(S.cnlevels, 1);
+        std::vector<int64_t> dense_last(nlaunch, -1), ragged_first(nlaunch, INT64_MAX);
         int64_t li = 0;
         for (const Launch& l : S.chol) {
             ++li;
@@ -1934,8 +2200,8 @@
                 --it;
                 return e < it->e1 ? &*it : nullptr;
             };
-            auto right_launch = [&](const Schedule::BigTask& b) {
-                return side != (b.next != 0) && (side ? l.wait_level : l.level - 1) == b.src_level;
+            auto right_launch = [&](int32_t src_level, int32_t next) {
+                return side != (next != 0) && (side ? l.wait_level : l.level - 1) == src_level;
             };
             for (int q = l.first; q < l.first + l.count; ++q) {
                 const TileDesc& td = S.big_tasks[(size_t)q];
@@ -1943,21 +2209,36 @@
                     if (td.wp != td.sp) fail("BIG launch task " + std::to_string(q) + " has a negative entry range");
                     continue;
                 }
-                const Schedule::BigTask* it = find_task(td.wp);
-                const bool ok = it && (dense ? (it->e0 == td.wp && it->em == td.sp && (td.part & ~kDenseStripTask) == it->dchunks &&
-                                                ((td.part & kDenseStripTask) != 0) == (it->strips > 0))
-                                             : (it->em == td.wp && it->e1 == td.sp));
-                if (!ok || it->sn != td.sn || it->row0 != td.row0 || it->col0 != td.col0) {
-                    fail("BIG launch task " + std::to_string(q) + " is not a task of the plan");
-                    continue;
-                }
-                if (!right_launch(*it)) fail("BIG launch task " + std::to_string(q) + " runs in the launch of another source level");
-                (dense ? dense_pos : ragged_pos)[(size_t)(it - S.big_all.data())] = li;
+                if (dense) {
+                    const Schedule::BigTask* it = find_task(td.wp);
+                    const bool ok = it && it->e0 == td.wp && it->em == td.sp && (td.part & ~kDenseStripTask) == it->dchunks &&
+                                    ((td.part & kDenseStripTask) != 0) == (it->strips > 0);
+                    if (!ok || it->sn != td.sn || it->row0 != td.row0 || it->col0 != td.col0) {
+                        fail("BIG launch task " + std::to_string(q) + " is not a task of the plan");
+                        continue;
+                    }
+                    if (!right_launch(it->src_level, it->next)) fail("BIG launch task " + std::to_string(q) + " runs in the launch of another source level");
+                    const size_t lid = (size_t)it->src_level * 2 + (it->next ? 0 : 1);
+                    dense_last[lid] = std::max(dense_last[lid], li);
+                } else {
+                    auto at = std::lower_bound(ragged_at.begin(), ragged_at.end(), std::make_pair(td.wp, (size_t)0));
+                    const Schedule::RaggedTask* it = at != ragged_at.end() && at->first == td.wp ? &S.big_ragged[at->second] : nullptr;
+                    if (!it || it->e1 != td.sp || td.part != 0 || it->sn != td.sn || it->row0 != td.row0 || it->col0 != td.col0) {
+                        fail("BIG launch task " + std::to_string(q) + " is not a task of the plan");
+                        continue;
+                    }
+                    if (!right_launch(it->src_level, it->next)) fail("BIG launch task " + std::to_string(q) + " runs in the launch of another source level");
+                    const size_t lid = (size_t)it->src_level * 2 + (it->next ? 0 : 1);
+                    ragged_first[lid] = std::min(ragged_first[lid], li);
+                }
                 starts.push_back(td.wp);
             }
         }
         std::sort(starts.begin(), starts.end());
         if (std::adjacent_find(starts.begin(), starts.end()) != starts.end()) fail("a BIG task is launched twice");
+        for (size_t l = 0; l < nlaunch; ++l)
+            if (dense_last[l] >= 0 && ragged_first[l] < dense_last[l])
+                fail("BIG launch " + std::to_string(l) + ": the ragged tasks are not launched after the dense parts");
         int64_t want = 0;
         for (size_t k = 0; k < S.big_all.size(); ++k) {
             const Schedule::BigTask& b = S.big_all[k];
@@ -1972,11 +2253,10 @@
             }
             if (dch != b.dchunks) fail("BIG task " + std::to_string(k) + " has a wrong dense chunk count");
             if (nst != b.strips) fail("BIG task " + std::to_string(k) + " has a wrong count of entries with strips");
-            if (!S.active_piece[b.sn]) continue;
-            want += (b.em > b.e0) + (b.e1 > b.em);
-            if (b.em > b.e0 && b.e1 > b.em && !(dense_pos[k] > 0 && ragged_pos[k] > dense_pos[k]))
-                fail("BIG task " + std::to_string(k) + ": the ragged part is not launched after the dense part");
-        }
+            if (S.active_piece[b.sn]) want += b.em > b.e0;
+        }
+        for (const Schedule::RaggedTask& r : S.big_ragged)
+            if (S.active_piece[r.sn]) want += r.e1 > r.e0;
         if ((int64_t)starts.size() != want)
             fail("BIG launches hold " + std::to_string(starts.size()) + " task parts, the active targets have " + std::to_string(want));
     }
diff --git a/parsy_bench_amd/csrc/schedule.hpp b/parsy_bench_amd/csrc/schedule.hpp
--- a/parsy_bench_amd/csrc/schedule.hpp
+++ b/parsy_bench_amd/csrc/schedule.hpp
@@ -135,6 +135,7 @@
 constexpr int kBigGroup = 8;
 constexpr int kBigGroupsPerXcd = 2;
 constexpr int kBigTailGroups = 16;
+constexpr int kRaggedSlots = 512;
 constexpr int kDenseChunk = 8;
 constexpr double kDenseMinShare = 0.25;
 constexpr double kDenseMinFill = 0.70;
@@ -207,6 +208,13 @@
                      int64_t em; int32_t dweight, dchunks;
                      int32_t strips; };
     std::vector<BigTask> big_all;
+    struct RaggedTask { int32_t sn, row0, col0, weight; int64_t e0, e1; int32_t src_level, next;
+                        int32_t br, bc;
+                        int64_t dense_task; };
+    std::vector<RaggedTask> big_ragged;
+    struct RaggedLaunch { int32_t launch, sr, sc, br, bc; int64_t tasks[2], chunks[2], bytes[2], span[2]; };
+    std::vector<RaggedLaunch> ragged_launches;
+    int64_t n_big_entries = 0;
     std::vector<TileDesc> big_tasks;
     double big_flops = 0;
     double dense_flops = 0;
```

New measurement: 2.999 factorizations/s (median of 6 runs). Within noise of the previous version (+0.6%).
